# Sthiber/COSC_4397_Pathtracing_Raytracing_Project

Hardware: AMD Instinct MI355X
Metric: Msamples/s, cornell.txt 1920x1080 depth 8 (+PSNR vs 5000spp ref) (higher is better)
Workload: dtype f32

## Files before the change

cosc_4397_pathtracing_raytracing_project_amd/capi.py:

```python
from __future__ import annotations

import ctypes as C
import os
from typing import Optional, Sequence, Tuple

import numpy as np

_PKG = os.path.dirname(os.path.abspath(__file__))
LIB_PATH = os.environ.get("PT_AMD_LIB") or os.path.join(_PKG, "libpt_amd.so")
PT_MAX_DEPTH = 64
ARITH = {"exact": 0, "fma": 1, "fast": 2}
ARITH_NAMES = {v: k for k, v in ARITH.items()}
FEATURE_PLANES = 3
NOISE_PLANES = 2
NOISE_PIXELS_PER_PARTIAL = 1024
CONVERGENCE_WAVES = 16
CONVERGENCE_CAPACITY = 65536
FLT_MAX = float(np.finfo(np.float32).max)


class PtGeom(C.Structure):
    _fields_ = [("type", C.c_int32), ("materialid", C.c_int32), ("transform", C.c_float * 16),
                ("inverseTransform", C.c_float * 16), ("invTranspose", C.c_float * 16)]


class PtMaterial(C.Structure):
    _fields_ = [("color", C.c_float * 3), ("specular_exponent", C.c_float), ("specular_color", C.c_float * 3),
                ("hasReflective", C.c_float), ("hasRefractive", C.c_float), ("indexOfRefraction", C.c_float),
                ("emittance", C.c_float)]


class PtCamera(C.Structure):
    _fields_ = [("resolution", C.c_int32 * 2), ("position", C.c_float * 3), ("lookAt", C.c_float * 3),
                ("view", C.c_float * 3), ("up", C.c_float * 3), ("right", C.c_float * 3), ("fov", C.c_float * 2),
                ("pixelLength", C.c_float * 2)]


class PtBVHNode(C.Structure):
    _fields_ = [("bmin", C.c_float * 3), ("bmax", C.c_float * 3), ("left", C.c_int32), ("right", C.c_int32),
                ("geomIndex", C.c_int32)]


class PtGridInfo(C.Structure):
    _fields_ = [("res", C.c_int32 * 3), ("origin", C.c_float * 3), ("cell_size", C.c_float * 3), ("pad", C.c_float),
                ("num_cells", C.c_int32), ("num_records", C.c_int32), ("num_leaves", C.c_int32)]


class PtGridRecord(C.Structure):
    _fields_ = [("bmin", C.c_float * 3), ("bmax", C.c_float * 3), ("leaf", C.c_int32), ("neighbours", C.c_int32)]


class PtSceneDesc(C.Structure):
    _fields_ = [("geoms", C.POINTER(PtGeom)), ("num_geoms", C.c_int32), ("materials", C.POINTER(PtMaterial)),
                ("num_materials", C.c_int32), ("camera", PtCamera), ("trace_depth", C.c_int32)]


class PtOptions(C.Structure):
    _fields_ = [("device", C.c_int32), ("pixel_begin", C.c_int32), ("pixel_count", C.c_int32),
                ("iters_per_batch", C.c_int32), ("num_queues", C.c_int32), ("blocks_per_cu", C.c_int32),
                ("time_kernels", C.c_int32), ("legacy_traversal", C.c_int32), ("debug_flags", C.c_int32), ("unfused_primary", C.c_int32), ("unfused_bounces", C.c_int32), ("stripe_pixels", C.c_int32), ("stripe_stride", C.c_int32),
                ("arith", C.c_int32), ("aa_jitter", C.c_int32), ("convergence", C.c_int32),
                ("lds_table_kb", C.c_int32), ("primary_pieces", C.c_int32), ("paths_pieces", C.c_int32), ("paths_min_piece", C.c_int32)]


class PtStats(C.Structure):
    _fields_ = [("samples", C.c_int64), ("live_rays", C.c_int64 * PT_MAX_DEPTH), ("intersect_launches", C.c_int64),
                ("intersect_ms", C.c_double), ("render_ms", C.c_double), ("num_cus", C.c_int32),
                ("grid_blocks", C.c_int32), ("num_queues", C.c_int32), ("iters_per_batch", C.c_int32),
                ("device_bytes", C.c_int64), ("primary_fused", C.c_int32), ("bounces_fused", C.c_int32),
                ("arith", C.c_int32), ("grid_cells", C.c_int32), ("tight_leaves", C.c_int32), ("paths_waves", C.c_int32)]


class PtDenoiseOptions(C.Structure):
    _fields_ = [("levels", C.c_int32), ("sigma_color", C.c_float), ("sigma_normal", C.c_float), ("sigma_position", C.c_float),
                ("keep_albedo", C.c_int32)]


class PtError(RuntimeError):
    pass


_lib: Optional[C.CDLL] = None
_fp = C.POINTER(C.c_float)
_ip = C.POINTER(C.c_int32)


def lib() -> C.CDLL:
    global _lib
    if _lib is not None:
        return _lib
    if not os.path.exists(LIB_PATH):
        raise PtError(f"{LIB_PATH} not found: run `python -c 'import __graft_entry__ as g; g.build()'` "
                      "(hipcc --offload-arch=gfx950).  There is no CPU fallback.")
    L = C.CDLL(LIB_PATH)
    L.pt_last_error.restype = C.c_char_p
    L.pt_scene_load.argtypes = [C.c_char_p, C.c_int, C.c_int, C.POINTER(C.c_void_p)]
    L.pt_scene_free.argtypes = [C.c_void_p]
    L.pt_scene_free.restype = None
    L.pt_scene_desc.argtypes = [C.c_void_p, C.POINTER(PtSceneDesc)]
    L.pt_scene_iterations.argtypes = [C.c_void_p]
    L.pt_scene_image_name.argtypes = [C.c_void_p]
    L.pt_scene_image_name.restype = C.c_char_p
    L.pt_build_bvh.argtypes = [C.POINTER(PtGeom), C.c_int, C.POINTER(PtBVHNode), C.c_int]
    L.pt_build_grid.argtypes = [C.POINTER(PtGeom), C.c_int, C.c_int, C.POINTER(PtGridInfo), C.POINTER(C.c_uint32), C.POINTER(PtGridRecord)]
    if hasattr(L, "pt_selfcheck_ieee"):
        L.pt_selfcheck_ieee.argtypes = [C.c_int, C.c_int, C.c_uint64, C.c_uint64, C.c_uint32, C.POINTER(C.c_uint64)]
    if hasattr(L, "pt_traversal_boxes"):
        L.pt_traversal_boxes.argtypes = [C.POINTER(PtGeom), C.c_int, _fp, _fp]
    if hasattr(L, "pt_center_half_box"):
        L.pt_center_half_box.argtypes = [_fp, _fp, C.c_int, C.c_float, _fp, _fp]
        L.pt_center_half_box.restype = None
    L.pt_build_transform.argtypes = [_fp, _fp, _fp, _fp]
    L.pt_init.argtypes = [C.POINTER(PtSceneDesc), C.POINTER(PtOptions)]
    L.pt_render.argtypes = [C.c_int, C.c_int]
    L.pt_readback.argtypes = [_fp]
    L.pt_readback_device.argtypes = [C.c_void_p]
    L.pt_preview_rgba8.argtypes = [C.c_int, C.POINTER(C.c_uint8)]
    L.pt_preview_rgba8_device.argtypes = [C.c_int, C.c_void_p]
    L.pt_get_stats.argtypes = [C.POINTER(PtStats)]
    L.pt_stage_generate.argtypes = [C.c_int, C.c_int, _fp, _fp]
    L.pt_stage_intersect.argtypes = [C.c_int, _fp, _fp, _fp, _fp, _ip, _fp]
    if hasattr(L, "pt_stage_intersect_grid"):
        L.pt_stage_intersect_grid.argtypes = [C.c_int, _fp, _fp, C.c_int, _fp, _fp, _ip, _fp]
        L.pt_stage_grid_info.argtypes = [C.POINTER(PtGridInfo), C.POINTER(C.c_int32)]
    L.pt_stage_shade.argtypes = [C.c_int, C.c_int, _ip, _ip, _fp, _fp, _ip, _fp, _fp, _fp, _fp, _ip]
    _u8p = C.POINTER(C.c_uint8)
    L.pt_save_u8.argtypes = [C.c_float, _u8p]
    L.pt_stage_save_u8.argtypes = [C.c_int, C.c_int, C.c_float, _fp, _u8p]
    L.pt_ctx_create.argtypes = [C.POINTER(PtSceneDesc), C.POINTER(PtOptions), C.POINTER(C.c_void_p)]
    L.pt_ctx_destroy.argtypes = [C.c_void_p]
    L.pt_ctx_render.argtypes = [C.c_void_p, C.c_int, C.c_int]
    L.pt_ctx_sync.argtypes = [C.c_void_p]
    L.pt_ctx_readback.argtypes = [C.c_void_p, _fp]
    L.pt_ctx_readback_device.argtypes = [C.c_void_p, C.c_void_p]
    L.pt_ctx_save_u8.argtypes = [C.c_void_p, C.c_float, _u8p]
    L.pt_ctx_get_stats.argtypes = [C.c_void_p, C.POINTER(PtStats)]
    L.pt_ctx_reset_stats.argtypes = [C.c_void_p]
    L.pt_ctx_clear.argtypes = [C.c_void_p]
    L.pt_ctx_pixel_count.argtypes = [C.c_void_p]
    L.pt_group_create.argtypes = [C.POINTER(PtSceneDesc), C.POINTER(PtOptions), _ip, C.c_int, C.POINTER(C.c_void_p)]
    if hasattr(L, "pt_group_create_ex"):
        L.pt_group_create_ex.argtypes = [C.POINTER(PtSceneDesc), C.POINTER(PtOptions), _ip, C.c_int, C.c_int, C.POINTER(C.c_void_p)]
        L.pt_group_transport.argtypes = [C.c_void_p]
    L.pt_group_destroy.argtypes = [C.c_void_p]
    L.pt_group_size.argtypes = [C.c_void_p]
    L.pt_group_context.argtypes = [C.c_void_p, C.c_int]
    L.pt_group_context.restype = C.c_void_p
    L.pt_group_render.argtypes = [C.c_void_p, C.c_int, C.c_int]
    L.pt_group_sync.argtypes = [C.c_void_p]
    L.pt_group_gather.argtypes = [C.c_void_p, _fp]
    L.pt_group_gather_u8.argtypes = [C.c_void_p, C.c_float, _u8p]
    L.pt_group_preview_rgba8.argtypes = [C.c_void_p, C.c_int, _u8p]
    L.pt_write_png_rgb8.argtypes = [C.c_char_p, _u8p, C.c_int, C.c_int]
    L.pt_output_basename.argtypes = [C.c_char_p, C.c_int, C.c_char_p, C.c_int]
    L.pt_save_png.argtypes = [C.c_char_p, _fp, C.c_int, C.c_int, C.c_float]
    L.pt_save_hdr.argtypes = [C.c_char_p, _fp, C.c_int, C.c_int, C.c_float]
    L.pt_save_pfm.argtypes = [C.c_char_p, _fp, C.c_int, C.c_int, C.c_float]
    L.pt_load_pfm.argtypes = [C.c_char_p, _fp, C.c_int, _ip, _ip, C.c_float]
    _dp = C.POINTER(C.c_double)
    L.pt_psnr_from_sse.argtypes = [C.c_double, C.c_int64]
    L.pt_psnr_from_sse.restype = C.c_float
    L.pt_set_reference.argtypes = [_fp]
    L.pt_get_convergence.argtypes = [C.c_int, C.c_int, _dp]
    L.pt_iterations_to_clean.argtypes = [C.c_float, _ip]
    L.pt_ctx_set_reference.argtypes = [C.c_void_p, _fp]
    L.pt_ctx_get_convergence.argtypes = [C.c_void_p, C.c_int, C.c_int, _dp]
    L.pt_ctx_iterations_to_clean.argtypes = [C.c_void_p, C.c_float, _ip]
    L.pt_group_set_reference.argtypes = [C.c_void_p, _fp]
    L.pt_group_get_convergence.argtypes = [C.c_void_p, C.c_int, C.c_int, _dp]
    L.pt_group_iterations_to_clean.argtypes = [C.c_void_p, C.c_float, _ip]
    if hasattr(L, "pt_render_features"):
        L.pt_render_features.argtypes = [C.c_int, C.c_int]
        L.pt_readback_features.argtypes = [_fp]
        L.pt_ctx_render_features.argtypes = [C.c_void_p, C.c_int, C.c_int]
        L.pt_ctx_readback_features.argtypes = [C.c_void_p, _fp]
        L.pt_ctx_device_features.argtypes = [C.c_void_p]
        L.pt_ctx_device_features.restype = C.c_void_p
        L.pt_group_render_features.argtypes = [C.c_void_p, C.c_int, C.c_int]
        L.pt_group_gather_features.argtypes = [C.c_void_p, _fp]
    if hasattr(L, "pt_denoise"):
        _dno = C.POINTER(PtDenoiseOptions)
        L.pt_denoise.argtypes = [C.c_float, _dno, _fp]
        L.pt_ctx_denoise.argtypes = [C.c_void_p, C.c_float, _dno, _fp]
        L.pt_ctx_denoise_device.argtypes = [C.c_void_p, C.c_float, _dno, C.POINTER(C.c_void_p)]
        L.pt_group_denoise.argtypes = [C.c_void_p, C.c_float, _dno, _fp]
        L.pt_stage_denoise.argtypes = [C.c_int, C.c_int, _fp, _fp, C.c_float, _dno, _fp]
        L.pt_denoise_host.argtypes = [C.c_int, C.c_int, _fp, _fp, C.c_float, _dno, _fp]
    if hasattr(L, "pt_denoise_guided"):
        _dno = C.POINTER(PtDenoiseOptions)
        _guided = [C.c_int, C.c_int, _fp, _fp, _fp, C.c_int, C.c_int64, _dno]
        L.pt_denoise_guided.argtypes = [_dno, _fp]
        L.pt_ctx_denoise_guided.argtypes = [C.c_void_p, _dno, _fp]
        L.pt_ctx_denoise_guided_device.argtypes = [C.c_void_p, _dno, C.POINTER(C.c_void_p)]
        L.pt_group_denoise_guided.argtypes = [C.c_void_p, _dno, _fp]
        L.pt_stage_denoise_guided.argtypes = _guided + [_fp]
        L.pt_denoise_guided_host.argtypes = _guided + [_fp]
        L.pt_denoise_guided_variance_host.argtypes = _guided + [_fp, _fp]
    if hasattr(L, "pt_noise_fold"):
        _until = [C.c_int, C.c_int, C.c_int, C.c_float, _ip, _fp]
        L.pt_noise_fold.argtypes = []
        L.pt_get_noise.argtypes = [_dp, _ip, _ip]
        L.pt_readback_noise.argtypes = [_fp]
        L.pt_render_until.argtypes = _until
        L.pt_ctx_noise_fold.argtypes = [C.c_void_p]
        L.pt_ctx_get_noise.argtypes = [C.c_void_p, _dp, _ip, _ip]
        L.pt_ctx_readback_noise.argtypes = [C.c_void_p, _fp]
        L.pt_ctx_render_until.argtypes = [C.c_void_p] + _until
        L.pt_ctx_device_noise.argtypes = [C.c_void_p]
        L.pt_ctx_device_noise.restype = C.c_void_p
        L.pt_group_noise_fold.argtypes = [C.c_void_p]
        L.pt_group_get_noise.argtypes = [C.c_void_p, _dp, _ip, _ip]
        L.pt_group_render_until.argtypes = [C.c_void_p] + _until
        L.pt_noise_fold_host.argtypes = [C.c_int, _fp, _fp, C.c_int, C.c_int, C.c_int64, _dp]
    if hasattr(L, "pt_adaptive_round"):
        _i64p = C.POINTER(C.c_int64)
        _adaptive = [C.c_int, C.c_int, C.c_int, C.c_float, C.c_float, _ip, _i64p, _fp]
        L.pt_adaptive_round.argtypes = [C.c_int, C.c_int, C.c_float]
        L.pt_render_adaptive.argtypes = _adaptive
        L.pt_readback_adaptive.argtypes = [_ip]
        L.pt_resolve.argtypes = [_fp]
        L.pt_ctx_adaptive_round.argtypes = [C.c_void_p, C.c_int, C.c_int, C.c_float]
        L.pt_ctx_render_adaptive.argtypes = [C.c_void_p] + _adaptive
        L.pt_ctx_readback_adaptive.argtypes = [C.c_void_p, _ip]
        L.pt_ctx_resolve.argtypes = [C.c_void_p, _fp]
        L.pt_ctx_resolve_device.argtypes = [C.c_void_p, C.POINTER(C.c_void_p)]
        L.pt_adaptive_select_host.argtypes = [C.c_int, C.c_int, _fp, _ip, C.c_int, _ip]
        L.pt_stage_adaptive_select.argtypes = [C.c_int, C.c_int, _fp, _ip, C.c_int, _ip]
        L.pt_adaptive_merge_host.argtypes = [C.c_int, _fp, _fp, _ip, _ip, C.c_int, _fp, C.c_int, _dp]
        L.pt_stage_render_list.argtypes = [_ip, C.c_int, C.c_int, C.c_int, _fp]
    if hasattr(L, "pt_denoise_adaptive"):
        _dno = C.POINTER(PtDenoiseOptions)
        _dn_adaptive = [C.c_int, C.c_int, _fp, _fp, _fp, _ip, _dno]
        L.pt_denoise_adaptive.argtypes = [_dno, _fp]
        L.pt_ctx_denoise_adaptive.argtypes = [C.c_void_p, _dno, _fp]
        L.pt_ctx_denoise_adaptive_device.argtypes = [C.c_void_p, _dno, C.POINTER(C.c_void_p)]
        L.pt_stage_denoise_adaptive.argtypes = _dn_adaptive + [_fp]
        L.pt_denoise_adaptive_host.argtypes = _dn_adaptive + [_fp]
        L.pt_denoise_adaptive_variance_host.argtypes = _dn_adaptive + [_fp, _fp]
    _lib = L
    return L


def _check(rc: int) -> None:
    if rc != 0:
        raise PtError(lib().pt_last_error().decode(errors="replace"))


def _f(a: np.ndarray):
    assert a.dtype == np.float32 and a.flags.c_contiguous
    return a.ctypes.data_as(_fp)


def _i(a: np.ndarray):
    assert a.dtype == np.int32 and a.flags.c_contiguous
    return a.ctypes.data_as(_ip)


class Scene:

    def __init__(self, path: str, res: Optional[Tuple[int, int]] = None):
        self._h = C.c_void_p()
        w, h = res if res else (0, 0)
        _check(lib().pt_scene_load(os.fsencode(path), int(w), int(h), C.byref(self._h)))
        self.desc = PtSceneDesc()
        _check(lib().pt_scene_desc(self._h, C.byref(self.desc)))

    def __del__(self):
        h = getattr(self, "_h", None)
        if h is not None and h.value and _lib is not None:
            _lib.pt_scene_free(h)
            self._h = C.c_void_p()

    @property
    def resolution(self) -> Tuple[int, int]:
        return self.desc.camera.resolution[0], self.desc.camera.resolution[1]

    @property
    def trace_depth(self) -> int:
        return self.desc.trace_depth

    @trace_depth.setter
    def trace_depth(self, d: int) -> None:
        self.desc.trace_depth = int(d)

    @property
    def iterations(self) -> int:
        return lib().pt_scene_iterations(self._h)

    @property
    def image_name(self) -> str:
        return lib().pt_scene_image_name(self._h).decode()

    def geoms(self):
        return [self.desc.geoms[i] for i in range(self.desc.num_geoms)]

    def materials(self):
        return [self.desc.materials[i] for i in range(self.desc.num_materials)]

    def grid(self, forced: bool = False):
        info = PtGridInfo()
        rc = lib().pt_build_grid(self.desc.geoms, self.desc.num_geoms, int(forced), C.byref(info), None, None)
        if rc < 0:
            raise PtError(lib().pt_last_error().decode(errors="replace"))
        if rc == 0:
            return None
        start = (C.c_uint32 * (info.num_cells + 1))()
        recs = (PtGridRecord * info.num_records)()
        lib().pt_build_grid(self.desc.geoms, self.desc.num_geoms, int(forced), C.byref(info), start, recs)
        return info, np.frombuffer(start, np.uint32).copy(), recs

    def traversal_boxes(self):
        boxes = np.zeros((self.desc.num_geoms, 6), np.float32)
        cam = np.asarray(list(self.desc.camera.position), np.float32)
        rc = lib().pt_traversal_boxes(self.desc.geoms, self.desc.num_geoms, _f(cam), _f(boxes))
        if rc < 0:
            raise PtError(lib().pt_last_error().decode(errors="replace"))
        return boxes, rc

    def bvh(self):
        n = lib().pt_build_bvh(self.desc.geoms, self.desc.num_geoms, None, 0)
        arr = (PtBVHNode * n)()
        lib().pt_build_bvh(self.desc.geoms, self.desc.num_geoms, arr, n)
        return arr


def selfcheck_ieee(kind: int, first: int, count: int, seed: int = 0, arith: str = "exact") -> int:
    n = C.c_uint64(0)
    _check(lib().pt_selfcheck_ieee(ARITH[arith], kind, first, count, seed, C.byref(n)))
    return int(n.value)


def build_transform(trs: Sequence[float]):
    t = np.asarray(trs, np.float32).copy()
    m, i, it = (np.zeros(16, np.float32) for _ in range(3))
    lib().pt_build_transform(_f(t), _f(m), _f(i), _f(it))
    return m, i, it


def make_options(device: int = 0, pixel_begin: int = 0, pixel_count: int = 0, iters_per_batch: int = 0,
                 num_queues: int = 0, blocks_per_cu: int = 0, time_kernels: bool = False, legacy_traversal: bool = False,
                 debug_flags: int = 0, unfused_primary: bool = False, unfused_bounces: bool = False,
                 stripe_pixels: int = 0, stripe_stride: int = 0, arith="exact", aa_jitter: bool = False,
                 lds_table_kb: int = 0, primary_pieces: int = 0, paths_pieces: int = 0, paths_min_piece: int = 0, primary_share: int = 0,
                 convergence: int = 0) -> PtOptions:
    opt = PtOptions()
    opt.device = device
    opt.pixel_begin = pixel_begin
    opt.pixel_count = pixel_count
    opt.iters_per_batch = iters_per_batch
    opt.num_queues = num_queues
    opt.blocks_per_cu = blocks_per_cu
    opt.time_kernels = 1 if time_kernels else 0
    opt.legacy_traversal = 1 if legacy_traversal else 0
    opt.debug_flags = int(debug_flags)
    opt.unfused_primary = 1 if unfused_primary else 0
    opt.unfused_bounces = 1 if unfused_bounces else 0
    opt.stripe_pixels = int(stripe_pixels)
    opt.stripe_stride = int(stripe_stride)
    opt.arith = ARITH[arith] if isinstance(arith, str) else int(arith)
    opt.aa_jitter = 1 if aa_jitter else 0
    opt.convergence = int(convergence)
    opt.lds_table_kb = int(lds_table_kb)
    pp = int(primary_pieces)
    opt.primary_pieces = pp if pp < 0 else min(pp, 0x7fff) | max(0, min(int(primary_share), 64)) << 16
    opt.paths_pieces = int(paths_pieces)
    opt.paths_min_piece = int(paths_min_piece)
    return opt


def split_features(planes: np.ndarray) -> dict:
    p = planes.reshape(FEATURE_PLANES, -1, 4)
    return dict(normal=np.ascontiguousarray(p[0, :, :3]), depth=np.ascontiguousarray(p[0, :, 3]),
                albedo=np.ascontiguousarray(p[1, :, :3]), hits=np.ascontiguousarray(p[1, :, 3]),
# ... 504 lines not shown
```

cosc_4397_pathtracing_raytracing_project_amd/csrc/pt_api.cpp:

```cpp
#include <cmath>
#include <cstdarg>
#include <cstdio>
#include <cstring>
#include <string>

#include "pt_adaptive.h"
#include "pt_context.h"
#include "pt_scene.h"
#include "pt_sched.h"

namespace {

std::string g_err;
constexpr int kDebugFlags = 16 | 32 | 64 | 128 | 256 | 512 | ptk::kRetireEveryIteration | 2048 | ptk::kWholeRecords;
static_assert(sizeof(PtOptions) == 80, "capi.PtOptions mirrors this layout");
static_assert(PT_CONVERGENCE_WAVES == ptk::kConvWaves, "pt_amd.h documents the size of the convergence metric's partial sums");
}
int pt_fail(const char* fmt, ...) {
  char buf[1024];
  va_list ap;
  va_start(ap, fmt);
  vsnprintf(buf, sizeof(buf), fmt, ap);
  va_end(ap);
  g_err = buf;
  return -1;
}

namespace ptc {
static PtContext* g_default = nullptr;
PtContext* default_context() { return g_default; }

int get_events(Ctx& g, EventPair* ev) {
  if (!g.free_events.empty()) {
    *ev = g.free_events.back();
    g.free_events.pop_back();
    return 0;
  }
  HIP_OK(hipEventCreate(&ev->a));
  HIP_OK(hipEventCreate(&ev->b));
  return 0;
}
static int resolve_events(Ctx& g) {
  auto drain = [&](std::vector<EventPair>& pending, double& total_ms) -> int {
    for (auto& e : pending) {
      float ms = 0;
      HIP_OK(hipEventElapsedTime(&ms, e.a, e.b));
      total_ms += ms;
      g.free_events.push_back(e);
    }
    pending.clear();
    return 0;
  };
  g.isect_launches += (int64_t)g.pending_isect.size();
  return drain(g.pending_isect, g.isect_ms) || drain(g.pending_render, g.render_ms) ? -1 : 0;
}

ptk::SceneTables tables(const Ctx& g) {
  ptk::SceneTables t = g.scene;
  if (g.debug_flags & 16) t.cull_margin = INFINITY;
  if (g.debug_flags & 32) t.top_xor = 0;
  t.lds_table_bytes = g.lds_table_bytes;
  t.max_batch_iters = g.K;
  t.trace_depth = g.depth;
  t.scan_nodes_lds = -1;
  t.use_grid = !g.grids.empty() && g.grid_enabled && !(g.debug_flags & 512) ? 1 : 0;
  if (t.use_grid) {
    const Ctx::DeviceGrid& gr = g.grids[g.grid_pick];
    t.lds_table_bytes = -1;
    t.grid_start = gr.d_start + gr.guard;
    t.grid_items = gr.d_items;
    t.grid_items_b = gr.d_items_b;
    for (int a = 0; a < 3; ++a)
      t.grid_res[a] = gr.shape.res[a], t.grid_min[a] = gr.shape.gmin[a], t.grid_cs[a] = gr.shape.cs[a], t.grid_inv_cs[a] = gr.shape.inv_cs[a];
    t.grid_pad = gr.shape.pad;
  }
  return t;
}

static size_t pathbuf_words(int64_t stride) { return (size_t)(2 * stride + (stride * ptd::kPathPlane2Bytes + 15) / 16); }
static int alloc_pathbuf(Ctx& g, ptd::PathBuf* b, int64_t stride) {
  b->stride = stride;
  return dalloc(g, &b->r, pathbuf_words(stride));
}
static int alloc_hitbuf(Ctx& g, ptd::HitBuf* h, int64_t stride) {
  h->stride = stride;
  return dalloc(g, &h->t, stride) || dalloc(g, &h->n, 3 * stride) || dalloc(g, &h->mat, stride) || dalloc(g, &h->p, 3 * stride) ? -1 : 0;
}

static ptd::Queues queues_for(const Ctx& g, int grid) {
  ptd::Queues q = g.qs;
  q.W = grid * ptk::kWavesPerBlock;
  return q;
}

static int primary_share_of(const Ctx& g) { return (g.debug_flags & 128) ? 1 : g.primary_share ? g.primary_share : ptk::kShareMax; }
static bool shares_first_hit(const Ctx& g) { return ptk::primary_shares(primary_share_of(g), g.aa_jitter, !g.fuse_bounces); }

ptk::BatchInfo tile_batch(const Ctx& g, int iter_first, int K) {
  ptk::BatchInfo b{};
  b.iter_first = iter_first;
  b.K = K;
  b.N = g.N;
  b.pixel_begin = g.pixel_begin;
  b.trace_depth = g.depth;
  b.aa_jitter = g.aa_jitter ? 1 : 0;
  b.stripe = g.stripe;
  b.gap = g.stripe ? g.stripe_stride - g.stripe : 0;
  b.inv_stripe = g.stripe ? 1.0f / (float)g.stripe : 0.0f;
  return b;
}

int run_batch(Ctx& g, int iter_first, int kb) {
  ptk::BatchInfo b = tile_batch(g, iter_first, kb);
  b.slot_shift = g.slot_shift;
  b.flat = g.fuse_bounces ? 0 : 1;
  b.primary_share = primary_share_of(g);
  b.primary_pieces = g.primary_pieces ? g.primary_pieces
                     : ptk::primary_shares(b) ? ptk::auto_shared_pieces(kb, g.qs.nq, g.ret.wq0) : ptk::auto_primary_pieces(kb, g.qs.nq, g.ret.wq0);
  b.paths_pieces = g.paths_pieces;
  b.retire_once = ptk::retires_once(b, g.debug_flags) ? 1 : 0;
  b.split_records = ptk::splits_records(b, g.debug_flags) ? 1 : 0;
  b.list = g.list;
  if (b.list) b.stripe = 1, b.gap = 0, b.inv_stripe = 1.0f;
  const ptk::SceneTables sc = tables(g);
  const ptk::KernelApi& k = *g.k;
  auto cnt_row = [&](int d) { return g.d_cnt + ptk::cnt_index(g.qs, d, 0); };
  int d0 = 0;
  if (g.fuse_primary) {
    k.primary(g.stream, g.grid_primary, sc, g.dcam, b, queues_for(g, g.grid_primary), cnt_row(0), cnt_row(1), g.buf[1],
              g.ret);
    d0 = 1;
  } else {
    k.generate(g.stream, g.grid_gen, g.dcam, b, queues_for(g, g.grid_gen), g.buf[0], cnt_row(0));
  }
  int src = d0 & 1;
  const bool all_depths = g.grid_paths > 0;
  EventPair ev{};
  auto timed_from = [&]() -> int {
    if (!g.time_kernels) return 0;
    if (get_events(g, &ev)) return -1;
    HIP_OK(hipEventRecord(ev.a, g.stream));
    return 0;
  };
  auto timed_to = [&]() -> int {
    if (!g.time_kernels) return 0;
    HIP_OK(hipEventRecord(ev.b, g.stream));
    g.pending_isect.push_back(ev);
    return 0;
  };
  if (all_depths) {
    if (timed_from()) return -1;
    k.paths(g.stream, g.grid_paths, sc, b, queues_for(g, g.grid_paths), g.d_cnt, g.buf[1], g.ret);
    if (timed_to()) return -1;
  }
  for (int d = d0; d < g.depth && !all_depths; ++d) {
    const int32_t* cin = cnt_row(d);
    int32_t* cout = cnt_row(d + 1);
    if (timed_from()) return -1;
    k.intersect(g.stream, g.grid_isect, sc, queues_for(g, g.grid_isect), cin, g.buf[src], g.hits, g.legacy, d == 0);
    if (timed_to()) return -1;
    k.shade(g.stream, g.grid_shade, sc, b, d, queues_for(g, g.grid_shade), cin, cout, g.buf[src], g.hits, g.buf[src ^ 1], g.ret);
    src ^= 1;
  }
  k.count_stats(g.stream, g.qs, g.d_cnt, g.depth, g.d_stats);
  ptk::ConvInfo cv{g.d_ref, g.d_partial, -1, kb};
  if (g.conv_live) {
    if (g.conv_have_ref) cv.first_k = 0;
    else if (g.conv >= iter_first && g.conv < iter_first + kb) cv.capture_k = g.conv - iter_first, cv.first_k = cv.capture_k + 1, g.conv_have_ref = true;
    g.conv_last = std::max(g.conv_last, iter_first + kb - 1);
  }
  if (cv.capture_k >= 0 || cv.first_k < kb) k.collect_conv(g.stream, b, g.qs, g.ret, g.d_image, cv, g.d_sse);
  else k.collect(g.stream, b, g.qs, g.ret, g.d_image);
  HIP_OK(hipGetLastError());
  g.samples += (int64_t)kb * g.N;
  if (g.pending_isect.size() > 16384) {
    HIP_OK(hipStreamSynchronize(g.stream));
    if (resolve_events(g)) return -1;
  }
  return 0;
}

void plan_launch(Ctx& g) {
  if (!g.borrowed) g.lds_table_bytes = g.k->lds_table_limit(tables(g), g.lds_table_forced);
  const ptk::SceneTables t = tables(g);
  g.grid_gen = g.num_cus * std::min(g.cap_bpc, g.k->resident_blocks_per_cu(ptk::kGenerate, t));
  g.grid_isect = g.num_cus * std::min(g.cap_bpc, g.k->resident_blocks_per_cu(g.legacy ? ptk::kIntersectLegacy : ptk::kIntersect, t));
  g.grid_shade = g.num_cus * std::min(g.cap_bpc, g.k->resident_blocks_per_cu(ptk::kShade, t));
  g.grid_primary = g.num_cus * std::min(g.cap_bpc, g.k->resident_blocks_per_cu(shares_first_hit(g) ? ptk::kPrimaryShared : ptk::kPrimary, t));
  g.ret.wq0 = ptk::wave_slot(0, g.qs.Q, g.grid_primary * ptk::kWavesPerBlock).wq;
  g.grid_paths = (g.fuse_bounces && g.depth > 1) ? g.num_cus * std::min(g.cap_bpc, g.k->resident_blocks_per_cu(ptk::kPaths, t)) : 0;
  g.qs.paths_W = g.grid_paths * ptk::kWavesPerBlock;
}

static int choose_traversal(Ctx& g) {
  auto drop_unused_grids = [&](size_t keep) {
    for (size_t i = 0; i < g.grids.size(); ++i) {
      const Ctx::DeviceGrid& d = g.grids[i];
      if (i == keep) continue;
      for (void* p : {(void*)d.d_start, (void*)d.d_items, d.d_items_b != d.d_items ? (void*)d.d_items_b : nullptr}) {
        if (!p) continue;
        (void)hipFree(p);
        g.allocs.erase(std::remove(g.allocs.begin(), g.allocs.end(), p), g.allocs.end());
      }
      g.device_bytes -= (int64_t)d.bytes;
    }
    g.grids = {g.grids[keep]};
    g.grid_pick = 0;
  };
  if (g.grids.empty()) return 0;
  if (!g.fuse_bounces || (g.debug_flags & (256 | 512))) {
    drop_unused_grids(0);
    return 0;
  }
  auto time_one = [&](float* ms) -> int {
    plan_launch(g);
    for (int rep = 0; rep < 2; ++rep) {
      EventPair ev{};
      if (get_events(g, &ev)) return -1;
      HIP_OK(hipEventRecord(ev.a, g.stream));
      if (run_batch(g, 1, std::min(g.K, 8))) return -1;
      HIP_OK(hipEventRecord(ev.b, g.stream));
      HIP_OK(hipStreamSynchronize(g.stream));
      HIP_OK(hipEventElapsedTime(ms, ev.a, ev.b));
      g.free_events.push_back(ev);
    }
    return 0;
  };
  g.grid_enabled = false;
  if (time_one(&g.probe_ms[0])) return -1;
  g.grid_enabled = true;
  size_t best = 0;
  for (size_t i = 0; i < g.grids.size(); ++i) {
    float ms = 0.f;
    g.grid_pick = i;
    if (time_one(&ms)) return -1;
    if (i == 0 || ms < 0.97f * g.probe_ms[1]) g.probe_ms[1] = ms, best = i;
  }
  drop_unused_grids(best);
  g.grid_enabled = g.probe_ms[1] < 0.95f * g.probe_ms[0];
  plan_launch(g);
  HIP_OK(hipMemsetAsync(g.d_image, 0, 3 * (size_t)g.N * sizeof(float), g.stream));
  HIP_OK(hipMemsetAsync(g.d_stats, 0, PT_MAX_DEPTH * sizeof(unsigned long long), g.stream));
  HIP_OK(hipStreamSynchronize(g.stream));
  g.samples = 0;
  return 0;
}

ptd::Queues single_queue(const Ctx& g, int n) {
  ptd::Queues qs{};
  qs.Q = 1;
  const ptk::QueuePlan p = ptk::queue_plan(n, 1, 1);
  qs.cap = p.cap;
  qs.W = g.grid * ptk::kWavesPerBlock;
  qs.cnt_stride = 16;
  qs.nq = p.nq;
  qs.inv_nq = 1.0f / (float)qs.nq;
  return qs;
}

void destroy(Ctx* c) {
  if (!c) return;
  destroy(c->worker);
  (void)hipSetDevice(c->device);
  if (c->stream) (void)hipStreamSynchronize(c->stream);
  for (void* p : c->allocs) (void)hipFree(p);
  auto kill = [](std::vector<EventPair>& v) {
    for (auto& e : v) {
      (void)hipEventDestroy(e.a);
      (void)hipEventDestroy(e.b);
    }
    v.clear();
  };
  kill(c->free_events);
  kill(c->pending_isect);
  kill(c->pending_render);
  if (c->stream && !c->borrowed) (void)hipStreamDestroy(c->stream);
  delete c;
}

static int open_device(Ctx& g, const PtOptions& opt) {
  g.arith = opt.arith;
  g.k = ptk::api_for(opt.arith);
  if (!g.k) return pt_fail("pt_init: arith %d is not one of PT_ARITH_EXACT / PT_ARITH_FMA / PT_ARITH_FAST", opt.arith);
  if (opt.convergence < -1) return pt_fail("pt_init: convergence %d is not 0 (off), N > 0 (frame captured at iteration N) or -1 (frame supplied)", opt.convergence);
  if (opt.convergence > PT_CONVERGENCE_CAPACITY) return pt_fail("pt_init: convergence %d exceeds PT_CONVERGENCE_CAPACITY (%d iterations)", opt.convergence, PT_CONVERGENCE_CAPACITY);
  if (opt.primary_pieces > 0 && (opt.primary_pieces >> 16) > ptk::kShareMax) return pt_fail("pt_init: primary_pieces 0x%x: primary_share %d exceeds %d (PT_PRIMARY_PIECES)", opt.primary_pieces, opt.primary_pieces >> 16, ptk::kShareMax);
  if (opt.debug_flags & ~kDebugFlags) return pt_fail("pt_init: debug_flags 0x%x: bits 0x%x are not defined", opt.debug_flags, opt.debug_flags & ~kDebugFlags);
  int ndev = 0;
  HIP_OK(hipGetDeviceCount(&ndev));
  if (ndev <= 0) return pt_fail("pt_init: no HIP device (this library has no CPU fallback)");
  if (opt.device < 0 || opt.device >= ndev) return pt_fail("pt_init: device %d of %d", opt.device, ndev);
  g.device = opt.device;
  HIP_OK(hipSetDevice(g.device));
  hipDeviceProp_t prop;
  HIP_OK(hipGetDeviceProperties(&prop, g.device));
  g.num_cus = prop.multiProcessorCount;
  HIP_OK(hipStreamCreateWithFlags(&g.stream, hipStreamNonBlocking));
  return 0;
}

static void take_scene_and_options(Ctx& g, const PtSceneDesc* sc, const PtOptions& opt) {
  g.cam = sc->camera;
  g.depth = sc->trace_depth;
  g.dcam.res_x = g.cam.resolution[0], g.dcam.res_y = g.cam.resolution[1];
  std::memcpy(g.dcam.pos, g.cam.position, 12);
  std::memcpy(g.dcam.view, g.cam.view, 12);
  std::memcpy(g.dcam.up, g.cam.up, 12);
  std::memcpy(g.dcam.right, g.cam.right, 12);
  g.dcam.pl_x = g.cam.pixelLength[0], g.dcam.pl_y = g.cam.pixelLength[1];
  g.legacy = opt.legacy_traversal != 0;
  g.aa_jitter = opt.aa_jitter != 0;
  g.debug_flags = opt.debug_flags;
  g.conv = opt.convergence;
  auto pieces = [](int v, int automatic) { return v ? std::clamp(v, 1, 0x7fff) : automatic; };
  g.lds_table_forced = opt.lds_table_kb ? std::clamp(opt.lds_table_kb, 0, ptk::kLdsTableBytes / 1024) * 1024 : -1;
  g.primary_pieces = pieces(opt.primary_pieces < 0 ? opt.primary_pieces : opt.primary_pieces & 0xffff, 0);
  g.primary_share = opt.primary_pieces < 0 ? 0 : std::min(opt.primary_pieces >> 16 & 0x7f, ptk::kShareMax);
  g.paths_pieces = ptk::pack_paths_pieces(pieces(opt.paths_pieces, 2), pieces(opt.paths_min_piece, 64));
  g.fuse_primary = !g.legacy && !opt.unfused_primary;
  g.fuse_bounces = g.fuse_primary && !opt.unfused_bounces;
  g.cap_bpc = opt.blocks_per_cu > 0 ? std::min(opt.blocks_per_cu, 8) : 8;
}

int batch_iters_for(int iters_per_batch, int N, int* slot_shift) {
  int K = iters_per_batch;
  if (K <= 0) {
    const int64_t target = 48ll << 20;
    K = (int)std::max<int64_t>(1, std::min<int64_t>(256, (target + N - 1) / N));
  }
  int shift = 1;
  while ((1ll << shift) < N) ++shift;
  if (shift > 30) return pt_fail("pt_init: tiles of more than 2^30 pixels are not supported");
  while (K > 1 && K > (1 << (31 - shift))) --K;
  if (slot_shift) *slot_shift = shift;
  return K;
}

int plan_batches(Ctx& g, const PtOptions& opt) {
  const int W = g.cam.resolution[0], H = g.cam.resolution[1];
  g.opt_iters_per_batch = opt.iters_per_batch, g.opt_num_queues = opt.num_queues;
  g.pixel_begin = opt.pixel_begin;
  g.N = opt.pixel_count > 0 ? opt.pixel_count : W * H - opt.pixel_begin;
  g.stripe = opt.stripe_pixels;
  g.stripe_stride = opt.stripe_stride;
  if (g.stripe < 0 || (g.stripe > 0 && g.stripe_stride < g.stripe)) return pt_fail("pt_init: bad stripe %d / stride %d", g.stripe, g.stripe_stride);
  {
    int64_t last = (int64_t)g.pixel_begin + g.N - 1;
    if (g.stripe > 0) last = (int64_t)g.pixel_begin + (g.N - 1) + (int64_t)((g.N - 1) / g.stripe) * (g.stripe_stride - g.stripe);
    if (g.pixel_begin < 0 || g.N <= 0 || last >= (int64_t)W * H)
      return pt_fail("pt_init: tile [%d, +%d, stripe %d/%d) outside %dx%d", opt.pixel_begin, opt.pixel_count, g.stripe, g.stripe_stride, W, H);
    if (g.stripe > 0 && g.N / g.stripe >= 32768) return pt_fail("pt_init: more than 32767 stripes");
    if (H >= 32768) return pt_fail("pt_init: image height %d not supported (>= 32768)", H);
  }
  const int K = batch_iters_for(opt.iters_per_batch, g.N, &g.slot_shift);
  if (K < 0) return -1;

  int Q = opt.num_queues > 0 ? opt.num_queues : 256;
  const int cu_waves = g.num_cus * ptk::kWavesPerBlock;
  if (Q > cu_waves) Q = cu_waves;
  while (cu_waves % Q) --Q;
  if (opt.num_queues <= 0)
    while (ptk::chunks_per_queue(g.N, Q) > 128 && 2 * Q <= cu_waves && cu_waves % (2 * Q) == 0) Q *= 2;
  const ptk::QueuePlan plan = ptk::queue_plan(g.N, Q, K);
  const int grid = g.num_cus * 8;
  g.K = K;
  g.grid = grid;
  g.qs.Q = Q;
  g.qs.W = grid * ptk::kWavesPerBlock;
  g.qs.cnt_stride = 16;
  g.qs.nq = plan.nq;
  g.qs.inv_nq = 1.0f / (float)plan.nq;
  g.qs.cap = plan.cap;
  g.stride = (int64_t)Q * g.qs.cap;
  g.ret.seg_cap = plan.seg_cap;
  g.ret.kmax = K;
  return 0;
}

template <typename T>
static const T* upload(Ctx& g, const std::vector<T>& v) {
  T* p = nullptr;
  if (dalloc(g, &p, v.size())) return nullptr;
  const hipError_t e = hipMemcpy(p, v.data(), v.size() * sizeof(T), hipMemcpyHostToDevice);
  return e == hipSuccess ? p : (pt_fail("hipMemcpy(%zu bytes) failed: %s", v.size() * sizeof(T), hipGetErrorString(e)), nullptr);
}
static int upload_tables(Ctx& g, const pt::HostTables& t) {
  ptk::SceneTables& s = g.scene;
  s.num_nodes = (int)t.nodes.size(), s.num_geoms = (int)t.geoms.size(), s.num_mats = (int)t.mats.size(), s.num_top = (int)t.top.size();
  std::memcpy(s.root_min, t.root_min, 12);
  std::memcpy(s.root_max, t.root_max, 12);
  s.cull_margin = t.cull_margin;
  s.top_xor = t.top_xor;
  s.has_triangles = t.has_triangles ? 1 : 0;
  g.tight_leaves = t.tight_leaves;
  if (!(s.nodes = upload(g, t.nodes)) || !(s.geoms = upload(g, t.geoms)) || !(s.mats = upload(g, t.mats)) || !(s.top = upload(g, t.top))) return -1;
  s.nodes_b = s.nodes, s.top_b = s.top;
  if (!t.nodes_b.empty() && (!(s.nodes_b = upload(g, t.nodes_b)) || !(s.top_b = upload(g, t.top_b)))) return -1;
  for (const pt::Grid& gr : t.grids) {
    Ctx::DeviceGrid d{gr.shape, gr.guard, nullptr, nullptr, nullptr, 0, gr.start};
    const int64_t before = g.device_bytes;
    if (!(d.d_start = upload(g, gr.start)) || !(d.d_items = upload(g, gr.items))) return -1;
    if (!(d.d_items_b = gr.items_b.empty() ? d.d_items : upload(g, gr.items_b))) return -1;
    d.bytes = (size_t)(g.device_bytes - before);
    g.grids.push_back(d);
  }
  return 0;
}

static __global__ void k_poison_records(ptd::Word4* rec, unsigned long long per_queue, unsigned long long total, int Q) {
  const float nan = __builtin_nanf("");
  for (unsigned long long i = (unsigned long long)blockIdx.x * blockDim.x + threadIdx.x; i < total; i += (unsigned long long)gridDim.x * blockDim.x)
    rec[i] = ptd::Word4{nan, nan, nan, __int_as_float(ptk::chunk_pixel((int)(i / per_queue), 0, Q))};
}

int alloc_batch_buffers(Ctx& g) {
  const int Q = g.qs.Q;
  if (alloc_pathbuf(g, &g.buf[0], g.stride) || alloc_pathbuf(g, &g.buf[1], g.stride)) return -1;
  for (const ptd::PathBuf& pb : g.buf) HIP_OK(hipMemset(pb.r, 0xff, pathbuf_words(pb.stride) * sizeof(ptd::Word4)));
  if (!g.fuse_bounces && alloc_hitbuf(g, &g.hits, g.stride)) return -1;
  {
    const size_t regions = (size_t)Q * g.ret.kmax;
    const size_t wq_max = ptk::sub_stride(g.num_cus * 8 * ptk::kWavesPerBlock, Q);
    if (dalloc(g, &g.ret.rec, regions * g.ret.seg_cap)) return -1;
    if (ensure(g, g.ret.cnt, regions * sizeof(*g.ret.cnt), Zero::blocking) || ensure(g, g.ret.sub, regions * wq_max * sizeof(*g.ret.sub), Zero::blocking)) return -1;
    {
      const size_t per_queue = (size_t)g.ret.kmax * g.ret.seg_cap;
      hipLaunchKernelGGL(k_poison_records, dim3((unsigned)std::min<size_t>((regions * g.ret.seg_cap + 255) / 256, 65536)), dim3(256), 0, g.stream, g.ret.rec,
                         (unsigned long long)per_queue, (unsigned long long)(regions * g.ret.seg_cap), Q);
      HIP_OK(hipGetLastError());
    }
  }
  const size_t image_bytes = 3 * (size_t)g.N * sizeof(float);
  const size_t cnt_words = ptk::cnt_index(g.qs, g.depth + 1, 0);
  if (ensure(g, g.d_image, image_bytes, Zero::blocking) || ensure(g, g.d_cnt, cnt_words * sizeof(int32_t), Zero::blocking) ||
      ensure(g, g.d_stats, PT_MAX_DEPTH * sizeof(*g.d_stats), Zero::blocking))
    return -1;
  if (!(g.debug_flags & 64) && ensure(g, g.qs.deal, (size_t)ptk::deal_map(g.qs).words() * sizeof(int32_t), Zero::blocking)) return -1;
  if (g.conv) {
    const size_t partials = (size_t)g.K * Q * ptk::kConvWaves;
    if (ensure(g, g.d_ref, image_bytes, Zero::blocking) || ensure(g, g.d_partial, partials * sizeof(double), Zero::blocking)) return -1;
    if (dalloc(g, &g.d_sse, (size_t)PT_CONVERGENCE_CAPACITY)) return -1;
    HIP_OK(hipMemset(g.d_sse, 0xff, (size_t)PT_CONVERGENCE_CAPACITY * sizeof(double)));
  }
  HIP_OK(hipDeviceSynchronize());
  return 0;
}

static int setup(Ctx& g, const PtSceneDesc* sc, const PtOptions& opt) {
  if (open_device(g, opt)) return -1;
  take_scene_and_options(g, sc, opt);
  if (plan_batches(g, opt)) return -1;
  if ((size_t)sc->num_materials * sizeof(ptd::Mat) > 60 * 1024) return pt_fail("pt_init: %zu materials exceed the LDS table", (size_t)sc->num_materials);
  const pt::HostTables host = pt::build_scene_tables(*sc, g.debug_flags, g.k->boxes_center_half != 0);
  if (upload_tables(g, host)) return -1;
  plan_launch(g);
  if (alloc_batch_buffers(g) || choose_traversal(g)) return -1;
  g.time_kernels = opt.time_kernels != 0;
  g.conv_live = g.conv != 0;
  return 0;
}

int need(const PtContext* c, const char* who) { return c ? 0 : pt_fail("%s: pt_init has not been called", who); }

int admit(const PtContext& g, const char* who, unsigned req) {
  if ((req & kNotFailed) && g.failed) return pt_fail("%s: an earlier batch of this context failed (%s); free it and create a new one", who, g_err.c_str());
  if ((req & kUniform) && g.adaptive)
    return pt_fail("%s: the renderer is in the adaptive state (pt_adaptive_round): one sample count no longer describes the image; read it with pt_resolve, or "
                   "return to the uniform state with pt_clear", who);
  const int W = g.cam.resolution[0];
  if ((req & kWholeRows) && (g.stripe || g.pixel_begin % W || g.N % W))
    return pt_fail("%s: the tile must consist of whole contiguous image rows (begin %d, count %d, stripe %d, width %d)", who, g.pixel_begin, g.N, g.stripe, W);
  if ((req & kFoldedAll) && g.rendered != g.noise_iters)
    return pt_fail("%s: %lld iteration(s) rendered since the last fold; fold first (pt_noise_fold)", who, (long long)(g.rendered - g.noise_iters));
  if (req & kOnDevice) HIP_OK(hipSetDevice(g.device));
  return 0;
}

}
using namespace ptc;

extern "C" {

const char* pt_last_error(void) { return g_err.c_str(); }

int pt_selfcheck_ieee(int arith, int kind, uint64_t first, uint64_t count, uint32_t seed, uint64_t* mismatches) {
  const ptk::KernelApi* k = ptk::api_for(arith);
  if (!k || kind < 0 || kind > 4 || !mismatches) return pt_fail("pt_selfcheck_ieee: bad argument");
  unsigned long long* d = nullptr;
  HIP_OK(hipMalloc(&d, sizeof(*d)));
  hipError_t e = hipMemset(d, 0, sizeof(*d));
  if (e == hipSuccess) {
    k->ieee_check(nullptr, kind, first, count, seed, d);
    e = hipGetLastError();
  }
  unsigned long long h = 0;
  if (e == hipSuccess) e = hipMemcpy(&h, d, sizeof(h), hipMemcpyDeviceToHost);
  (void)hipFree(d);
  if (e != hipSuccess) return pt_fail("pt_selfcheck_ieee: %s", hipGetErrorString(e));
  *mismatches = h;
  return 0;
}

struct PtScene {
  pt::Scene scene;
  explicit PtScene(const std::string& f) : scene(f) {}
};

int pt_scene_load(const char* path, int res_w, int res_h, PtScene** out) {
  if (!path || !out) return pt_fail("pt_scene_load: null argument");
  try {
    PtScene* s = new PtScene(path);
    if (res_w > 0 && res_h > 0) s->scene.overrideResolution(res_w, res_h);
    s->scene.applyInitialCameraState();
    *out = s;
    return 0;
  } catch (const std::exception& e) {
    return pt_fail("pt_scene_load: %s", e.what());
  }
}
void pt_scene_free(PtScene* s) { delete s; }
int pt_scene_desc(const PtScene* s, PtSceneDesc* out) {
  if (!s || !out) return pt_fail("pt_scene_desc: null argument");
  *out = s->scene.desc();
  return 0;
}
int pt_scene_iterations(const PtScene* s) { return s ? (int)s->scene.state.iterations : 0; }
const char* pt_scene_image_name(const PtScene* s) { return s ? s->scene.state.imageName.c_str() : ""; }

int pt_build_bvh(const PtGeom* geoms, int num_geoms, PtBVHNode* out, int cap) {
  std::vector<PtBVHNode> nodes;
  pt::buildBVH(geoms, num_geoms, nodes);
  if (out) std::memcpy(out, nodes.data(), sizeof(PtBVHNode) * std::min<size_t>(nodes.size(), (size_t)std::max(cap, 0)));
  return (int)nodes.size();
}

int pt_traversal_boxes(const PtGeom* geoms, int num_geoms, const float camera_position[3], float* boxes) {
  if (!geoms || num_geoms <= 0 || !camera_position || !boxes) return pt_fail("pt_traversal_boxes: null argument");
  pt::ThreadedBvh bvh = pt::threaded_bvh(geoms, num_geoms);
  double olo[3], ohi[3];
  pt::origin_region(bvh.ref[0].bmin, bvh.ref[0].bmax, camera_position, olo, ohi);
  const int tightened = pt::tighten_sphere_leaves(bvh.nodes, geoms, olo, ohi);
  for (const ptd::Node& n : bvh.nodes)
    if (n.geom >= 0) std::memcpy(boxes + 6 * (size_t)n.geom, n.bmin, 12), std::memcpy(boxes + 6 * (size_t)n.geom + 3, n.bmax, 12);
  return tightened;
}

int pt_build_grid(const PtGeom* geoms, int num_geoms, int forced, PtGridInfo* info, uint32_t* cell_start, PtGridRecord* records) {
  if (!geoms || num_geoms <= 0 || !info) return pt_fail("pt_build_grid: null argument");
  const pt::ThreadedBvh bvh = pt::threaded_bvh(geoms, num_geoms);
  std::memset(info, 0, sizeof(*info));
  info->num_leaves = num_geoms;
  if (!forced && (int)bvh.nodes.size() < pt::kGridNodes) return 0;
  pt::Grid gr;
  if (!pt::build_grid(bvh.nodes, geoms, num_geoms, bvh.ref[0].bmin, bvh.ref[0].bmax, 0.0, 0.0, forced != 0, gr)) return 0;
  for (int a = 0; a < 3; ++a) info->res[a] = gr.shape.res[a], info->origin[a] = gr.shape.gmin[a], info->cell_size[a] = gr.shape.cs[a];
  info->pad = gr.shape.pad;
  info->num_cells = (int32_t)(gr.start.size() - 1);
  info->num_records = (int32_t)gr.items.size();
  if (cell_start) std::memcpy(cell_start, gr.start.data(), gr.start.size() * sizeof(uint32_t));
  static_assert(sizeof(PtGridRecord) == sizeof(ptd::Node), "PtGridRecord mirrors the device record");
  if (records) std::memcpy(records, gr.items.data(), gr.items.size() * sizeof(ptd::Node));
  return 1;
}

void pt_center_half_box(const float lo[3], const float hi[3], int inner, float magnitude, float center[3], float half_extent[3]) {
  float a[3] = {lo[0], lo[1], lo[2]}, b[3] = {hi[0], hi[1], hi[2]};
  pt::center_half_box(a, b, inner != 0, (double)magnitude);
  std::memcpy(center, a, 12);
  std::memcpy(half_extent, b, 12);
}

int pt_build_transform(const float* trs, float* transform, float* inverse, float* invTranspose) {
  if (!trs || !transform || !inverse || !invTranspose) return pt_fail("pt_build_transform: null argument");
  pt::buildTransform(trs, transform, inverse, invTranspose);
  return 0;
}

int pt_ctx_create(const PtSceneDesc* sc, const PtOptions* opt_in, PtContext** out) {
  if (!out) return pt_fail("pt_ctx_create: null output");
  *out = nullptr;
  if (!sc) return pt_fail("pt_init: null scene");
  if (sc->num_geoms <= 0 || !sc->geoms) return pt_fail("pt_init: scene has no geometry");
  if (sc->num_materials <= 0 || !sc->materials) return pt_fail("pt_init: scene has no materials");
  if (sc->trace_depth <= 0 || sc->trace_depth > PT_MAX_DEPTH) return pt_fail("pt_init: trace_depth %d out of range", sc->trace_depth);
  const int W = sc->camera.resolution[0], H = sc->camera.resolution[1];
  if (W <= 0 || H <= 0 || (int64_t)W * H > (1ll << 30)) return pt_fail("pt_init: bad resolution %dx%d", W, H);
  for (int i = 0; i < sc->num_geoms; ++i) {
    if (sc->geoms[i].materialid < 0 || sc->geoms[i].materialid >= sc->num_materials)
      return pt_fail("pt_init: geom %d references material %d of %d", i, sc->geoms[i].materialid, sc->num_materials);
    if (sc->geoms[i].type < PT_GEOM_SPHERE || sc->geoms[i].type > PT_GEOM_TRIANGLE)
      return pt_fail("pt_init: geom %d has unknown type %d", i, sc->geoms[i].type);
  }
  PtOptions opt{};
  if (opt_in) opt = *opt_in;
  PtContext* c = new PtContext();
  if (setup(*c, sc, opt)) {
    destroy(c);
    return -1;
  }
  *out = c;
  return 0;
}

int pt_ctx_destroy(PtContext* c) {
  if (c == g_default) g_default = nullptr;
  destroy(c);
  return 0;
}

int pt_ctx_render(PtContext* c, int iter_first, int iter_count) {
  if (need(c, "pt_render")) return -1;
  if (iter_count <= 0) return 0;
  Ctx& g = *c;
  if (admit(g, "pt_render", kNotFailed | kUniform)) return -1;
  if (g.conv_live) {
    if (iter_first < 1 || (int64_t)iter_first + iter_count - 1 > PT_CONVERGENCE_CAPACITY)
      return pt_fail("pt_render: iterations %d .. %lld outside 1 .. %d (PT_CONVERGENCE_CAPACITY) with the convergence metric on", iter_first,
                  (long long)iter_first + iter_count - 1, PT_CONVERGENCE_CAPACITY);
    if (g.conv < 0 && !g.conv_have_ref) return pt_fail("pt_render: PtOptions.convergence is -1 but no reference frame has been supplied (pt_set_reference)");
  }
  HIP_OK(hipSetDevice(g.device));
  EventPair ev{};
  if (get_events(g, &ev)) return -1;
  HIP_OK(hipEventRecord(ev.a, g.stream));
  const int end = iter_first + iter_count;
  for (int it = iter_first; it < end; it += g.K)
    if (run_batch(g, it, std::min(g.K, end - it))) {
      g.failed = true;
      g.free_events.push_back(ev);
      return -1;
    }
  HIP_OK(hipEventRecord(ev.b, g.stream));
  g.pending_render.push_back(ev);
  g.rendered += iter_count;
  return 0;
}

int pt_ctx_sync(PtContext* c) {
  if (need(c, "pt_sync")) return -1;
  HIP_OK(hipSetDevice(c->device));
  HIP_OK(hipStreamSynchronize(c->stream));
  return resolve_events(*c);
}

int pt_ctx_readback(PtContext* c, float* out) {
  if (need(c, "pt_readback")) return -1;
  return copy_out(c, "pt_readback", out, 3, [&](const float** d) { return *d = c->d_image, 0; });
}

int pt_ctx_readback_device(PtContext* c, void* out) {
  if (need(c, "pt_readback_device")) return -1;
  return copy_out(c, "pt_readback_device", static_cast<float*>(out), 3, [&](const float** d) { return *d = c->d_image, 0; }, hipMemcpyDeviceToDevice);
}

const float* pt_ctx_device_image(PtContext* c) { return c ? c->d_image : nullptr; }
void* pt_ctx_stream(PtContext* c) { return c ? (void*)c->stream : nullptr; }
int pt_ctx_pixel_count(const PtContext* c) { return c ? c->N : 0; }
int pt_ctx_device(const PtContext* c) { return c ? c->device : -1; }

int pt_ctx_save_u8_device(PtContext* c, float samples, const uint8_t** rgb8_dev) {
  if (need(c, "pt_save_u8")) return -1;
  Ctx& g = *c;
  const int W = g.cam.resolution[0];
  if (!(samples > 0.0f)) return pt_fail("pt_save_u8: samples must be positive");
  if (admit(g, "pt_save_u8", kUniform)) return -1;
  if (g.pixel_begin % W || g.N % W || (g.stripe && g.stripe != W))
    return pt_fail("pt_save_u8: the tile must consist of whole image rows (begin %d, count %d, stripe %d, width %d)", g.pixel_begin, g.N, g.stripe, W);
  HIP_OK(hipSetDevice(g.device));
  if (ensure(g, g.d_rgb8, 3 * (size_t)g.N)) return -1;
  g.k->save_u8(g.stream, g.N, W, samples, g.d_image, g.d_rgb8);
  HIP_OK(hipGetLastError());
  if (rgb8_dev) *rgb8_dev = g.d_rgb8;
  return 0;
}
int pt_ctx_save_u8(PtContext* c, float samples, uint8_t* rgb8_host) {
  return copy_out(c, "pt_save_u8", rgb8_host, 3, [&](const uint8_t** d) { return pt_ctx_save_u8_device(c, samples, d); });
}

int pt_ctx_preview_rgba8_device(PtContext* c, int iterations, void* rgba_dev) {
  if (need(c, "pt_preview_rgba8_device")) return -1;
  if (!rgba_dev || iterations <= 0) return pt_fail("pt_preview_rgba8_device: bad argument");
  if (admit(*c, "pt_preview_rgba8_device", kUniform | kOnDevice)) return -1;
  c->k->preview(c->stream, c->N, iterations, c->d_image, reinterpret_cast<uchar4*>(rgba_dev));
  HIP_OK(hipStreamSynchronize(c->stream));
  return 0;
}

int pt_ctx_preview_rgba8(PtContext* c, int iterations, uint8_t* rgba_host) {
  if (need(c, "pt_preview_rgba8")) return -1;
  if (!rgba_host || iterations <= 0) return pt_fail("pt_preview_rgba8: bad argument");
  if (admit(*c, "pt_preview_rgba8", kUniform | kOnDevice)) return -1;
  uchar4* d = nullptr;
  HIP_OK(hipMalloc((void**)&d, (size_t)c->N * 4));
  c->k->preview(c->stream, c->N, iterations, c->d_image, d);
  hipError_t e = hipMemcpyAsync(rgba_host, d, (size_t)c->N * 4, hipMemcpyDeviceToHost, c->stream);
  if (e == hipSuccess) e = hipStreamSynchronize(c->stream);
  (void)hipFree(d);
  if (e != hipSuccess) return pt_fail("pt_preview_rgba8: %s", hipGetErrorString(e));
  return 0;
}

int pt_ctx_get_stats(PtContext* c, PtStats* out) {
  if (need(c, "pt_get_stats")) return -1;
  if (!out) return pt_fail("pt_get_stats: null");
  if (pt_ctx_sync(c)) return -1;
  Ctx& g = *c;
  std::memset(out, 0, sizeof(*out));
  unsigned long long st[PT_MAX_DEPTH];
  HIP_OK(hipMemcpy(st, g.d_stats, sizeof(st), hipMemcpyDeviceToHost));
  for (int d = 0; d < PT_MAX_DEPTH; ++d) out->live_rays[d] = (int64_t)st[d];
  out->samples = g.samples;
  out->intersect_launches = g.isect_launches;
  out->intersect_ms = g.isect_ms;
  out->render_ms = g.render_ms;
  out->num_cus = g.num_cus;
  out->grid_blocks = g.grid_paths > 0 ? g.grid_paths : g.grid_isect;
  out->num_queues = g.qs.Q;
  out->iters_per_batch = g.K;
  out->device_bytes = g.device_bytes;
  out->primary_fused = g.fuse_primary ? 1 : 0;
  out->bounces_fused = g.fuse_bounces ? 1 : 0;
  out->arith = g.arith;
  if (tables(g).use_grid && g.fuse_bounces) {
    const int* res = g.grids[g.grid_pick].shape.res;
    out->grid_cells = res[0] * res[1] * res[2];
  }
  out->tight_leaves = g.tight_leaves;
  out->paths_waves = 0;
  if (g.qs.deal && g.grid_paths > 0) {
    const ptk::DealMap dm = ptk::deal_map(g.qs);
    std::vector<int32_t> first((size_t)dm.made_for() + 1);
    HIP_OK(hipMemcpy(first.data(), g.qs.deal + dm.first(0), first.size() * sizeof(int32_t), hipMemcpyDeviceToHost));
    if (first[dm.made_for()] == g.qs.paths_W) {
      int lo = first[1] - first[0], hi = lo;
      for (int q = 1; q < g.qs.Q; ++q) lo = std::min(lo, first[q + 1] - first[q]), hi = std::max(hi, first[q + 1] - first[q]);
      out->paths_waves = std::min(lo, 0xffff) << 16 | std::min(hi, 0xffff);
    }
  }
  return 0;
}

int pt_ctx_reset_stats(PtContext* c) {
  if (need(c, "pt_reset_stats")) return -1;
  if (pt_ctx_sync(c)) return -1;
  Ctx& g = *c;
  HIP_OK(hipMemsetAsync(g.d_stats, 0, PT_MAX_DEPTH * sizeof(unsigned long long), g.stream));
  HIP_OK(hipStreamSynchronize(g.stream));
  g.samples = 0;
  g.isect_ms = g.render_ms = 0;
  g.isect_launches = 0;
  return 0;
}

int pt_ctx_clear(PtContext* c) {
  if (need(c, "pt_clear")) return -1;
  if (pt_ctx_sync(c)) return -1;
  HIP_OK(hipMemsetAsync(c->d_image, 0, 3 * (size_t)c->N * sizeof(float), c->stream));
  if (c->d_feat) HIP_OK(hipMemsetAsync(c->d_feat, 0, (size_t)PT_FEATURE_PLANES * c->N * sizeof(float4), c->stream));
  if (c->d_noise) HIP_OK(hipMemsetAsync(c->d_noise, 0, pt_noise_state_bytes((size_t)c->N), c->stream));
  c->noise_groups = 0;
  c->noise_iters = c->rendered = 0;
  if (c->d_acnt) HIP_OK(hipMemsetAsync(c->d_acnt, 0, (size_t)c->N * sizeof(ptad::Cnt), c->stream));
  c->adaptive = false;
  c->adaptive_rounds = 0;
  c->adaptive_last = 0;
  if (c->conv) {
    HIP_OK(hipMemsetAsync(c->d_sse, 0xff, (size_t)PT_CONVERGENCE_CAPACITY * sizeof(double), c->stream));
    c->conv_last = 0;
    if (c->conv > 0) c->conv_have_ref = false;
  }
  return pt_ctx_reset_stats(c);
}

int pt_ctx_set_reference(PtContext* c, const float* rgb_avg_host) {
  if (need(c, "pt_set_reference")) return -1;
  if (!rgb_avg_host) return pt_fail("pt_set_reference: null image");
  if (c->conv != -1) return pt_fail("pt_set_reference: the renderer was created with PtOptions.convergence = %d, not -1", c->conv);
  if (pt_ctx_sync(c)) return -1;
  HIP_OK(hipMemcpyAsync(c->d_ref, rgb_avg_host, 3 * (size_t)c->N * sizeof(float), hipMemcpyHostToDevice, c->stream));
  HIP_OK(hipStreamSynchronize(c->stream));
  c->conv_have_ref = true;
  return 0;
}

int pt_ctx_get_convergence(PtContext* c, int iter_first, int iter_count, double* sse) {
  if (need(c, "pt_get_convergence")) return -1;
  if (!c->conv) return pt_fail("pt_get_convergence: the renderer was created with PtOptions.convergence = 0 (metric off)");
  if (iter_count < 0 || (iter_count > 0 && !sse)) return pt_fail("pt_get_convergence: bad argument");
  if (pt_ctx_sync(c)) return -1;
  for (int j = 0; j < iter_count; ++j) sse[j] = -1.0;
  const int64_t lo = std::max<int64_t>(iter_first, 1), hi = std::min<int64_t>((int64_t)iter_first + iter_count, (int64_t)PT_CONVERGENCE_CAPACITY + 1);
  if (lo >= hi) return 0;
  double* dst = sse + (lo - iter_first);
  HIP_OK(hipMemcpy(dst, c->d_sse + (lo - 1), (size_t)(hi - lo) * sizeof(double), hipMemcpyDeviceToHost));
  for (int64_t j = 0; j < hi - lo; ++j)
    if (!(dst[j] >= 0.0)) dst[j] = -1.0;
  return 0;
}

int pt_ctx_iterations_to_clean(PtContext* c, float threshold_db, int* iteration) {
  if (need(c, "pt_iterations_to_clean")) return -1;
  if (!iteration) return pt_fail("pt_iterations_to_clean: null output");
  std::vector<double> sse((size_t)std::max(c->conv_last, 0));
  if (pt_ctx_get_convergence(c, 1, (int)sse.size(), sse.data())) return -1;
  *iteration = -1;
  for (size_t i = 0; i < sse.size(); ++i)
    if (sse[i] >= 0.0 && pt_psnr_from_sse(sse[i], c->N) > threshold_db) {
      *iteration = (int)i + 1;
      break;
    }
  return 0;
}

int pt_free(void) {
  PtContext* c = g_default;
  g_default = nullptr;
  destroy(c);
  return 0;
}
int pt_init(const PtSceneDesc* sc, const PtOptions* opt) {
  pt_free();
  return pt_ctx_create(sc, opt, &g_default);
}
int pt_render(int iter_first, int iter_count) { return pt_ctx_render(g_default, iter_first, iter_count); }
int pt_sync(void) { return pt_ctx_sync(g_default); }
int pt_readback(float* out) { return pt_ctx_readback(g_default, out); }
int pt_readback_device(void* out) { return pt_ctx_readback_device(g_default, out); }
int pt_save_u8(float samples, uint8_t* rgb8_host) { return pt_ctx_save_u8(g_default, samples, rgb8_host); }
int pt_preview_rgba8(int iterations, uint8_t* rgba_host) { return pt_ctx_preview_rgba8(g_default, iterations, rgba_host); }
int pt_preview_rgba8_device(int iterations, void* rgba_dev) { return pt_ctx_preview_rgba8_device(g_default, iterations, rgba_dev); }
int pt_get_stats(PtStats* out) { return pt_ctx_get_stats(g_default, out); }
int pt_reset_stats(void) { return pt_ctx_reset_stats(g_default); }
int pt_clear(void) { return pt_ctx_clear(g_default); }
int pt_render_features(int iter_first, int iter_count) { return pt_ctx_render_features(g_default, iter_first, iter_count); }
int pt_readback_features(float* planes_host) { return pt_ctx_readback_features(g_default, planes_host); }
int pt_denoise(float samples, const PtDenoiseOptions* opt, float* rgb_avg_host) { return pt_ctx_denoise(g_default, samples, opt, rgb_avg_host); }
int pt_denoise_guided(const PtDenoiseOptions* opt, float* rgb_avg_host) { return pt_ctx_denoise_guided(g_default, opt, rgb_avg_host); }
int pt_denoise_adaptive(const PtDenoiseOptions* opt, float* rgb_avg_host) { return pt_ctx_denoise_adaptive(g_default, opt, rgb_avg_host); }
int pt_noise_fold(void) { return pt_ctx_noise_fold(g_default); }
int pt_get_noise(double* sse, int* groups, int* iterations) { return pt_ctx_get_noise(g_default, sse, groups, iterations); }
int pt_readback_noise(float* planes_host) { return pt_ctx_readback_noise(g_default, planes_host); }
int pt_render_until(int iter_first, int max_iters, int group_iters, float target_db, int* iters_done, float* psnr_db) {
  return pt_ctx_render_until(g_default, iter_first, max_iters, group_iters, target_db, iters_done, psnr_db);
}
int pt_adaptive_round(int iter_first, int group_iters, float fraction) { return pt_ctx_adaptive_round(g_default, iter_first, group_iters, fraction); }
int pt_render_adaptive(int iter_first, int max_iters, int group_iters, float fraction, float target_db, int* iters_done, int64_t* samples_done,
                       float* psnr_db) {
  return pt_ctx_render_adaptive(g_default, iter_first, max_iters, group_iters, fraction, target_db, iters_done, samples_done, psnr_db);
}
int pt_readback_adaptive(int32_t* counts) { return pt_ctx_readback_adaptive(g_default, counts); }
int pt_resolve(float* rgb_avg_host) { return pt_ctx_resolve(g_default, rgb_avg_host); }
int pt_set_reference(const float* rgb_avg_host) { return pt_ctx_set_reference(g_default, rgb_avg_host); }
int pt_get_convergence(int iter_first, int iter_count, double* sse) { return pt_ctx_get_convergence(g_default, iter_first, iter_count, sse); }
int pt_iterations_to_clean(float threshold_db, int* iteration) { return pt_ctx_iterations_to_clean(g_default, threshold_db, iteration); }

}
```

cosc_4397_pathtracing_raytracing_project_amd/csrc/pt_context.h:

```cpp
#pragma once
#include <hip/hip_runtime.h>

#include <algorithm>
#include <cstdint>
#include <vector>

#include "../../include/pt_amd.h"
#include "pt_device.h"
#include "pt_internal.h"
#include "pt_kernels.h"
#include "pt_tables.h"

#define HIP_OK(expr)                                                                                      \
  do {                                                                                                    \
    hipError_t e_ = (expr);                                                                               \
    if (e_ != hipSuccess) return pt_fail("%s failed: %s (%s:%d)", #expr, hipGetErrorString(e_), __FILE__, __LINE__); \
  } while (0)

struct EventPair {
  hipEvent_t a, b;
};

struct PtShared {
  int device = 0;
  hipStream_t stream = nullptr;
  const ptk::KernelApi* k = nullptr;
  int arith = 0;
  int num_cus = 0;
  PtCamera cam{};
  ptd::Camera dcam{};
  int depth = 0;
  ptk::SceneTables scene{};
  int lds_table_bytes = -1;
  int lds_table_forced = -1;
  int primary_pieces = 0;
  int primary_share = 0;
  int paths_pieces = 0;
  struct DeviceGrid {
    pt::GridShape shape;
    size_t guard;
    const uint32_t* d_start;
    const ptd::Node* d_items;
    const ptd::Node* d_items_b;
    size_t bytes;
    std::vector<uint32_t> start;
  };
  std::vector<DeviceGrid> grids;
  size_t grid_pick = 0;
  int tight_leaves = 0;
  bool grid_enabled = true;
  int cap_bpc = 8;
  bool legacy = false;
  int debug_flags = 0;
  bool fuse_primary = true, fuse_bounces = true;
  bool aa_jitter = false;
};

struct PtContext : PtShared {
  int N = 0, pixel_begin = 0, K = 1;
  int slot_shift = 0;
  int stripe = 0, stripe_stride = 0;
  int grid = 0;
  int grid_gen = 0, grid_isect = 0, grid_shade = 0;
  ptd::Queues qs{};
  int64_t stride = 0;
  std::vector<void*> allocs;
  int64_t device_bytes = 0;
  float probe_ms[2] = {0.f, 0.f};
  int grid_primary = 0, grid_paths = 0;
  ptd::PathBuf buf[2]{};
  ptd::HitBuf hits{};
  ptd::RetireBuf ret{};
  float* d_image = nullptr;
  float4* d_feat = nullptr;
  int grid_features = 0;
  void* d_denoise = nullptr;
  void* d_noise = nullptr;
  int noise_groups = 0;
  int64_t noise_iters = 0;
  int64_t rendered = 0;
  int conv = 0;
  bool conv_live = false;
  bool conv_have_ref = false;
  int conv_last = 0;
  float* d_ref = nullptr;
  double* d_partial = nullptr;
  double* d_sse = nullptr;
  uint8_t* d_rgb8 = nullptr;
  int32_t* d_cnt = nullptr;
  unsigned long long* d_stats = nullptr;
  bool time_kernels = false;
  std::vector<EventPair> free_events, pending_isect, pending_render;
  double isect_ms = 0, render_ms = 0;
  int64_t isect_launches = 0;
  int64_t samples = 0;
  bool failed = false;
  int opt_iters_per_batch = 0, opt_num_queues = 0;
  bool borrowed = false;
  const int32_t* list = nullptr;
  PtContext* worker = nullptr;
  int32_t* d_list = nullptr;
  void* d_acnt = nullptr;
  void* d_select = nullptr;
  float* d_resolved = nullptr;
  bool adaptive = false;
  int adaptive_rounds = 0;
  int64_t adaptive_last = 0;
};

namespace ptc {
using Ctx = PtContext;

PtContext* default_context();

template <typename T>
int dalloc(Ctx& g, T** out, size_t count) {
  void* p = nullptr;
  size_t bytes = std::max<size_t>(count * sizeof(T), 16);
  hipError_t e = hipMalloc(&p, bytes);
  if (e != hipSuccess) return pt_fail("hipMalloc(%zu bytes) failed: %s", bytes, hipGetErrorString(e));
  g.allocs.push_back(p);
  g.device_bytes += (int64_t)bytes;
  *out = reinterpret_cast<T*>(p);
  return 0;
}
enum class Zero { none, blocking, on_stream };
template <typename T>
int ensure(Ctx& g, T*& p, size_t bytes, Zero zero = Zero::none) {
  if (p) return 0;
  char* q = nullptr;
  if (dalloc(g, &q, bytes)) return -1;
  p = reinterpret_cast<T*>(q);
  if (zero == Zero::blocking) HIP_OK(hipMemset(q, 0, bytes));
  if (zero == Zero::on_stream) HIP_OK(hipMemsetAsync(q, 0, bytes, g.stream));
  return 0;
}
struct Scratch {
  std::vector<void*> p;
  ~Scratch() { for (void* q : p) (void)hipFree(q); }
  template <typename T>
  T* get(size_t n) {
    void* q = nullptr;
    if (hipMalloc(&q, std::max<size_t>(n * sizeof(T), 16)) != hipSuccess) return nullptr;
    p.push_back(q);
    return reinterpret_cast<T*>(q);
  }
};

int need(const PtContext* c, const char* who);
enum Require : unsigned {
  kNotFailed = 1,
  kUniform = 2,
  kWholeRows = 4,
  kFoldedAll = 8,
  kOnDevice = 16,
};
int admit(const PtContext& g, const char* who, unsigned req);

template <typename T, typename Source>
int copy_out(PtContext* c, const char* who, T* host, size_t per_pixel, Source source, hipMemcpyKind kind = hipMemcpyDeviceToHost) {
  if (!host) return pt_fail("%s: null buffer", who);
  const T* d = nullptr;
  if (source(&d)) return -1;
  HIP_OK(hipSetDevice(c->device));
  HIP_OK(hipMemcpyAsync(host, d, per_pixel * (size_t)c->N * sizeof(T), kind, c->stream));
  return pt_ctx_sync(c);
}

ptk::SceneTables tables(const Ctx& g);
ptk::BatchInfo tile_batch(const Ctx& g, int iter_first, int K);
int run_batch(Ctx& g, int iter_first, int kb);
int batch_iters_for(int iters_per_batch, int N, int* slot_shift);
int plan_batches(Ctx& g, const PtOptions& opt);
void plan_launch(Ctx& g);
int alloc_batch_buffers(Ctx& g);
int get_events(Ctx& g, EventPair* ev);
ptd::Queues single_queue(const Ctx& g, int n);
void destroy(Ctx* c);
int ensure_worker(Ctx& g, int m);
int render_list(Ctx& g, int iter_first, int iter_count);
}
```

cosc_4397_pathtracing_raytracing_project_amd/csrc/pt_kernels.hip:

```cpp
#include "pt_kernels.h"

#include <float.h>

#include <type_traits>

#include "pt_lds.h"
#include "pt_sched.h"
#include "pt_portable_math.h"

#ifndef PT_ARITH
#define PT_ARITH 0
#endif
#if PT_ARITH == 0
#define PT_NS arith_exact
#define PT_API_FN api_exact
#elif PT_ARITH == 1
#define PT_NS arith_fma
#define PT_API_FN api_fma
#elif PT_ARITH == 2
#define PT_NS arith_fast
#define PT_API_FN api_fast
#else
#error "PT_ARITH must be 0, 1 or 2"
#endif
// ... 573 lines not shown
        scan_step<EX>(reinterpret_cast<const v4f*>(nodes), wk.o, wk.ri, act, wk.cur, bt, cand, at_n, aux);
      },
      [&](bool cand, int at_n, int own, int aux) {
        const bool cbox = cand && geoms[aux].type == 1;
        const bool csph = cand && !cbox;
        const unsigned long long mb = ballot(cbox), msp = ballot(csph);
        if (mb | msp) {
          if (nb + ns + 128 > kCandCap) {
            flush_candidates<false, EX>(w, nb, ns, lane, o, d, nodes, geoms, tri);
            nb = ns = 0;
          }
          const uint32_t entry = ((uint32_t)at_n << 6) | (uint32_t)own;
          const int rb = rank_in(mb);
          const int rs = rank_in(msp);
          const int cb = __popcll(mb), cs = __popcll(msp);
          if (cbox) w.list[nb + rb] = entry;
          if (csph) w.list[kCandCap - ns - cs + rs] = entry;
          nb += cb;
          ns += cs;
        }
      });
  if (nb + ns) flush_candidates<false, EX>(w, nb, ns, lane, o, d, nodes, geoms, tri);
}

typedef __attribute__((address_space(4))) const v4f cnode4;
template <bool EX>
PT_DEV void trace_group_packet(const WaveLds& w, const ptd::Node* __restrict__ nodes, int num_nodes, const ptd::Geom* __restrict__ geoms,
                               f3 o, f3 d, bool valid, int lane, bool tri) {
  const RayInv ri = Ar<EX>::ray_inv(d, o);
  w.best[lane] = kNoHit;
  int nb = 0, ns = 0;
  cnode4* cn = (cnode4*)(uintptr_t)nodes;
  int i = 0;
  while (i < num_nodes) {
    const v4f NA = cn[2 * i], NB = cn[2 * i + 1];
    const bool pass = valid && Ar<EX>::slab(o, ri, NA.x, NA.y, NA.z, NA.w, NB.x, NB.y);
    const unsigned long long m = ballot(pass);
    const int gi = __float_as_int(NB.w);
    if (!m) {
      i = __float_as_int(NB.z);
      continue;
    }
    if (gi >= 0) {
      if (nb + ns + 64 > kCandCap) {
        flush_candidates<true, EX>(w, nb, ns, lane, o, d, nodes, geoms, tri);
        nb = ns = 0;
      }
      const int rank = rank_in(m), cnt = __popcll(m);
      const uint32_t entry = ((uint32_t)i << 6) | (uint32_t)lane;
      if (__builtin_amdgcn_readfirstlane(geoms[gi].type) == 1) {
        if (pass) w.list[nb + rank] = entry;
        nb += cnt;
      } else {
        if (pass) w.list[kCandCap - ns - cnt + rank] = entry;
        ns += cnt;
      }
    }
    ++i;
  }
  if (nb + ns) flush_candidates<true, EX>(w, nb, ns, lane, o, d, nodes, geoms, tri);
}

template <bool TABLES_IN_LDS, bool EX>
__global__ __launch_bounds__(kBlock) void k_intersect(SceneTables sc, ptd::Queues qs, const int32_t* __restrict__ cnt_in,
                                                      ptd::PathBuf paths, ptd::HitBuf hits) {
  extern __shared__ float4 lds_raw[];
  char* lds = reinterpret_cast<char*>(lds_raw);
  const IntersectLds L = intersect_lds<TABLES_IN_LDS>(sc);
  stage16(lds + L.top, EX ? sc.top : sc.top_b, top_bytes(sc));
  const float4* top = reinterpret_cast<const float4*>(lds + L.top);
  const ptd::Node* nodes = EX ? sc.nodes : sc.nodes_b;
  const ptd::Geom* geoms = sc.geoms;
  if (TABLES_IN_LDS) {
    stage16(lds + L.nodes, nodes, node_bytes(sc));
    stage16(lds + L.geoms, sc.geoms, geom_bytes(sc));
    nodes = reinterpret_cast<const ptd::Node*>(lds + L.nodes);
    geoms = reinterpret_cast<const ptd::Geom*>(lds + L.geoms);
  }
  __syncthreads();
  const int wib = threadIdx.x >> 6;
  WaveLds w = wave_lds_init(lds + L.waves + wib * L.wave_bytes);
  const int ntop = sc.num_top;

  const int wave = blockIdx.x * kWavesPerBlock + wib;
  const int lane = lane_id();
  const auto [q, r, wq] = wave_slot(wave, qs.Q, qs.W);
  const int n_q = cnt_in[cnt_index(qs, 0, q)];
  const int64_t HS = hits.stride;
  const int64_t qbase = (int64_t)q * qs.cap;
  const int last = qs.cap - 64 + lane;
  f3 no, nd;
  path_load_ray(paths, qbase + min(r * 64 + lane, last), no, nd);
  for (int j = r; j * 64 < n_q; j += wq) {
    const int i = j * 64 + lane;
    const bool valid = i < n_q;
    const int64_t at = qbase + i;
    const f3 o = no, d = nd;
    path_load_ray(paths, qbase + min((j + wq) * 64 + lane, last), no, nd);
    trace_group<EX>(w, top, ntop, nodes, geoms, o, d, valid, lane, sc.cull_margin, sc.top_xor, sc.has_triangles != 0);

    const unsigned long long best = w.best[lane];
    const bool hit = (uint32_t)(best >> 32) != 0x7f7fffffu;
    const int leaf = hit ? (int)(uint32_t)best : 0;
    hits.t[at] = hit ? __uint_as_float((uint32_t)(best >> 32)) : -1.0f;
    hits.n[at] = hit ? w.rec[0 * 64 + lane] : 0.f;
    hits.n[HS + at] = hit ? w.rec[1 * 64 + lane] : 0.f;
    hits.n[2 * HS + at] = hit ? w.rec[2 * 64 + lane] : 0.f;
    hits.mat[at] = hit ? geoms[nodes[leaf].geom].material : 0;
    hits.p[at] = hit ? w.rec[3 * 64 + lane] : 0.f;
    hits.p[HS + at] = hit ? w.rec[4 * 64 + lane] : 0.f;
    hits.p[2 * HS + at] = hit ? w.rec[5 * 64 + lane] : 0.f;
  }
}

#include "pt_shade.inc"
template <bool SMALL, int NPAR>
struct Carry {
  using Ent = typename std::conditional<SMALL, uint16_t, uint32_t>::type;
  unsigned long long* best;
  float* rec;
  Ent* ent;
  float* ray;
  f3 cam_o;
  static constexpr int kRayPlanes = SMALL ? 3 : 6;
  int* slot;
  uint32_t* gix;
  const float* qo_tab;
  int head, count;
  int appended, processed;
  const __attribute__((address_space(3))) v4f* lnodes;
  bool lds_nodes;
};
template <bool SMALL, int NPAR>
PT_DEV Carry<SMALL, NPAR> carry_init(char* base) {
  using M = CarryMap<SMALL, NPAR>;
  Carry<SMALL, NPAR> c;
  c.best = reinterpret_cast<unsigned long long*>(base + M::best);
  c.rec = reinterpret_cast<float*>(base + M::rec);
  c.ray = reinterpret_cast<float*>(base + M::ray);
  c.ent = reinterpret_cast<typename Carry<SMALL, NPAR>::Ent*>(base + M::ent);
  c.slot = reinterpret_cast<int*>(base + M::slot);
  c.cam_o = mk(0.f, 0.f, 0.f);
  c.head = c.count = c.appended = c.processed = 0;
  c.gix = nullptr;
  c.qo_tab = nullptr;
  c.lnodes = nullptr;
  c.lds_nodes = false;
  return c;
}
template <bool SMALL, int NPAR, bool EX = false, bool LEAN = false, bool QO = false>
PT_DEV void carry_chunk(Carry<SMALL, NPAR>& c, int n, int lane, const ptd::Node* __restrict__ nodes,
                        const ptd::Geom* __restrict__ geoms) {
  const bool valid = lane < n;
  PT_STAT(6, 1);
  PT_STAT(7, n);
  const int idx = (c.head + lane) & (kRing - 1);
  const uint32_t entry = (uint32_t)c.ent[idx];
  const int src = (int)(entry & 63u);
  const int par = (int)((entry >> 6) & 1u);
  const uint32_t leaf = entry >> 7;
  constexpr int RP = Carry<SMALL, NPAR>::kRayPlanes;
  const float* ray = c.ray + par * RP * 64 + src;
  const f3 ro = SMALL ? c.cam_o : mk(ray[0 * 64], ray[1 * 64], ray[2 * 64]);
  const f3 rd = mk(ray[(RP - 3) * 64], ray[(RP - 2) * 64], ray[(RP - 1) * 64]);
  const uint32_t gw = LEAN ? c.gix[idx] : 0u;
  const int gi = valid ? (LEAN ? (int)(gw & 0x3fffffffu) : nodes[leaf].geom) : 0;
  const ptd::Geom* G = geoms + gi;
  f3 pt = mk(0.f, 0.f, 0.f), nrm = mk(0.f, 0.f, 0.f);
  float t = -1.0f;
  if (LEAN) t = Ar<EX>::template geom_test<-1, false, true>(G, ro, rd, pt, nrm, mk(0.f, 0.f, 0.f), valid ? (int)(gw >> 30) : 0);
  else if (QO) t = Ar<EX>::template geom_test<-1, true>(G, ro, rd, pt, nrm, mk(c.qo_tab[3 * gi], c.qo_tab[3 * gi + 1], c.qo_tab[3 * gi + 2]));
  else t = Ar<EX>::template geom_test<-1, false>(G, ro, rd, pt, nrm, mk(0.f, 0.f, 0.f));
  keep_closest(&c.best[par * 64 + src], c.rec + par * 6 * 64 + src, 0, t, leaf, nrm, pt, valid);
  c.head = (c.head + n) & (kRing - 1);
  c.count -= n;
  c.processed += n;
}
template <bool SMALL, int NPAR, bool EX = false, bool LEAN = false>
PT_DEV void carry_append(Carry<SMALL, NPAR>& c, bool pass, uint32_t leaf, int par, int owner, int lane,
                         const ptd::Node* __restrict__ nodes, const ptd::Geom* __restrict__ geoms, uint32_t gword = 0u) {
  const unsigned long long m = ballot(pass);
  if (!m) return;
  const int rank = rank_in(m);
  if (pass) {
    const int idx = (c.head + c.count + rank) & (kRing - 1);
    c.ent[idx] = (typename Carry<SMALL, NPAR>::Ent)((leaf << 7) | ((uint32_t)par << 6) | (uint32_t)owner);
    if (LEAN) c.gix[idx] = gword;
  }
  const int cnt = __popcll(m);
  c.count += cnt;
  c.appended += cnt;
  if (c.count >= 64) carry_chunk<SMALL, NPAR, EX, LEAN>(c, 64, lane, nodes, geoms);
}
template <bool SUB, int NPAR, bool CAM = false, bool EX = false>
PT_DEV void carry_search(Carry<!SUB, NPAR>& c, const float4* top, int ntop, const ptd::Node* __restrict__ nodes,
                         const ptd::Geom* __restrict__ geoms, f3 o, f3 d, bool valid, int lane, int par, float cull,
                         unsigned long long top_xor) {
  static_assert(CAM == !SUB, "the top-list-only form is the primary kernel's camera ring (Carry<true>: origins not stored); subtree scans take any origin");
  const RayInv ri = Ar<EX>::ray_inv(d, o);
  {
    constexpr int RP = Carry<!SUB, NPAR>::kRayPlanes;
    float* ray = c.ray + par * RP * 64 + lane;
    if (RP == 6) ray[0 * 64] = o.x, ray[1 * 64] = o.y, ray[2 * 64] = o.z;
    ray[(RP - 3) * 64] = d.x, ray[(RP - 2) * 64] = d.y, ray[(RP - 1) * 64] = d.z;
  }
  if (!SUB) {
    uint32_t mask = 0;
    for (int e0 = 0; e0 < ntop; e0 += 8) {
#pragma unroll
      for (int u = 0; u < 8; ++u) {
        const int e = e0 + u;
        if (e < ntop) {
          const float4 A = top[2 * e], B = top[2 * e + 1];
          mask = push_bit(mask, CAM ? Ar<EX>::slab_rel(ri, A.x, A.y, A.z, A.w, B.x, B.y) : Ar<EX>::slab(o, ri, A.x, A.y, A.z, A.w, B.x, B.y));
        }
      }
    }
    mask = valid ? mask : 0u;
    const uint32_t tag = ((uint32_t)par << 6) | (uint32_t)lane;
    while (true) {
      const unsigned long long m = ballot(mask != 0u);
      if (!m) break;
      const int rank = rank_in(m);
      if (mask != 0u) {
        const int te = ntop - 1 - __builtin_ctz(mask);
        mask &= mask - 1u;
        const uint32_t leaf = __float_as_uint(reinterpret_cast<const float*>(top)[8 * te + 6]);
        c.ent[(c.head + c.count + rank) & (kRing - 1)] = (typename Carry<!SUB, NPAR>::Ent)((leaf << 7) | tag);
      }
      const int cnt = __popcll(m);
      c.count += cnt;
      c.appended += cnt;
      if (c.count >= 64) carry_chunk<!SUB, NPAR, EX, false, CAM>(c, 64, lane, nodes, geoms);
    }
    return;
  }
  uint32_t pend = 0;
  PT_STAT(0, 1);
  PT_STAT(13, __popcll(ballot(valid)));
  float4 A = top[0], B = top[1];
  for (int e = 0; e < ntop; ++e) {
    const float4 TA = A, TB = B;
    if (e + 1 < ntop) A = top[2 * e + 2], B = top[2 * e + 3];
    const int t_idx = __builtin_amdgcn_readfirstlane(__float_as_int(TB.z));
    const int t_link = __builtin_amdgcn_readfirstlane(__float_as_int(TB.w));
    const bool pass = valid && slab(o, ri, TA.x, TA.y, TA.z, TA.w, TB.x, TB.y);
    PT_STAT(8, __popcll(ballot(pass)));
    if (t_link < 0) carry_append(c, pass, (uint32_t)t_idx, par, lane, lane, nodes, geoms);
    else if (pass) pend |= 1u << e;
  }
  if constexpr (SUB)
    scan_subtrees(
        pend, top, o, ri, lane, top_xor, cull, c.best + par * 64, c.slot,
        [&](Walker& wk, bool act, float bt, bool& cand, int& at_n, int& aux) {
          if (c.lds_nodes) scan_step(c.lnodes, wk.o, wk.ri, act, wk.cur, bt, cand, at_n, aux);
          else scan_step(reinterpret_cast<const v4f*>(nodes), wk.o, wk.ri, act, wk.cur, bt, cand, at_n, aux);
        },
        [&](bool cand, int at_n, int own, int) { carry_append(c, cand, (uint32_t)at_n, par, own, lane, nodes, geoms); });
}
template <bool SMALL, int NPAR, bool EX = false, bool QO = false>
PT_DEV void carry_drain_to(Carry<SMALL, NPAR>& c, int mark, int lane, const ptd::Node* __restrict__ nodes,
                           const ptd::Geom* __restrict__ geoms) {
  while (c.processed - mark < 0) carry_chunk<SMALL, NPAR, EX, false, QO>(c, min(64, c.count), lane, nodes, geoms);
}

#include "pt_grid.inc"
template <bool EX>
__global__ __launch_bounds__(kBlock) void k_intersect_grid(SceneTables sc, ptd::Queues qs, const int32_t* __restrict__ cnt_in,
                                                           ptd::PathBuf paths, ptd::HitBuf hits) {
  extern __shared__ float4 lds_raw[];
  char* lds = reinterpret_cast<char*>(lds_raw);
  const IntersectGridLds L = intersect_grid_lds<kFast, EX>(sc);
  const ptd::Node* nodes = EX ? sc.nodes : sc.nodes_b;
  const ptd::Geom* geoms = sc.geoms;
  const int wib = threadIdx.x >> 6;
  GridRings ws = grid_rings_init<EX>(lds + L.waves + wib * L.wave_bytes);
  const LeafGeom<true, EX> leaf_geom{nodes, geoms};

  const int wave = blockIdx.x * kWavesPerBlock + wib;
  const int lane = lane_id();
  const auto [q, r, wq] = wave_slot(wave, qs.Q, qs.W);
  const int n_q = cnt_in[cnt_index(qs, 0, q)];
  const int64_t HS = hits.stride;
  const int64_t qbase = (int64_t)q * qs.cap;
  const int last = qs.cap - 64 + lane;
  f3 no, nd;
  path_load_ray(paths, qbase + min(r * 64 + lane, last), no, nd);
  for (int j = r; j * 64 < n_q; j += wq) {
    const int i = j * 64 + lane;
    const bool valid = i < n_q;
    const int64_t at = qbase + i;
    const f3 o = no, d = nd;
    path_load_ray(paths, qbase + min((j + wq) * 64 + lane, last), no, nd);
    ws.cy.best[lane] = kNoHit;
    grid_search<1, EX>(ws.cy, ws.cr, sc, nodes, geoms, o, d, valid, lane, 0);
    while (ws.cy.count > 0) carry_chunk<false, 1, EX, true>(ws.cy, min(64, ws.cy.count), lane, nodes, geoms);
    const Hit h = resolve_hit(ws.cy.best[lane], ws.cy.rec + lane, valid, leaf_geom);
    hits.t[at] = h.t;
    hits.n[at] = h.n.x, hits.n[HS + at] = h.n.y, hits.n[2 * HS + at] = h.n.z;
    hits.mat[at] = h.mat;
    hits.p[at] = h.p.x, hits.p[HS + at] = h.p.y, hits.p[2 * HS + at] = h.p.z;
  }
}
template <Search F, bool SPLIT>
constexpr int primary_waves() {
  return SPLIT && ((PT_ARITH == 2 && F == kTopScan) || (PT_ARITH == 0 && F == kLdsTables)) ? 7 : kPrimaryWaves;
}
template <Search F, bool SHARE = false, bool SPLIT = false>
__global__ __launch_bounds__(kBlock, (primary_waves<F, SPLIT>())) void k_primary(SceneTables sc, ptd::Camera cam, BatchInfo b, ptd::Queues qs,
                                                    int32_t* __restrict__ cnt0, int32_t* __restrict__ cnt_out,
                                                    ptd::PathBuf out, ptd::RetireBuf ret) {
  extern __shared__ float4 lds_raw[];
  char* lds = reinterpret_cast<char*>(lds_raw);
  constexpr bool GRID = F == kGrid, TABLES_IN_LDS = F == kLdsTables, RING = TABLES_IN_LDS;
  const PrimaryLds L = primary_lds<F, kFast, kD0>(sc);
  stage16(lds + L.top, sc.top, GRID ? 0 : top_bytes(sc));
  stage16(lds + L.mats, sc.mats, mat_bytes(sc));
  const ptd::Mat* mats = reinterpret_cast<const ptd::Mat*>(lds + L.mats);
  const ptd::Node* nodes = sc.nodes;
  const ptd::Geom* geoms = sc.geoms;
  if (TABLES_IN_LDS) {
    stage16(lds + L.nodes, sc.nodes, node_bytes(sc));
    stage16(lds + L.geoms, sc.geoms, geom_bytes(sc));
    nodes = reinterpret_cast<const ptd::Node*>(lds + L.nodes);
    geoms = reinterpret_cast<const ptd::Geom*>(lds + L.geoms);
  }
  uint32_t* ihash = reinterpret_cast<uint32_t*>(lds + L.ihash);
  iter_hash_fill(ihash, sc, b, 0);
  float4* cam_top = reinterpret_cast<float4*>(lds + L.cam_top);
  float* cam_qo = reinterpret_cast<float*>(lds + L.cam_qo);
  {
    const f3 cp = mk(cam.pos[0], cam.pos[1], cam.pos[2]);
    for (int e = threadIdx.x; !GRID && e < sc.num_top; e += blockDim.x) {
      const ptd::TopEntry t = sc.top[e];
      cam_top[2 * e] = make_float4(t.bmin[0] - cp.x, t.bmin[1] - cp.y, t.bmin[2] - cp.z, t.bmax[0] - cp.x);
      cam_top[2 * e + 1] = make_float4(t.bmax[1] - cp.y, t.bmax[2] - cp.z, __int_as_float(t.idx), __int_as_float(t.link));
    }
    for (int gi = threadIdx.x; TABLES_IN_LDS && gi < sc.num_geoms; gi += blockDim.x) {
      const f3 q = Ar<kD0>::xf_point(sc.geoms[gi].inv, cp);
      cam_qo[3 * gi] = q.x, cam_qo[3 * gi + 1] = q.y, cam_qo[3 * gi + 2] = q.z;
    }
  }
  __syncthreads();
  const int wib = threadIdx.x >> 6;
  char* wbase = lds + L.waves + wib * L.wave_bytes;
  auto ws = [wbase] {
    if constexpr (RING) return carry_init<true, 2>(wbase);
    else if constexpr (GRID) return grid_rings_init<kD0>(wbase);
    else return wave_lds_init(wbase);
  }();
  const int ntop = sc.num_top;
  const int wave = __builtin_amdgcn_readfirstlane(blockIdx.x * kWavesPerBlock + wib);
  const int lane = lane_id();
  const StrandPlan plan = strand_plan(b.K, b.primary_pieces, qs.deal != nullptr, b.flat != 0);
  for (int strand = wave; strand < qs.W * plan.pieces;) {
    const Strand st = strand_of(strand, plan, b.K, qs.Q, qs.W);
    const int piece = st.piece, q = st.q, r = st.r, wq = st.wq, k0 = st.k0, k1 = st.k1;
    const Retire rt = retire_of(ret, q);
    const QueueShare sh = queue_share(b, qs, q);
    if (piece == 0 && r == 0 && lane == 0) cnt0[cnt_index(qs, 0, q)] = b.K * sh.my_pixels;
    const int64_t qbase = (int64_t)q * qs.cap;
    const float inv_w = 1.0f / (float)cam.res_x;
    const f3 o = mk(cam.pos[0], cam.pos[1], cam.pos[2]);
    int32_t* counter = &cnt_out[cnt_index(qs, 0, q)];
    const int quo = sh.my_nq / wq, rem = sh.my_nq % wq;
    int ck = k0 - 1, crho = strand_rho_before(r, k0, wq), nl = 0, nd = 0;
    auto publish = [&]() {
      if (ck >= k0 && lane == 0) rt.sub[ck * rt.wq0 + crho] = ((unsigned long long)(uint32_t)nd << 32) | (uint32_t)nl;
    };
    auto next_iteration = [&]() {
      publish();
      nl = nd = 0;
      ++ck;
      crho = crho + 1 == wq ? 0 : crho + 1;
    };
    struct Group {
      f3 d;
      int k, pl, slot;
      uint32_t phash;
      int valid;
    };
    auto group_of = [&](int jj, int k) {
      Group g;
      const int pl_raw = chunk_pixel(q, jj, qs.Q) + lane;
      g.valid = pl_raw < b.N;
      g.pl = g.valid ? pl_raw : b.N - 1;
      g.k = k, g.slot = SHARE ? 0 : make_slot(b, k, g.pl);
      const int p = global_pixel(b, g.pl);
      g.phash = utilhash((uint32_t)p);
      float jx = 0.f, jy = 0.f;
      const bool aa = !SHARE && b.aa_jitter != 0;
      if (aa) aa_jitter(b.iter_first + k, p, jx, jy);
      g.d = Ar<kD0>::camera_dir(cam, inv_w, p, aa, jx, jy);
      return g;
    };
    struct {
      Group g;
      int par, mark;
      bool any;
    } pp;
    pp.any = false;
    auto trace = [&](int it, const Group& g, auto&& shade) {
      const bool near_scene = ballot(g.valid && Ar<kD0>::slab(o, Ar<kD0>::ray_inv(g.d, o), sc.root_min[0], sc.root_min[1], sc.root_min[2],
                                                       sc.root_max[0], sc.root_max[1], sc.root_max[2])) != 0;
      if constexpr (RING) {
        const int par = it & 1;
        ws.best[par * 64 + lane] = kNoHit;
        if (near_scene) carry_search<false, 2, true, kD0>(ws, cam_top, ntop, nodes, geoms, o, g.d, g.valid, lane, par, sc.cull_margin, sc.top_xor);
        if (pp.any) {
          carry_drain_to<true, 2, kD0, true>(ws, pp.mark, lane, nodes, geoms);
          shade(ws.best[pp.par * 64 + lane], ws.rec + pp.par * 6 * 64 + lane, pp.g);
        }
        pp.g = g, pp.par = par, pp.mark = ws.appended, pp.any = true;
      } else if constexpr (GRID) {
        ws.cy.best[lane] = kNoHit;
        if (near_scene) {
          grid_search<1, kD0>(ws.cy, ws.cr, sc, nodes, geoms, o, g.d, g.valid, lane, 0);
          while (ws.cy.count > 0) carry_chunk<false, 1, kD0, true>(ws.cy, min(64, ws.cy.count), lane, nodes, geoms);
        }
        shade(ws.cy.best[lane], ws.cy.rec + lane, g);
      } else {
        if (near_scene) trace_group_packet<kD0>(ws, nodes, sc.num_nodes, geoms, o, g.d, g.valid, lane, sc.has_triangles != 0);
        else ws.best[lane] = kNoHit;
        shade(ws.best[lane], ws.rec + lane, g);
      }
    };
    const LeafGeom<GRID, kD0> leaf_geom{nodes, geoms};
    auto shade_group = [&](unsigned long long best, const float* rec, const Group& g) {
      const bool valid = g.valid;
      const int k = g.k, pl = g.pl;
      ShadeIO s;
      s.o = o;
      s.d = g.d;
      s.c = mk(1.0f, 1.0f, 1.0f);
      s.alive = false;
      Bounce bo;
      bo.kind = 0;
      const Hit h = resolve_hit(best, rec, valid, leaf_geom);
      if (valid) bo = shade_decide(mats, b.trace_depth, 0, iter_hash_of(ihash, sc, b, 0, k) ^ g.phash, h.t, h.mat, s);
      const bool alive = valid && s.alive, dead = valid && !s.alive;
      if (alive) shade_bounce(bo, h.n, h.p, s);
      const unsigned long long live = ballot(alive);
      const PathTag tag{g.slot, g.phash, k};
      if (b.flat) {
        int base = 0;
        if (live && lane == 0) base = atomicAdd(counter, (int)__popcll(live));
        base = __builtin_amdgcn_readfirstlane(base);
        if (alive) path_store(out, qbase + base + rank_in(live), s.o, s.d, s.c, tag);
        retire_append(rt, dead, k, pl, s.c);
        return;
      }
      while (ck < k) next_iteration();
      const int sub0 = k * rt.seg_cap + sub_offset(quo, rem, crho) * 64;
      const unsigned long long deadm = ballot(dead);
      if (alive) path_store(out, qbase + sub0 + nl + rank_in(live), s.o, s.d, s.c, tag);
      if (dead) rt.rec[sub0 + nd + rank_in(deadm)] = ptd::Word4{s.c.x, s.c.y, s.c.z, __int_as_float(pl)};
      nl += (int)__popcll(live), nd += (int)__popcll(deadm);
    };
    if constexpr (RING) ws = carry_init<true, 2>(wbase), ws.qo_tab = cam_qo, ws.cam_o = o;
    if constexpr (SHARE) {
      const int cap = shared_run_cap(b.primary_share), sub_off = sub_offset(quo, rem, shared_rho(r, k0, wq)) * 64;
      const bool once = b.retire_once != 0;
      for (int run = 0, runs = shared_runs(k0, k1, cap); run < runs; ++run) {
        const Run sr = shared_run(k0, k1, cap, run);
        const int s0 = sr.k0, s1 = sr.k1;
        int vnl = 0, vnd = 0;
        auto shade_run = [&](unsigned long long best, const float* rec, const Group& g) {
          const bool valid = g.valid;
          const int pl = g.pl;
          const uint32_t phash = g.phash;
          const f3 d = g.d;
          const Hit h = resolve_hit(best, rec, valid, leaf_geom);
          const float ht = h.t;
          const int hmat = h.mat;
          const f3 hn = h.n, hp = h.p;
          if constexpr (SPLIT) {
            if (s0 == 0) {
              const bool lives = valid && !(ht < 0.0f || mats[hmat].emittance > 0.0f);
              const unsigned long long livem = ballot(lives);
              const f3 o1 = bounce_origin(hn, hp);
              if (lives) out.r[out.stride + qbase + sub_off + __builtin_amdgcn_readlane(vnl, 0) + rank_in(livem)] = ptd::Word4{o1.x, o1.y, o1.z, __int_as_float(hmat)};
            }
          }
          const bool cdead = once && valid && (ht < 0.0f || mats[hmat].emittance > 0.0f);
          const unsigned long long cdeadm = once ? ballot(cdead) : 0ull;
          if (once) {
            if (s0 == 0 && cdeadm) {
              ShadeIO s;
              s.o = o;
              s.d = d;
              s.c = mk(1.0f, 1.0f, 1.0f);
              s.alive = false;
              if (cdead) {
                shade_decide(mats, b.trace_depth, 0, iter_hash_of(ihash, sc, b, 0, 0) ^ phash, ht, hmat, s);
                rt.rec[sub_off + __builtin_amdgcn_readlane(vnd, 0) + rank_in(cdeadm)] = ptd::Word4{s.c.x, s.c.y, s.c.z, __int_as_float(pl)};
              }
            }
            if (ballot(valid && !cdead) == 0) {
              if (lane < s1 - s0) vnd += (int)__popcll(cdeadm);
              return;
            }
          }
          for (int k = s0; k < s1; ++k) {
            ShadeIO s;
            s.o = o;
            s.d = d;
            s.c = mk(1.0f, 1.0f, 1.0f);
            s.alive = false;
            Bounce bo;
            bo.kind = 0;
            if (valid) bo = shade_decide(mats, b.trace_depth, 0, iter_hash_of(ihash, sc, b, 0, k) ^ phash, ht, hmat, s);
            const bool alive = valid && s.alive, dead = valid && !s.alive;
            if (alive) shade_bounce(bo, hn, hp, s);
            const unsigned long long live = ballot(alive), deadm = once ? cdeadm : ballot(dead);
            const int nl = __builtin_amdgcn_readlane(vnl, k - s0), nd = __builtin_amdgcn_readlane(vnd, k - s0);
            const int sub0 = k * rt.seg_cap + sub_off;
            const PathTag tag{make_slot(b, k, pl), phash, k};
            if constexpr (SPLIT) {
              if (alive) out.r[qbase + sub0 + nl + rank_in(live)] = ptd::Word4{s.d.x, s.d.y, s.d.z, __uint_as_float(pack_kind(tag.slot, bo.kind == 1))};
            } else if (alive) path_store(out, qbase + sub0 + nl + rank_in(live), s.o, s.d, s.c, tag);
            if (dead && !once) rt.rec[sub0 + nd + rank_in(deadm)] = ptd::Word4{s.c.x, s.c.y, s.c.z, __int_as_float(pl)};
            if (lane == k - s0) vnl += (int)__popcll(live), vnd += (int)__popcll(deadm);
          }
        };
        if constexpr (RING) ws = carry_init<true, 2>(wbase), ws.qo_tab = cam_qo, ws.cam_o = o;
        pp.any = false;
        int it = 0;
        for (int jj = shared_rho(r, s0, wq); jj < sh.my_nq; jj += wq, ++it) trace(it, group_of(jj, 0), shade_run);
        if constexpr (RING) {
          if (pp.any) {
            carry_drain_to<true, 2, kD0, true>(ws, pp.mark, lane, nodes, geoms);
            shade_run(ws.best[pp.par * 64 + lane], ws.rec + pp.par * 6 * 64 + lane, pp.g);
          }
        }
        if (lane < s1 - s0) rt.sub[(s0 + lane) * rt.wq0 + shared_rho(r, s0 + lane, wq)] = ((unsigned long long)(uint32_t)vnd << 32) | (uint32_t)vnl;
      }
    } else {
      int it = 0;
      for (int k = k0, rho = strand_rho(r, k0, wq); k < k1; ++k, rho = rho + 1 == wq ? 0 : rho + 1) {
        for (int jj = rho; jj < sh.my_nq; jj += wq, ++it) trace(it, group_of(jj, k), shade_group);
      }
      if constexpr (RING) {
        if (pp.any) {
          carry_drain_to<true, 2, kD0, true>(ws, pp.mark, lane, nodes, geoms);
          shade_group(ws.best[pp.par * 64 + lane], ws.rec + pp.par * 6 * 64 + lane, pp.g);
        }
      }
      if (!b.flat)
        while (ck < k1) next_iteration();
    }
    if (plan.pieces == 1) break;
    int nx = 0;
    if (lane == 0) nx = atomicAdd(&qs.deal[deal_map(qs).strand_counter()], 1);
    strand = qs.W + __builtin_amdgcn_readfirstlane(nx);
  }
}

constexpr int kPathsWaves = 6;
constexpr int kPathsMinReady = 32;
PT_DEV uint32_t lds_offset(const void* p) { return (uint32_t)(uintptr_t)(__attribute__((address_space(3))) const char*)p; }
template <typename T>
PT_DEV const T* uniform_ptr(const T* p) {
  const uint64_t v = (uint64_t)(uintptr_t)p;
  const uint32_t lo = (uint32_t)__builtin_amdgcn_readfirstlane((int)(uint32_t)v), hi = (uint32_t)__builtin_amdgcn_readfirstlane((int)(uint32_t)(v >> 32));
  return reinterpret_cast<const T*>((uintptr_t)(((uint64_t)hi << 32) | lo));
}
PT_DEV void fetch_record_to_lds(const void* b0, const void* b1, const void* b2, int i, uint32_t lds_base) {
  uint32_t keep;
  const uint32_t off16 = (uint32_t)i << 4, off8 = (uint32_t)i << 3;
  asm volatile(
      "s_mov_b32 %[keep], m0\n\t"
      "s_mov_b32 m0, %[base]\n\t"
      "s_nop 0\n\t"
      "global_load_lds_dwordx4 %[o16], %[b0]\n\t"
      "s_add_u32 m0, m0, 0x400\n\t"
      "s_nop 0\n\t"
      "global_load_lds_dwordx4 %[o16], %[b1]\n\t"
      "s_add_u32 m0, m0, 0x400\n\t"
      "s_nop 0\n\t"
      "global_load_lds_dword %[o8], %[b2]\n\t"
      "s_add_u32 m0, m0, 0xfc\n\t"
      "s_nop 0\n\t"
      "global_load_lds_dword %[o8], %[b2] offset:4\n\t"
      "s_mov_b32 m0, %[keep]"
      : [keep] "=&s"(keep)
      : [base] "s"(lds_base), [b0] "s"(b0), [b1] "s"(b1), [b2] "s"(b2), [o16] "v"(off16), [o8] "v"(off8)
      : "memory", "scc");
}
PT_DEV void fetch_split_to_lds(const void* b0, const void* b1, int i, int i0, uint32_t lds_base) {
  uint32_t keep;
  const uint32_t off = (uint32_t)i << 4, off0 = (uint32_t)i0 << 4;
  asm volatile(
      "s_mov_b32 %[keep], m0\n\t"
      "s_mov_b32 m0, %[base]\n\t"
      "s_nop 0\n\t"
      "global_load_lds_dwordx4 %[o], %[b0]\n\t"
      "s_add_u32 m0, m0, 0x400\n\t"
      "s_nop 0\n\t"
      "global_load_lds_dwordx4 %[o0], %[b1]\n\t"
      "s_mov_b32 m0, %[keep]"
      : [keep] "=&s"(keep)
      : [base] "s"(lds_base), [b0] "s"(b0), [b1] "s"(b1), [o] "v"(off), [o0] "v"(off0)
      : "memory", "scc");
}
struct Lanes {
  unsigned long long* best;
  float* rec;
  uint16_t* ent;
  int head, count;
  int appended, processed;
};
PT_DEV Lanes lanes_init(char* base) {
  Lanes c;
  c.best = reinterpret_cast<unsigned long long*>(base + LanesMap::best);
  c.rec = reinterpret_cast<float*>(base + LanesMap::rec);
  c.ent = reinterpret_cast<uint16_t*>(base + LanesMap::ent);
  c.head = c.count = c.appended = c.processed = 0;
  return c;
}
PT_DEV void paths_chunk(Lanes& c, int n, int lane, f3 o, f3 d, const uint32_t* tword, const ptd::Geom* __restrict__ geoms) {
  const bool valid = lane < n;
  const uint32_t entry = c.ent[(c.head + lane) & (kRing - 1)];
  const int src = (int)(entry & 63u);
  const uint32_t tw = tword[valid ? entry >> 6 : 0u];
  const uint32_t leaf = tw & 255u;
  const f3 ro = mk(bperm(src, o.x), bperm(src, o.y), bperm(src, o.z));
  const f3 rd = mk(bperm(src, d.x), bperm(src, d.y), bperm(src, d.z));
  const ptd::Geom* G = geoms + (valid ? (int)(tw >> 8) : 0);
  f3 pt = mk(0.f, 0.f, 0.f), nrm = mk(0.f, 0.f, 0.f);
  const float t = geom_test<-1, false>(G, ro, rd, pt, nrm, mk(0.f, 0.f, 0.f));
  const uint32_t tb = __float_as_uint(t);
  if (valid && t > 0.f && tb < 0x7f7fffffu) {
    const unsigned long long key = ((unsigned long long)tb << 32) | leaf;
    unsigned long long* slot = &c.best[src];
    atomicMin(slot, key);
    if (*slot == key) {
      float* r = c.rec + src;
      r[0 * 64] = nrm.x, r[1 * 64] = nrm.y, r[2 * 64] = nrm.z;
      r[3 * 64] = pt.x, r[4 * 64] = pt.y, r[5 * 64] = pt.z;
    }
  }
  c.head = (c.head + n) & (kRing - 1);
  c.count -= n;
  c.processed += n;
}
typedef __attribute__((address_space(4))) const v4f cfloat4;
template <typename TOP>
PT_DEV void paths_search(Lanes& c, TOP* top, const uint32_t* tword, int ntop, const ptd::Geom* __restrict__ geoms, f3 o, f3 d,
                         bool fresh, int lane, int& mark) {
  const RayInv ri = ray_inv(d, o);
  if (fresh) {
    c.best[lane] = kNoHit;
    mark = c.processed;
  }
  uint32_t mask = 0;
  for (int e0 = 0; e0 < ntop; e0 += 8) {
#pragma unroll
    for (int u = 0; u < 8; ++u) {
      const int e = e0 + u;
      if (e < ntop) {
        const auto A = top[2 * e], B = top[2 * e + 1];
        mask = push_bit(mask, slab(o, ri, A.x, A.y, A.z, A.w, B.x, B.y));
      }
    }
  }
  mask = fresh ? mask : 0u;
  while (true) {
    const unsigned long long m = ballot(mask != 0u);
    if (!m) break;
    const int rank = rank_in(m);
    if (mask != 0u) {
      const int te = ntop - 1 - __builtin_ctz(mask);
      mask &= mask - 1u;
      c.ent[(c.head + c.count + rank) & (kRing - 1)] = (uint16_t)((te << 6) | lane);
      if (mask == 0u) mark = c.appended + rank + 1;
    }
    const int cnt = __popcll(m);
    c.count += cnt;
    c.appended += cnt;
    if (c.count >= 64) paths_chunk(c, 64, lane, o, d, tword, geoms);
  }
}
constexpr int kPathsScanWaves = 5, kPathsGridWaves = 5;
constexpr int kVisitLap = 32, kVisitsPerRefill = 31;
static_assert(kVisitLap + kVisitsPerRefill + 1 <= kVisitRing, "the visit ring laps a path in flight");
static_assert((kVisitRing & (kVisitRing - 1)) == 0, "visit numbers wrap with a mask");
template <Search MODE, bool SPLIT = false>
__global__ __launch_bounds__(kBlock, MODE == 0 ? kPathsWaves : MODE == 1 ? kPathsScanWaves : kPathsGridWaves) void k_paths(SceneTables sc, BatchInfo b, ptd::Queues qs, int32_t* __restrict__ cnt ,
                                                               ptd::PathBuf in, ptd::RetireBuf ret) {
  extern __shared__ float4 lds_raw[];
  char* lds = reinterpret_cast<char*>(lds_raw);
  const PathsLds L = paths_lds<MODE, kFast>(sc);
  stage16(lds + L.top, sc.top_b, MODE == 2 ? 0 : top_bytes(sc));
  stage16(lds + L.mats, sc.mats, mat_bytes(sc));
  const float4* top = reinterpret_cast<const float4*>(lds + L.top);
  const ptd::Mat* mats = reinterpret_cast<const ptd::Mat*>(lds + L.mats);
  const ptd::Node* nodes = sc.nodes_b;
  const ptd::Geom* geoms = sc.geoms;
  if (MODE == 0) {
    stage16(lds + L.geoms, sc.geoms, geom_bytes(sc));
    geoms = reinterpret_cast<const ptd::Geom*>(lds + L.geoms);
  }
  const char* lnodes = nullptr;
  if (MODE == 1 && sc.scan_nodes_lds > 0) {
    stage16(lds + L.nodes, sc.nodes_b, node_bytes(sc));
    lnodes = lds + L.nodes;
  }
  using WM = PathsWaveMap<MODE, kFast>;
  const int he = iter_hash_entries(sc);
  uint32_t* tword = reinterpret_cast<uint32_t*>(lds + L.tword);
  int* lmat = reinterpret_cast<int*>(lds + L.lmat);
  uint32_t* ihash = reinterpret_cast<uint32_t*>(lds + L.ihash);
  for (int d = 1; d < b.trace_depth; ++d) iter_hash_fill(ihash + (d - 1) * he, sc, b, d);
  for (int e = threadIdx.x; MODE == 0 && e < sc.num_top; e += blockDim.x) {
    const int leaf = sc.top[e].idx, gi = sc.nodes[leaf].geom;
    tword[e] = (uint32_t)leaf | ((uint32_t)gi << 8);
    lmat[leaf & 63] = sc.geoms[gi].material;
  }
  __syncthreads();
  const int wib = threadIdx.x >> 6;
  char* wbase = lds + L.waves + wib * L.wave_bytes;
  Lanes cy = lanes_init(wbase);
  GridRings gr = grid_rings_init<false>(wbase);
  Carry<false, 1>& cb = gr.cy;
  CellRing& cr = gr.cr;
  cb.lnodes = (const __attribute__((address_space(3))) v4f*)(lnodes ? lnodes : lds), cb.lds_nodes = lnodes != nullptr;
  constexpr bool SLOTS = MODE == 0;
  char* slots = wbase + WM::slots;
  int* died = reinterpret_cast<int*>(wbase + WM::died);
  int* fillc = reinterpret_cast<int*>(wbase + WM::fillc);
  const int ntop = sc.num_top;
  const int wave = __builtin_amdgcn_readfirstlane(blockIdx.x * kWavesPerBlock + wib);
  const int lane = lane_id();
  died[lane] = 0;
  const uint64_t t_begin = __builtin_amdgcn_s_memrealtime();
  const DealMap dm = deal_map(qs);
  const WaveSlot even = wave_slot(wave, qs.Q, qs.W);
  int q = even.q, r = even.r, wq = even.wq;
  if (qs.deal != nullptr && qs.deal[dm.made_for()] == qs.W) {
    int at_or_before = 0;
    for (int e0 = 0; e0 < qs.Q; e0 += 64) at_or_before += (int)__popcll(ballot(e0 + lane < qs.Q && qs.deal[dm.first(e0 + lane)] <= wave));
    q = at_or_before - 1;
    const int first = qs.deal[dm.first(q)];
    r = wave - first, wq = qs.deal[dm.first(q + 1)] - first;
  }
  const Retire rt = retire_of(ret, q);
  const int64_t qbase = (int64_t)q * qs.cap;
  const int wq0 = rt.wq0, ne = b.K * wq0;
  const int my_nq = queue_share(b, qs, q).my_nq, quo = my_nq / wq0, rem = my_nq % wq0;
  auto count_of = [&](int e) { return e < ne ? (int)(uint32_t)rt.sub[e] : 0; };
  int total = 0, csum = 0;
  const bool chunk_sums = ne <= 64 * 64;
  for (int e0 = 0; e0 < ne; e0 += 256) {
    int n4[4];
#pragma unroll
    for (int j = 0; j < 4; ++j) n4[j] = count_of(e0 + 64 * j + lane);
#pragma unroll
    for (int j = 0; j < 4; ++j) {
      int sum;
      (void)wave_prefix6(n4[j], sum);
      total += sum;
      if (lane == (e0 >> 6) + j) csum = sum;
    }
  }
  if (r == 0 && lane == 0) cnt[cnt_index(qs, 1, q)] = total;
  const PiecePlan pieces = piece_plan(total, wq, b.paths_pieces, qs.deal != nullptr, chunk_sums);
  [[maybe_unused]] int clist0 = 0;
  int ce = ne, cstart = total, ccnt = 0, clist = 0;
  int cord = 0;
  int win0 = -64;
  unsigned long long wsub = 0ull;
  auto window_to = [&](int e) {
    if (e < win0 || e >= win0 + 64) {
      win0 = e;
      wsub = (e + lane < ne) ? rt.sub[e + lane] : 0ull;
    }
  };
  auto sub_word = [&](int e) -> unsigned long long {
    const uint32_t lo32 = (uint32_t)__builtin_amdgcn_readlane((int)(uint32_t)wsub, e - win0);
    const uint32_t hi32 = (uint32_t)__builtin_amdgcn_readlane((int)(uint32_t)(wsub >> 32), e - win0);
    return ((unsigned long long)hi32 << 32) | lo32;
  };
  window_to(0);
  auto cursor_bases = [&](int first_rank) {
    const int ec = min(ce, ne - 1), ck = ec / wq0, crho = ec - ck * wq0;
    clist = ck * rt.seg_cap + sub_offset(quo, rem, crho) * 64;
    if constexpr (SPLIT) clist0 = invariant_slot(clist, ck, rt.seg_cap);
    window_to(ec);
    const int crec = clist + (int)(uint32_t)(sub_word(ec) >> 32);
    if (lane == 0) fillc[cord & (kVisitRing - 1)] = crec + (first_rank - cstart);
  };
  auto seek = [&](int at_rank) {
    int cum = 0, e_begin = 0;
    if (chunk_sums) {
      int all;
      const int cbefore = wave_prefix6(csum, all);
      const unsigned long long here = ballot(csum > 0 && cbefore <= at_rank && at_rank < cbefore + csum);
      if (here) {
        const int l = __builtin_ctzll(here);
        e_begin = l * 64, cum = __builtin_amdgcn_readlane(cbefore, l);
      }
    }
    for (int e0 = e_begin; e0 < ne; e0 += 64) {
      const int n = count_of(e0 + lane);
      int sum;
      const int before = wave_prefix6(n, sum);
      const unsigned long long here = ballot(n > 0 && cum + before <= at_rank && at_rank < cum + before + n);
      if (here) {
        const int l = __builtin_ctzll(here);
        ce = e0 + l, cstart = cum + __builtin_amdgcn_readlane(before, l), ccnt = __builtin_amdgcn_readlane(n, l);
        break;
      }
      cum += sum;
    }
    ++cord;
    cursor_bases(at_rank);
  };
  auto assign = [&](bool want, int rank, int& at, [[maybe_unused]] int& at0, int& rs) -> bool {
    bool pending = want;
    const int cord0 = cord;
    while (true) {
      const bool in = pending && rank < cstart + ccnt;
      if (in) at = clist + (rank - cstart), rs = cord;
      if constexpr (SPLIT)
        if (in) at0 = clist0 + (rank - cstart);
      pending = pending && !in;
      if (!ballot(pending) || ce >= ne || cord - cord0 >= kVisitsPerRefill) break;
      cstart += ccnt;
      ccnt = 0;
      int nxt = ce + 1;
      while (nxt < ne) {
        window_to(nxt);
        const unsigned long long holds = ballot((uint32_t)wsub != 0u) & (~0ull << (nxt - win0));
        if (holds) {
          nxt = win0 + (int)__builtin_ctzll(holds);
          ccnt = (int)(uint32_t)sub_word(nxt);
          break;
        }
        nxt = win0 + 64;
      }
      ce = min(nxt, ne);
      ++cord;
      cursor_bases(cstart);
    }
    return want && !pending;
  };
  const uint32_t s_base = (uint32_t)__builtin_amdgcn_readfirstlane((int)lds_offset(slots));
  const uint32_t s16 = s_base + (uint32_t)lane * 16u, s4 = s_base + (uint32_t)kSlotTail + (uint32_t)lane * 4u;
  const ptd::Word4 *in0 = uniform_ptr(in.r + qbase), *in1 = uniform_ptr(in.r + in.stride + qbase);
  const float* in2 = uniform_ptr(reinterpret_cast<const float*>(in.r + 2 * in.stride) + 2 * qbase);
  PathRec nx;
  nx.o = nx.d = nx.c = mk(0.f, 0.f, 0.f), nx.tag = PathTag{0, 0u, 0};
  int nx_rs = 0;
  int* slot_rs = reinterpret_cast<int*>(slots + kSlotVisit) + lane;
  auto fetch = [&](int at, [[maybe_unused]] int at0, int rs) {
    if constexpr (SLOTS && SPLIT) fetch_split_to_lds(in0, in1, at, at0, s_base), *slot_rs = rs;
    else if constexpr (SLOTS) fetch_record_to_lds(in0, in1, in2, at, s_base), *slot_rs = rs;
    else if constexpr (SPLIT) {
      const ptd::Word4 w0 = in.r[qbase + at], w1 = in.r[in.stride + qbase + at0];
      nx.o = mk(w0.x, w0.y, w0.z), nx.d = mk(w0.w, w1.x, w1.y), nx.c = mk(w1.z, w1.w, 0.f), nx_rs = rs;
    } else nx = path_load(in, qbase + at), nx_rs = rs;
  };
  f3 o = mk(0.f, 0.f, 0.f), d = o, c = o;
  int slot = 0, depth = 1, mark = 0, rslot = 0;
  uint32_t phash = 0u;
  bool valid = false, fresh = false, owes = false;
  bool has_next = false;
  int streamed = 0, p_hi = 0;
  while (true) {
    if (streamed >= p_hi && p_hi >= 0) {
      int nextp = -1;
      if (cord == 0) nextp = r;
      else if (pieces.needs_counter()) {
        int v = 0;
        if (lane == 0) v = atomicAdd(&qs.deal[dm.piece_counter(q)], 1);
        nextp = wq + __builtin_amdgcn_readfirstlane(v);
      }
      const PieceRange pr = pieces.piece_range(nextp);
      if (pr.some) {
        streamed = pr.start, p_hi = pr.end;
        seek(streamed);
      } else {
        p_hi = -1;
      }
    }
    const bool take = !valid && has_next;
    if (ballot(take || owes || (!valid && !has_next && streamed < p_hi))) {
      v4f w0, w1;
      float cz;
      int nslot, nrs;
      if constexpr (SLOTS && SPLIT) {
        asm volatile(
            "s_waitcnt vmcnt(0)\n\t"
            "ds_read_b128 %0, %3\n\t"
            "ds_read_b128 %1, %3 offset:1024\n\t"
            "ds_read_b32 %2, %4 offset:512\n\t"
            "s_waitcnt lgkmcnt(0)"
            : "=&v"(w0), "=&v"(w1), "=&v"(nrs)
            : "v"(s16), "v"(s4)
            : "memory");
        cz = 0.f, nslot = 0;
      } else if constexpr (SLOTS) {
        asm volatile(
            "s_waitcnt vmcnt(0)\n\t"
            "ds_read_b128 %0, %5\n\t"
            "ds_read_b128 %1, %5 offset:1024\n\t"
            "ds_read_b32 %2, %6\n\t"
            "ds_read_b32 %3, %6 offset:256\n\t"
            "ds_read_b32 %4, %6 offset:512\n\t"
            "s_waitcnt lgkmcnt(0)"
            : "=&v"(w0), "=&v"(w1), "=&v"(cz), "=&v"(nslot), "=&v"(nrs)
            : "v"(s16), "v"(s4)
            : "memory");
      } else {
        w0 = v4f{nx.o.x, nx.o.y, nx.o.z, nx.d.x}, w1 = v4f{nx.d.y, nx.d.z, nx.c.x, nx.c.y}, cz = nx.c.z, nslot = nx.tag.slot, nrs = nx_rs;
      }
      if (owes) {
        rt.rec[rslot] = ptd::Word4{c.x, c.y, c.z, __int_as_float(slot & ((1 << b.slot_shift) - 1))};
        owes = false;
      }
      if constexpr (SPLIT) {
        if (take) {
          const uint32_t word = __float_as_uint(w0.w);
          const ptd::Mat* m = mats + __float_as_int(w1.w);
          nslot = kind_sample_id(word);
          o = mk(w1.x, w1.y, w1.z), d = mk(w0.x, w0.y, w0.z);
          c = mul(mk(1.0f, 1.0f, 1.0f), kind_specular(word) ? mk(m->spec[0], m->spec[1], m->spec[2]) : mk(m->color[0], m->color[1], m->color[2]));
        }
      } else if (take) o = mk(w0.x, w0.y, w0.z), d = mk(w0.w, w1.x, w1.y), c = mk(w1.z, w1.w, cz);
      if (take) {
        slot = nslot, rslot = nrs;
        phash = utilhash((uint32_t)global_pixel(b, nslot & ((1 << b.slot_shift) - 1)));
        depth = 1;
        valid = fresh = true;
        has_next = false;
      }
      const bool lapping = ballot(valid && cord - rslot >= kVisitLap) != 0ull;
      const bool empty = !has_next && !lapping;
      const unsigned long long em = ballot(empty);
      const int rank = rank_in(em);
      const bool more = empty && streamed + rank < p_hi;
      int at = 0, at0 = 0, rs = 0;
      const bool served = assign(more, streamed + rank, at, at0, rs);
      if (served) {
        has_next = true;
        fetch(at, at0, rs);
      }
      streamed += (int)__popcll(ballot(served));
    }
    if (!ballot(valid || has_next) && p_hi < 0) break;
    bool ready;
    if constexpr (MODE == 0) {
      if (ballot(fresh)) {
        if constexpr (kFast) paths_search(cy, (cfloat4*)(uintptr_t)sc.top_b, tword, ntop, geoms, o, d, fresh, lane, mark);
        else paths_search(cy, top, tword, ntop, geoms, o, d, fresh, lane, mark);
      }
      ready = valid && (cy.processed - mark) >= 0;
      if (cy.count > 0 && __popcll(ballot(ready)) < kPathsMinReady) {
        paths_chunk(cy, cy.count, lane, o, d, tword, geoms);
        ready = valid;
      }
    } else {
      cb.best[lane] = kNoHit;
      if constexpr (MODE == 2) grid_search<1>(cb, cr, sc, nodes, geoms, o, d, valid, lane, 0);
      else {
        PT_STAT(14, 1);
        PT_STAT(15, __popcll(ballot(valid)));
        carry_search<true, 1>(cb, top, ntop, nodes, geoms, o, d, valid, lane, 0, sc.cull_margin, sc.top_xor);
      }
      while (cb.count > 0) carry_chunk<false, 1, false, MODE == 2>(cb, min(64, cb.count), lane, nodes, geoms);
      ready = valid;
    }
    fresh = false;
    {
      ShadeIO s;
      s.o = mk(0.f, 0.f, 0.f);
      s.d = d;
      s.c = c;
      s.alive = false;
      Bounce bo;
      bo.kind = 0;
      const int k = (int)((uint32_t)slot >> b.slot_shift);
      const unsigned long long best = cy.best[lane];
      Hit h{false, -1.0f, -1, 0, mk(0.f, 0.f, 0.f), mk(0.f, 0.f, 0.f)};
      if (ready) {
        if ((uint32_t)(best >> 32) != 0x7f7fffffu) {
          h.t = __uint_as_float((uint32_t)(best >> 32));
          const float* rr = cy.rec + lane;
          h.n = mk(rr[0 * 64], rr[1 * 64], rr[2 * 64]);
          h.p = mk(rr[3 * 64], rr[4 * 64], rr[5 * 64]);
          if constexpr (MODE == 0) {
            h.mat = lmat[(uint32_t)best & 63u];
          } else {
            const ptd::Geom* G = geoms + nodes[(uint32_t)best].geom;
            h.mat = G->material;
            if (MODE == 2) h.n = finish_normal(G, h.n);
          }
        }
        const uint32_t ih = he > 0 ? ihash[(depth - 1) * he + k] : iter_hash(b.iter_first + k, depth);
        bo = shade_decide(mats, b.trace_depth, depth, ih ^ phash, h.t, h.mat, s);
      }
      const bool alive = ready && s.alive, dead = ready && !s.alive;
      if (dead) atomicAdd(&died[depth & 63], 1);
      if (dead) rslot = atomicAdd(&fillc[rslot & (kVisitRing - 1)], 1);
      if (alive) shade_bounce(bo, h.n, h.p, s);
      if (ready) {
        c = s.c;
        if (alive) o = s.o, d = s.d, depth += 1, fresh = true;
        else valid = false, owes = true;
      }
    }
  }
  if (lane == 0) {
    int reached = 0, rays = 0;
    for (int dd = min(b.trace_depth - 1, 63); dd >= 2; --dd) {
      reached += died[dd];
      rays += reached;
      if (reached) atomicAdd(&cnt[cnt_index(qs, dd, q)], reached);
    }
    rays += reached + died[1];
    const int ticks = (int)min((uint64_t)(__builtin_amdgcn_s_memrealtime() - t_begin) >> 6, (uint64_t)0x3ffff);
    if (qs.deal != nullptr && rays) atomicAdd(&qs.deal[dm.time(q)], ticks), atomicAdd(&qs.deal[dm.rays(q)], rays);
  }
}

__global__ __launch_bounds__(kBlock) void k_shade_stage(SceneTables sc, int trace_depth, int depth, int n,
                                                        const int32_t* __restrict__ iter,
                                                        const int32_t* __restrict__ pixel, ptd::HitBuf hits,
                                                        ptd::PathBuf paths, int32_t* __restrict__ alive) {
  extern __shared__ float4 lds_raw[];
  char* lds = reinterpret_cast<char*>(lds_raw);
  const ShadeLds L = shade_lds<false>(sc);
  stage16(lds + L.mats, sc.mats, mat_bytes(sc));
  __syncthreads();
  const ptd::Mat* mats = reinterpret_cast<const ptd::Mat*>(lds + L.mats);
  const int64_t HS = hits.stride;
  for (int at = blockIdx.x * blockDim.x + threadIdx.x; at < n; at += gridDim.x * blockDim.x) {
    const PathRec pr = path_load(paths, at);
    ShadeIO s;
    s.o = pr.o;
    s.d = pr.d;
    s.c = pr.c;
    s.alive = false;
    const Bounce bo = shade_decide(mats, trace_depth, depth, iter_hash(iter[at], depth) ^ utilhash((uint32_t)pixel[at]), hits.t[at], hits.mat[at], s);
    if (bo.kind) shade_bounce(bo, mk(hits.n[at], hits.n[HS + at], hits.n[2 * HS + at]),
                              mk(hits.p[at], hits.p[HS + at], hits.p[2 * HS + at]), s);
    path_store(paths, at, s.o, s.d, s.c, pr.tag);
    alive[at] = s.alive ? 1 : 0;
  }
}

#include "pt_features.inc"
#include "pt_output.inc"
#include "pt_launch.inc"
const KernelApi kApi = {
#if PT_ARITH == 0
    "exact",
#elif PT_ARITH == 1
    "fma",
#else
    "fast",
#endif
    launch_generate, launch_primary, launch_intersect, launch_shade, launch_collect, launch_count_stats,
    launch_preview, launch_save_u8, launch_shade_stage, lds_table_limit, resident_blocks_per_cu, launch_ieee_check, launch_paths,
    launch_collect_conv, launch_features, kFast ? 1 : 0, launch_intersect_grid};

}
}

const KernelApi* PT_API_FN() { return &PT_NS::kApi; }

#if defined(PT_WALK_STATS) && PT_ARITH == 2
}
extern "C" int pt_debug_walk_stats(unsigned long long* out) {
  unsigned long long zero[16] = {0};
  if (hipDeviceSynchronize() != hipSuccess) return -1;
  if (hipMemcpyFromSymbol(out, HIP_SYMBOL(ptk::arith_fast::g_walk_stats), sizeof(zero)) != hipSuccess) return -1;
  if (hipMemcpyToSymbol(HIP_SYMBOL(ptk::arith_fast::g_walk_stats), zero, sizeof(zero)) != hipSuccess) return -1;
  return 16;
}
namespace ptk {
#endif

}
```

cosc_4397_pathtracing_raytracing_project_amd/csrc/pt_launch.inc:

```
template <bool EX, typename F>
void with_intersect_of(const SceneTables& sc, bool legacy, F&& f) {
  const bool in_lds = tables_in_lds(sc);
  if (legacy) in_lds ? f(k_intersect_legacy<true, EX>, legacy_lds<true>(sc).total) : f(k_intersect_legacy<false, EX>, legacy_lds<false>(sc).total);
  else in_lds ? f(k_intersect<true, EX>, intersect_lds<true>(sc).total) : f(k_intersect<false, EX>, intersect_lds<false>(sc).total);
}
template <typename F>
void with_intersect(const SceneTables& sc, bool legacy, bool exact, F&& f) {
  exact ? with_intersect_of<kD0>(sc, legacy, f) : with_intersect_of<false>(sc, legacy, f);
}
template <typename F>
void with_intersect_grid(const SceneTables& sc, bool primary, F&& f) {
  primary ? f(k_intersect_grid<kD0>, intersect_grid_lds<kFast, kD0>(sc).total) : f(k_intersect_grid<false>, intersect_grid_lds<kFast, false>(sc).total);
}
bool leaves_fit_top(const SceneTables& sc) { return (sc.num_nodes + 1) / 2 <= kMaxTop; }
template <typename F>
void with_features(const SceneTables& sc, F&& f) {
  if (tables_in_lds(sc)) return f(k_features<true, false>, intersect_lds<true>(sc).total);
  if (leaves_fit_top(sc)) return f(k_features<false, false>, intersect_lds<false>(sc).total);
  return f(k_features<false, true>, intersect_lds<false>(sc).total);
}
template <Search S, typename F>
void with_primary_of(const SceneTables& sc, bool share, bool split, F&& f) {
  const int lds = primary_lds<S, kFast, kD0>(sc).total;
  return !share ? f(k_primary<S>, lds) : split ? f(k_primary<S, true, true>, lds) : f(k_primary<S, true>, lds);
}
template <typename F>
void with_primary(const SceneTables& sc, bool share, bool split, F&& f) {
  switch (search_form(sc)) {
    case kLdsTables: return with_primary_of<kLdsTables>(sc, share, split, f);
    case kTopScan: return with_primary_of<kTopScan>(sc, share, split, f);
    case kGrid: return with_primary_of<kGrid>(sc, share, split, f);
  }
}

template <typename F>
void with_paths(const SceneTables& sc, Search form, bool split, F&& f) {
  switch (form) {
    case kLdsTables: return split ? f(k_paths<kLdsTables, true>, paths_lds<kLdsTables, kFast>(sc).total) : f(k_paths<kLdsTables>, paths_lds<kLdsTables, kFast>(sc).total);
    case kTopScan: return split ? f(k_paths<kTopScan, true>, paths_lds<kTopScan, kFast>(sc).total) : f(k_paths<kTopScan>, paths_lds<kTopScan, kFast>(sc).total);
    case kGrid: return split ? f(k_paths<kGrid, true>, paths_lds<kGrid, kFast>(sc).total) : f(k_paths<kGrid>, paths_lds<kGrid, kFast>(sc).total);
  }
}
int paths_lds_bytes(const SceneTables& sc, Search form) {
  int bytes = 0;
  with_paths(sc, form, false, [&](auto, int lds) { bytes = lds; });
  return bytes;
}
int lds_share_limit(int bytes);
SceneTables resolve_scan_nodes(const SceneTables& sc_in) {
  SceneTables sc = sc_in;
  if (iter_hash_entries(sc) > 0) {
    SceneTables without = sc;
    without.max_batch_iters = kIterHashMax + 1;
    const Search form = search_form(sc);
    const int reg_waves = form == kLdsTables ? kPathsWaves : form == kTopScan ? kPathsScanWaves : kPathsGridWaves;
    SceneTables a = sc, b = without;
    if (a.scan_nodes_lds < 0) a.scan_nodes_lds = b.scan_nodes_lds = 0;
    const bool costs = min(lds_share_limit(paths_lds_bytes(b, form)), reg_waves) > min(lds_share_limit(paths_lds_bytes(a, form)), reg_waves);
    if (costs) sc = without;
  }
  SceneTables t = sc;
  if (t.scan_nodes_lds >= 0) return t;
  SceneTables with = sc, without = sc;
  with.scan_nodes_lds = 1, without.scan_nodes_lds = 0;
  const int bw = paths_lds_bytes(with, kTopScan), bo = paths_lds_bytes(without, kTopScan);
  t.scan_nodes_lds = (bw <= 64 * 1024 && lds_share_limit(bw) >= min(lds_share_limit(bo), kPathsScanWaves)) ? 1 : 0;
  return t;
}
auto occupancy_into(int& n, int fallback) {
  return [&n, fallback](auto kernel, int lds) {
    if (hipOccupancyMaxActiveBlocksPerMultiprocessor(&n, kernel, kBlock, lds) != hipSuccess) n = fallback;
  };
}
int lds_table_limit(const SceneTables& sc, int forced_bytes) {
  if (forced_bytes >= 0) return leaves_fit_top(sc) ? forced_bytes : -1;
  const int tbl = table_bytes(sc);
  int with = 0, without = 0;
  if (tbl <= kLdsTableBytes && leaves_fit_top(sc)) {
    SceneTables in = sc;
    in.lds_table_bytes = tbl;
    with_paths(in, kLdsTables, false, occupancy_into(with, 0));
  }
  with_paths(sc, kTopScan, false, occupancy_into(without, 1));
  (void)hipGetLastError();
  return (with >= without && with > 0) ? tbl : -1;
}

constexpr int kLdsGranule = 1280;
int lds_share_limit(int bytes) { return bytes > 0 ? (160 * 1024) / (((bytes + kLdsGranule - 1) / kLdsGranule) * kLdsGranule) : 8; }
int resident_blocks_per_cu(KernelId id, const SceneTables& sc) {
  int n = 0, m = 0, lds = 0;
  const auto query = occupancy_into(n, 1);
  const auto query_share = [&](auto kernel, int bytes) { query(kernel, bytes), lds = bytes; };
  switch (id) {
    case kGenerate: query(k_generate, 0); break;
    case kIntersect: with_intersect(sc, false, false, query); break;
    case kIntersectLegacy: with_intersect(sc, true, false, query); break;
    case kPrimary: with_primary(sc, false, false, query_share); break;
    case kPrimaryShared: with_primary(sc, true, false, query_share), m = n, with_primary(sc, true, true, query_share), n = min(n, m); break;
    case kPaths: with_paths(resolve_scan_nodes(sc), search_form(sc), false, query_share), m = n, with_paths(resolve_scan_nodes(sc), search_form(sc), true, query_share), n = min(n, m); break;
    case kShade: query(k_shade, shade_lds<true>(sc).total); break;
    case kFeatures: with_features(sc, query); break;
  }
  if (n < 1) n = 1;
  n = min(n, max(1, lds_share_limit(lds)));
  return n > 8 ? 8 : n;
}

void launch_generate(hipStream_t s, int grid, const ptd::Camera& cam, const BatchInfo& b, const ptd::Queues& qs,
                     ptd::PathBuf out, int32_t* cnt0) {
  hipLaunchKernelGGL(k_generate, dim3(grid), dim3(kBlock), 0, s, cam, b, qs, out, cnt0);
}

void launch_intersect(hipStream_t s, int grid, const SceneTables& sc, const ptd::Queues& qs, const int32_t* cnt_in,
                      ptd::PathBuf paths, ptd::HitBuf hits, bool legacy, bool exact_arith) {
  with_intersect(sc, legacy, exact_arith, [&](auto kernel, int lds) { hipLaunchKernelGGL(kernel, dim3(grid), dim3(kBlock), lds, s, sc, qs, cnt_in, paths, hits); });
}

void launch_intersect_grid(hipStream_t s, int grid, const SceneTables& sc, const ptd::Queues& qs, const int32_t* cnt_in,
                           ptd::PathBuf paths, ptd::HitBuf hits, bool primary) {
  with_intersect_grid(sc, primary, [&](auto kernel, int lds) { hipLaunchKernelGGL(kernel, dim3(grid), dim3(kBlock), lds, s, sc, qs, cnt_in, paths, hits); });
}

void launch_primary(hipStream_t s, int grid, const SceneTables& sc, const ptd::Camera& cam, const BatchInfo& b,
                    const ptd::Queues& qs, int32_t* cnt0, int32_t* cnt_out, ptd::PathBuf out, ptd::RetireBuf ret) {
  with_primary(sc, primary_shares(b), primary_shares(b) && b.split_records != 0, [&](auto kernel, int lds) { hipLaunchKernelGGL(kernel, dim3(grid), dim3(kBlock), lds, s, sc, cam, b, qs, cnt0, cnt_out, out, ret); });
}

void launch_features(hipStream_t s, int grid, const SceneTables& sc, const ptd::Camera& cam, const BatchInfo& b, float4* feat) {
  with_features(sc, [&](auto kernel, int lds) {
    if (lds > 64 * 1024) (void)hipFuncSetAttribute(reinterpret_cast<const void*>(kernel), hipFuncAttributeMaxDynamicSharedMemorySize, lds);
    hipLaunchKernelGGL(kernel, dim3(grid), dim3(kBlock), lds, s, sc, cam, b, feat);
  });
}

void launch_paths(hipStream_t s, int grid, const SceneTables& sc_in, const BatchInfo& b, const ptd::Queues& qs, int32_t* cnt, ptd::PathBuf in, ptd::RetireBuf ret) {
  const SceneTables sc = resolve_scan_nodes(sc_in);
  with_paths(sc, search_form(sc), b.split_records != 0, [&](auto kernel, int lds) { hipLaunchKernelGGL(kernel, dim3(grid), dim3(kBlock), lds, s, sc, b, qs, cnt, in, ret); });
}
void launch_shade(hipStream_t s, int grid, const SceneTables& sc, const BatchInfo& b, int depth, const ptd::Queues& qs,
                  const int32_t* cnt_in, int32_t* cnt_out, ptd::PathBuf in, ptd::HitBuf hits, ptd::PathBuf out,
                  ptd::RetireBuf ret) {
  hipLaunchKernelGGL(k_shade, dim3(grid), dim3(kBlock), shade_lds<true>(sc).total, s, sc, b, depth, qs, cnt_in, cnt_out, in, hits, out,
                     ret);
}

int flat_grid(int n, int cap) {
  int grid = (n + kBlock - 1) / kBlock;
  return grid > cap ? cap : (grid < 1 ? 1 : grid);
}
void launch_collect(hipStream_t s, const BatchInfo& b, const ptd::Queues& qs, ptd::RetireBuf ret, float* image_rgb) {
  (void)hipFuncSetAttribute(reinterpret_cast<const void*>(k_collect), hipFuncAttributeMaxDynamicSharedMemorySize, collect_lds_bytes(ret.wq0));
  hipLaunchKernelGGL(k_collect, dim3(qs.Q), dim3(kCollectThreads), collect_lds_bytes(ret.wq0), s, b, qs, ret, image_rgb);
}
void launch_collect_conv(hipStream_t s, const BatchInfo& b, const ptd::Queues& qs, ptd::RetireBuf ret, float* image_rgb, const ConvInfo& cv, double* sse) {
  (void)hipFuncSetAttribute(reinterpret_cast<const void*>(k_collect_conv), hipFuncAttributeMaxDynamicSharedMemorySize, collect_lds_bytes(ret.wq0));
  hipLaunchKernelGGL(k_collect_conv, dim3(qs.Q), dim3(kCollectThreads), collect_lds_bytes(ret.wq0), s, b, qs, ret, image_rgb, cv);
  if (cv.first_k < b.K) hipLaunchKernelGGL(k_conv_reduce, dim3(b.K - cv.first_k), dim3(kBlock), 0, s, b.iter_first, cv.first_k, qs.Q * kCollectWaves, cv.partial, sse);
}

#include "pt_ieee_check.inc"

void launch_count_stats(hipStream_t s, const ptd::Queues& qs, int32_t* cnt, int depth_count,
                        unsigned long long* stats) {
  hipLaunchKernelGGL(k_count_stats, dim3(depth_count + 2), dim3(kBlock), 0, s, qs, cnt, depth_count, stats);
}

void launch_preview(hipStream_t s, int n, int iterations, const float* image_rgb, uchar4* rgba) {
  hipLaunchKernelGGL(k_preview, dim3(flat_grid(n, 4096)), dim3(kBlock), 0, s, n, iterations, image_rgb, rgba);
}

void launch_save_u8(hipStream_t s, int n, int width, float samples, const float* image_rgb, uint8_t* rgb8) {
  hipLaunchKernelGGL(k_save_u8, dim3(flat_grid(n, 4096)), dim3(kBlock), 0, s, n, width, samples, image_rgb, rgb8);
}

void launch_shade_stage(hipStream_t s, const SceneTables& sc, int trace_depth, int depth, int n, const int32_t* iter,
                        const int32_t* pixel, ptd::HitBuf hits, ptd::PathBuf paths, int32_t* alive) {
  hipLaunchKernelGGL(k_shade_stage, dim3(flat_grid(n, 2048)), dim3(kBlock), shade_lds<false>(sc).total, s, sc, trace_depth, depth, n, iter, pixel, hits,
                     paths, alive);
}
```

cosc_4397_pathtracing_raytracing_project_amd/csrc/pt_sched.h:

```cpp
#pragma once
#include "pt_kernels.h"

#define PT_SCHED __host__ __device__ inline __attribute__((always_inline))

namespace ptk {

PT_SCHED int sched_min(int a, int b) { return a < b ? a : b; }
PT_SCHED int sched_max(int a, int b) { return a > b ? a : b; }

struct DealMap {
  int Q;
  PT_SCHED int first(int q) const { return q; }
  PT_SCHED int made_for() const { return Q; }
  PT_SCHED int time(int q) const { return Q + 1 + q; }
  PT_SCHED int strand_counter() const { return 2 * Q + 1; }
  PT_SCHED int piece_counter(int q) const { return 2 * Q + 2 + q; }
  PT_SCHED int rays(int q) const { return 3 * Q + 2 + q; }
  PT_SCHED int words() const { return 4 * Q + 2; }
};
PT_SCHED DealMap deal_map(const ptd::Queues& qs) { return DealMap{qs.Q}; }

PT_SCHED int dealt_first(int q, int W, int Q, unsigned long long work_before, unsigned long long work_total) {
  return q + (int)((unsigned long long)(W - Q) * work_before / work_total);
}
PT_SCHED bool queues_close_together(int heaviest_rays, unsigned long long total_rays, int W, int Q) {
  return (unsigned long long)heaviest_rays * W * Q <= total_rays * ((unsigned long long)W + Q);
}

struct WaveSlot {
  int q, r, wq;
};
PT_SCHED WaveSlot wave_slot(int wave, int Q, int W) { return WaveSlot{wave % Q, wave / Q, W / Q}; }

struct QueueShare {
  int my_nq;
  int my_pixels;
  float inv_my_nq;
};
PT_SCHED QueueShare queue_share(const BatchInfo& b, const ptd::Queues& qs, int q) {
  const int chunks = (b.N + 63) >> 6;
  QueueShare sh;
  sh.my_nq = q < chunks ? (chunks - q + qs.Q - 1) / qs.Q : 0;
  const int last_q = (chunks - 1) % qs.Q;
  sh.my_pixels = sh.my_nq * 64 - ((q == last_q && (b.N & 63)) ? 64 - (b.N & 63) : 0);
  sh.inv_my_nq = sh.my_nq > 0 ? 1.0f / (float)sh.my_nq : 0.0f;
  return sh;
}
PT_SCHED int chunk_pixel(int q, int jj, int Q) { return (q + jj * Q) * 64; }
PT_SCHED int slot_pixel(int q, int li, int Q) { return chunk_pixel(q, li >> 6, Q) + (li & 63); }

PT_SCHED int sub_chunks(int quo, int rem, int rho) { return quo + (rho < rem ? 1 : 0); }
PT_SCHED int sub_offset(int quo, int rem, int rho) { return rho * quo + sched_min(rho, rem); }
struct Gap {
  int g0, g1;
};
PT_SCHED Gap region_gap(const QueueShare& sh, int wq0) {
  Gap g{0, 0};
  const int missing = sh.my_nq * 64 - sh.my_pixels;
  if (missing > 0) {
    const int quo = sh.my_nq / wq0, rem = sh.my_nq % wq0, rho = (sh.my_nq - 1) % wq0;
    g.g1 = (sub_offset(quo, rem, rho) + sub_chunks(quo, rem, rho)) * 64;
    g.g0 = g.g1 - missing;
  }
  return g;
}

PT_SCHED size_t cnt_index(const ptd::Queues& qs, int d, int q) { return (size_t)qs.Q * qs.cnt_stride * d + (size_t)q * qs.cnt_stride; }

struct QueuePlan {
  int nq, seg_cap, cap;
};
PT_SCHED int chunks_per_queue(int64_t N, int Q) { return (int)(((N + 63) / 64 + Q - 1) / Q); }
PT_SCHED QueuePlan queue_plan(int64_t N, int Q, int K) {
  QueuePlan p;
  p.nq = chunks_per_queue(N, Q);
  p.seg_cap = p.nq * 64;
  p.cap = K * p.seg_cap;
  return p;
}
PT_SCHED size_t sub_stride(int widest_grid_waves, int Q) { return (size_t)widest_grid_waves / Q; }

struct StrandPlan {
  int kp, pieces;
};
PT_SCHED StrandPlan strand_plan(int K, int primary_pieces, bool deal_present, bool flat) {
  StrandPlan p;
  p.kp = primary_pieces > 1 && deal_present && !flat ? (K + primary_pieces - 1) / primary_pieces : K;
  p.pieces = (K + p.kp - 1) / p.kp;
  return p;
}
struct Strand {
  int piece, q, r, wq, k0, k1;
};
PT_SCHED Strand strand_of(int strand, const StrandPlan& p, int K, int Q, int W) {
  Strand s;
  s.piece = strand / W;
  const WaveSlot w = wave_slot(strand - s.piece * W, Q, W);
  s.q = w.q, s.r = w.r, s.wq = w.wq;
  s.k0 = s.piece * p.kp, s.k1 = sched_min(K, s.k0 + p.kp);
  return s;
}
PT_SCHED int strand_rho(int r, int k, int wq) { return (r + k) % wq; }
PT_SCHED int strand_rho_before(int r, int k, int wq) { return (r + k + wq - 1) % wq; }
PT_SCHED int auto_primary_pieces(int K, int nq, int wq0) {
  const int64_t want = (int64_t)K * nq / sched_max(1, wq0) / 48;
  return want < 1 ? 1 : want > 4 ? 4 : (int)want;
}

constexpr int kShareMax = 64;
PT_SCHED bool primary_shares(int primary_share, bool aa_jitter, bool flat) { return primary_share > 1 && !aa_jitter && !flat; }
PT_SCHED bool primary_shares(const BatchInfo& b) { return primary_shares(b.primary_share, b.aa_jitter != 0, b.flat != 0); }
PT_SCHED int shared_rho(int r, int , int ) { return r; }
PT_SCHED int shared_run_cap(int primary_share) { return primary_share < 1 ? 1 : sched_min(primary_share, kShareMax); }
struct Run {
  int k0, k1;
};
PT_SCHED int shared_runs(int k0, int k1, int cap) { return (k1 - k0 + cap - 1) / cap; }
PT_SCHED Run shared_run(int k0, int k1, int cap, int i) { return Run{k0 + i * cap, sched_min(k1, k0 + (i + 1) * cap)}; }
PT_SCHED int auto_shared_pieces(int K, int , int ) {
  const int want = sched_max(2, (K + kShareMax - 1) / kShareMax);
  return sched_max(1, sched_min(want, K));
}

constexpr int kRetireEveryIteration = 1024;
PT_SCHED bool retires_once(int primary_share, bool aa_jitter, bool flat, int trace_depth, int debug_flags) {
  return primary_shares(primary_share, aa_jitter, flat) && trace_depth >= 2 && !(debug_flags & kRetireEveryIteration);
}
PT_SCHED bool retires_once(const BatchInfo& b, int debug_flags) {
  return retires_once(b.primary_share, b.aa_jitter != 0, b.flat != 0, b.trace_depth, debug_flags);
}
struct SubSlot {
  int rho, pos;
};
PT_SCHED SubSlot sub_slot(int quo, int rem, int i) {
  const int c = i >> 6, big = rem * (quo + 1);
  const int rho = c < big ? c / (quo + 1) : rem + (c - big) / sched_max(quo, 1);
  return SubSlot{rho, i - sub_offset(quo, rem, rho) * 64};
}
PT_SCHED bool retiree_slot(const SubSlot& s, int retirees) { return s.pos < retirees; }

constexpr int kWholeRecords = 4096;
PT_SCHED bool splits_records(int primary_share, bool aa_jitter, bool flat, int trace_depth, int debug_flags) {
  return primary_shares(primary_share, aa_jitter, flat) && trace_depth >= 2 && !(debug_flags & kWholeRecords);
}
PT_SCHED bool splits_records(const BatchInfo& b, int debug_flags) {
  return splits_records(b.primary_share, b.aa_jitter != 0, b.flat != 0, b.trace_depth, debug_flags);
}
PT_SCHED int invariant_slot(int at, int k, int seg_cap) { return at - k * seg_cap; }
PT_SCHED uint32_t pack_kind(int sample_id, bool specular) { return (uint32_t)sample_id | (specular ? 0x80000000u : 0u); }
PT_SCHED int kind_sample_id(uint32_t word) { return (int)(word & 0x7fffffffu); }
PT_SCHED bool kind_specular(uint32_t word) { return (word >> 31) != 0u; }

PT_SCHED int pack_paths_pieces(int count, int min_piece) { return count | min_piece << 16; }
PT_SCHED int paths_pieces_count(int word) { return word & 0xffff; }
PT_SCHED int paths_pieces_min(int word) { return word >> 16; }
struct PieceRange {
  int start, end;
  bool some;
};
struct PiecePlan {
  int total, wq, pieces_per_wave, ps_min, ps0;
  PT_SCHED bool needs_counter() const { return ps0 * wq < total; }
  PT_SCHED PieceRange piece_range(int nextp) const {
    int start = total, sz = ps0;
    if (nextp >= 0) {
      start = 0;
      int level = nextp / wq;
      const int idx = nextp - level * wq;
      for (; level > 0 && start < total; --level) start += wq * sz, sz = sched_max(sz - sz / pieces_per_wave, ps_min);
      start += idx * sz;
    }
    return start < total ? PieceRange{start, sched_min(start + sz, total), true} : PieceRange{total, total, false};
  }
};
PT_SCHED PiecePlan piece_plan(int total, int wq, int paths_pieces, bool deal_present, bool chunk_sums) {
  PiecePlan p;
  p.total = total, p.wq = wq;
  p.pieces_per_wave = deal_present && chunk_sums && paths_pieces_count(paths_pieces) > 1 ? paths_pieces_count(paths_pieces) : 1;
  p.ps_min = paths_pieces_min(paths_pieces);
  p.ps0 = sched_max((total + wq * p.pieces_per_wave - 1) / (wq * p.pieces_per_wave), p.ps_min);
  return p;
}

}
```

cosc_4397_pathtracing_raytracing_project_amd/csrc/pt_shade.inc:

```
PT_DEV void local_frame(f3 n, f3& tangent, f3& bitangent) {
  const bool a = __builtin_fabsf(n.x) > __builtin_fabsf(n.y);
  tangent = normalize(a ? mk(n.z, 0.f, -n.x) : mk(0.f, -n.z, n.y));
  bitangent = cross(n, tangent);
}
PT_DEV f3 sky_factor(f3 dir) {
  const float t = 0.5f * (dir.y + 1.0f);
  const float w = (1.0f - t) * 1.0f;
  return scl(mk(w + t * 0.5f, w + t * 0.7f, w + t * 1.0f), 0.5f);
}

struct ShadeIO {
  f3 o, d, c;
  bool alive;
};
struct Bounce {
  uint32_t rng_x;
  int kind;
  float roughness;
};
PT_DEV Bounce shade_decide(const ptd::Mat* __restrict__ mats, int trace_depth, int depth, uint32_t seed, float ht, int hmat,
                           ShadeIO& s) {
  Bounce bo;
  bo.kind = 0;
  bo.rng_x = 1u;
  bo.roughness = 0.f;
  s.alive = false;
  if (ht < 0.0f) {
    const f3 sky = sky_factor(s.d);
    for (int k = depth; k < trace_depth; ++k) s.c = mul(s.c, sky);
    return bo;
  }
  MinStd rng(seed);
  const ptd::Mat* m = mats + hmat;
  const f3 mcolor = mk(m->color[0], m->color[1], m->color[2]);
  if (m->emittance > 0.0f) {
    s.c = mul(s.c, scl(mcolor, m->emittance));
    return bo;
  }
  if (depth > 3) {
    const float q = __builtin_fmaxf(mcolor.x, __builtin_fmaxf(mcolor.y, mcolor.z));
    if (rng.u01() > q) return bo;
    if (kFast) s.c = scl(s.c, __builtin_amdgcn_rcpf(q));
    else ieee::div3(s.c.x, s.c.y, s.c.z, q);
  }
  const float reflectivity = m->reflective;
  bo.roughness = 1.0f - m->refractive;
  if (reflectivity > 0.0f && rng.u01() < reflectivity) {
    bo.kind = 1;
    s.c = mul(s.c, mk(m->spec[0], m->spec[1], m->spec[2]));
  } else {
    bo.kind = 2;
    s.c = mul(s.c, mcolor);
  }
  bo.rng_x = rng.x;
  s.alive = (depth + 1) < trace_depth;
  return bo;
}
PT_DEV f3 bounce_origin(f3 hn, f3 hp) {
  if (kFast || kFloatTrig) return madd(hn, 0.001f, hp);
  return add(hp, scl(hn, 0.001f));
}
template <bool HW>
PT_DEV void shade_bounce_float(const Bounce& bo, f3 hn, f3 hp, ShadeIO& s) {
  MinStd rng(1u);
  rng.x = bo.rng_x;
  const bool spec = bo.kind == 1;
  const float r1 = rng.u01(), r2 = rng.u01(), r3 = rng.u01();
  const f3 refl = madd(hn, -2.0f * dot(s.d, hn), s.d);
  const f3 f = spec ? refl : hn;
  const float rev = bo.roughness * r1 * 0.25f;
  const float ct = HW ? __builtin_amdgcn_sqrtf(1.0f - r1) : __builtin_sqrtf(1.0f - r1);
  const float st2 = __builtin_fmaxf(fma_(-ct, ct, 1.0f), 0.0f);
  const float st = HW ? __builtin_amdgcn_sqrtf(st2) : __builtin_sqrtf(st2);
  float sA = 0.0f, cA = 1.0f, c1, s2;
  if (HW) {
    sA = __builtin_amdgcn_sinf(rev), cA = __builtin_amdgcn_cosf(rev);
    c1 = __builtin_amdgcn_cosf(r2);
    s2 = __builtin_amdgcn_sinf(spec ? r3 : r2);
  } else {
    ptmath::sincos_rev(r2, &s2, &c1);
    if (ballot(spec)) {
      float s3, c3;
      ptmath::sincos_rev(rev, &sA, &cA);
      ptmath::sincos_rev(r3, &s3, &c3);
      s2 = spec ? s3 : s2;
    }
  }
  const float sX = spec ? sA : st;
  const float cX = spec ? cA : ct;
  const float x = sX * c1, z = sX * s2, y = cX;
  f3 tangent, bitangent;
  local_frame(f, tangent, bitangent);
  const f3 pert = normalize(madd(tangent, x, madd(f, y, scl(bitangent, z))));
  const bool perturb = !spec || bo.roughness > 0.0f;
  s.o = bounce_origin(hn, hp);
  s.d = perturb ? pert : refl;
}
PT_DEV void shade_bounce(const Bounce& bo, f3 hn, f3 hp, ShadeIO& s) {
  if (kFast) return shade_bounce_float<true>(bo, hn, hp, s);
  if (kFloatTrig) return shade_bounce_float<false>(bo, hn, hp, s);
  const double kPi = 3.14159265358979323846;
  MinStd rng(1u);
  rng.x = bo.rng_x;
  const bool spec = bo.kind == 1;
  const float r1 = rng.u01(), r2 = rng.u01(), r3 = rng.u01();
  const f3 refl = sub(s.d, scl(hn, 2.0f * dot(s.d, hn)));
  const f3 f = spec ? refl : hn;
  const float angle = (float)((double)(bo.roughness * r1) * kPi * (double)0.5f);
  const float theta = ptmath::acosf32(__builtin_sqrtf(1.0f - r1));
  const float phi = (float)((double)2.0f * kPi * (double)r2);
  const float X = spec ? angle : theta;
  const double Y1 = spec ? (double)2.0f * kPi * (double)r2 : (double)phi;
  const double Y2 = spec ? (double)2.0f * kPi * (double)r3 : (double)phi;
  float sX, cX;
  ptmath::sincosf32(X, &sX, &cX);
  const float c1 = ptmath::cos_r(Y1);
  const float s2 = ptmath::sin_r(Y2);
  const float x = sX * c1;
  const float z = sX * s2;
  const float y = cX;
  f3 tangent, bitangent;
  local_frame(f, tangent, bitangent);
  const f3 pert = normalize(add(add(scl(tangent, x), scl(f, y)), scl(bitangent, z)));
  const bool perturb = !spec || bo.roughness > 0.0f;
  s.o = bounce_origin(hn, hp);
  s.d = perturb ? pert : refl;
}


__global__ __launch_bounds__(kBlock) void k_shade(SceneTables sc, BatchInfo b, int depth, ptd::Queues qs,
                                                  const int32_t* __restrict__ cnt_in, int32_t* __restrict__ cnt_out,
                                                  ptd::PathBuf in, ptd::HitBuf hits, ptd::PathBuf out,
                                                  ptd::RetireBuf ret) {
  extern __shared__ float4 lds_raw[];
  char* lds = reinterpret_cast<char*>(lds_raw);
  const ShadeLds L = shade_lds<true>(sc);
  stage16(lds + L.mats, sc.mats, mat_bytes(sc));
  uint32_t* ihash = reinterpret_cast<uint32_t*>(lds + L.ihash);
  iter_hash_fill(ihash, sc, b, depth);
  __syncthreads();
  const ptd::Mat* mats = reinterpret_cast<const ptd::Mat*>(lds + L.mats);

  const int wave = blockIdx.x * kWavesPerBlock + (threadIdx.x >> 6);
  const int lane = lane_id();
  const auto [q, r, wq] = wave_slot(wave, qs.Q, qs.W);
  const Retire rt = retire_of(ret, q);
  const int n_q = cnt_in[cnt_index(qs, 0, q)];
  const int64_t HS = hits.stride;
  const int64_t qbase = (int64_t)q * qs.cap;
  struct In {
    PathTag tag;
    int hmat;
    float ht;
    f3 hn, hp, d, c;
  };
  const int last = qs.cap - 64 + lane;
  auto load = [&](int i) {
    In v;
    const int64_t at = qbase + min(i, last);
    v.ht = hits.t[at];
    v.hn = mk(hits.n[at], hits.n[HS + at], hits.n[2 * HS + at]);
    v.hmat = hits.mat[at];
    v.hp = mk(hits.p[at], hits.p[HS + at], hits.p[2 * HS + at]);
    path_load_tail(in, at, v.d, v.c, v.tag);
    return v;
  };
  In nx = load(r * 64 + lane);
  for (int j = r; j * 64 < n_q; j += wq) {
    const int i = j * 64 + lane;
    const bool valid = i < n_q;
    const In cur = nx;
    nx = load((j + wq) * 64 + lane);
    ShadeIO s;
    s.o = mk(0.f, 0.f, 0.f);
    s.d = cur.d;
    s.c = cur.c;
    s.alive = false;
    Bounce bo;
    bo.kind = 0;
    int k, pl;
    sample_of(cur.tag, b, k, pl);
    if (valid) bo = shade_decide(mats, b.trace_depth, depth, path_seed(k, pl, ihash, sc, b, depth), cur.ht, cur.hmat, s);
    retire_append(rt, valid && !s.alive, k, pl, s.c);
    const bool alive = valid && s.alive;
    const unsigned long long live = ballot(alive);
    int base = 0;
    if (live && lane == 0) base = atomicAdd(&cnt_out[cnt_index(qs, 0, q)], (int)__popcll(live));
    if (alive) shade_bounce(bo, cur.hn, cur.hp, s);
    if (live) {
      base = __builtin_amdgcn_readfirstlane(base);
      if (alive) path_store(out, qbase + base + rank_in(live), s.o, s.d, s.c, cur.tag);
    }
  }
}
```

include/pt_amd.h:

```cpp
#ifndef PT_AMD_H
#define PT_AMD_H

#include <stdint.h>

#ifdef __cplusplus
extern "C" {
#endif

#define PT_GEOM_SPHERE 0
#define PT_GEOM_CUBE 1
#define PT_GEOM_TRIANGLE 2

typedef struct PtGeom {
  int32_t type;
  int32_t materialid;
  float transform[16];
  float inverseTransform[16];
  float invTranspose[16];
} PtGeom;

typedef struct PtMaterial {
  float color[3];
  float specular_exponent;
  float specular_color[3];
  float hasReflective;
  float hasRefractive;
  float indexOfRefraction;
  float emittance;
} PtMaterial;

typedef struct PtCamera {
  int32_t resolution[2];
  float position[3];
  float lookAt[3];
  float view[3];
  float up[3];
  float right[3];
  float fov[2];
  float pixelLength[2];
} PtCamera;

typedef struct PtBVHNode {
  float bmin[3];
  float bmax[3];
  int32_t left, right, geomIndex;
} PtBVHNode;

typedef struct PtSceneDesc {
  const PtGeom* geoms;
  int32_t num_geoms;
  const PtMaterial* materials;
  int32_t num_materials;
  PtCamera camera;
  int32_t trace_depth;
} PtSceneDesc;

typedef struct PtOptions {
  int32_t device;
  int32_t pixel_begin;
  int32_t pixel_count;
  int32_t iters_per_batch;
  int32_t num_queues;
  int32_t blocks_per_cu;
  int32_t time_kernels;
  int32_t legacy_traversal;
  int32_t debug_flags;
  int32_t unfused_primary;
  int32_t unfused_bounces;
  int32_t stripe_pixels;
  int32_t stripe_stride;
  int32_t arith;
  int32_t aa_jitter;
  int32_t convergence;
  int32_t lds_table_kb;
  int32_t primary_pieces;
  int32_t paths_pieces;
  int32_t paths_min_piece;
} PtOptions;
#define PT_PRIMARY_PIECES(pieces, share) ((int32_t)((pieces) | (share) << 16))

#define PT_ARITH_EXACT 0
#define PT_ARITH_FMA 1
#define PT_ARITH_FAST 2

#define PT_MAX_DEPTH 64
typedef struct PtStats {
  int64_t samples;
  int64_t live_rays[PT_MAX_DEPTH];
  int64_t intersect_launches;
  double intersect_ms;
  double render_ms;
  int32_t num_cus, grid_blocks, num_queues, iters_per_batch;
  int64_t device_bytes;
  int32_t primary_fused;
  int32_t bounces_fused;
  int32_t arith;
  int32_t grid_cells;
  int32_t tight_leaves;
  int32_t paths_waves;
} PtStats;

typedef struct PtScene PtScene;
int pt_scene_load(const char* path, int res_w, int res_h, PtScene** out);
void pt_scene_free(PtScene* s);
int pt_scene_desc(const PtScene* s, PtSceneDesc* out);
int pt_scene_iterations(const PtScene* s);
const char* pt_scene_image_name(const PtScene* s);

int pt_build_bvh(const PtGeom* geoms, int num_geoms, PtBVHNode* out, int cap);

typedef struct PtGridInfo {
  int32_t res[3];
  float origin[3], cell_size[3], pad;
  int32_t num_cells, num_records, num_leaves;
} PtGridInfo;
typedef struct PtGridRecord {
  float bmin[3], bmax[3];
  int32_t leaf;
  int32_t neighbours;
} PtGridRecord;
int pt_build_grid(const PtGeom* geoms, int num_geoms, int forced, PtGridInfo* info, uint32_t* cell_start, PtGridRecord* records);

int pt_traversal_boxes(const PtGeom* geoms, int num_geoms, const float camera_position[3], float* boxes);

void pt_center_half_box(const float lo[3], const float hi[3], int inner, float magnitude, float center[3], float half_extent[3]);

int pt_build_transform(const float* trs, float* transform, float* inverse, float* invTranspose);

int pt_init(const PtSceneDesc* scene, const PtOptions* opt);
int pt_free(void);
int pt_render(int iter_first, int iter_count);
int pt_sync(void);
int pt_readback(float* rgb_sum_host);
int pt_readback_device(void* rgb_sum_dev);
int pt_preview_rgba8(int iterations, uint8_t* rgba_host);
int pt_preview_rgba8_device(int iterations, void* rgba_dev);
int pt_get_stats(PtStats* out);
int pt_reset_stats(void);
int pt_clear(void);
const char* pt_last_error(void);
int pt_selfcheck_ieee(int arith, int kind, uint64_t first, uint64_t count, uint32_t seed, uint64_t* mismatches);
#define PT_CONVERGENCE_WAVES 16
#define PT_CONVERGENCE_CAPACITY 65536
int pt_set_reference(const float* rgb_avg_host);
int pt_get_convergence(int iter_first, int iter_count, double* sse);
int pt_iterations_to_clean(float threshold_db, int* iteration);
float pt_psnr_from_sse(double sse, int64_t pixels);

#define PT_FEATURE_PLANES 3
int pt_render_features(int iter_first, int iter_count);
int pt_readback_features(float* planes_host);

typedef struct PtDenoiseOptions {
  int32_t levels;
  float sigma_color;
  float sigma_normal;
  float sigma_position;
  int32_t keep_albedo;
} PtDenoiseOptions;
int pt_denoise(float samples, const PtDenoiseOptions* opt, float* rgb_avg_host);
int pt_denoise_host(int w, int rows, const float* rgb_sum, const float* planes, float samples, const PtDenoiseOptions* opt, float* rgb_avg);

#define PT_NOISE_PLANES 2
#define PT_NOISE_PIXELS_PER_PARTIAL 1024
int pt_noise_fold(void);
int pt_get_noise(double* sse, int* groups, int* iterations);
int pt_readback_noise(float* planes_host);
int pt_render_until(int iter_first, int max_iters, int group_iters, float target_db, int* iters_done, float* psnr_db);
int pt_noise_fold_host(int pixels, const float* rgb_sum, float* planes, int group_iters, int groups_after, int64_t iters_after, double* sse);

#define PT_DENOISE_VARIANCE_FLOOR 1e-8f
int pt_denoise_guided(const PtDenoiseOptions* opt, float* rgb_avg_host);
int pt_denoise_guided_host(int w, int rows, const float* rgb_sum, const float* planes, const float* noise_planes, int groups, int64_t iters,
                           const PtDenoiseOptions* opt, float* rgb_avg);
int pt_denoise_guided_variance_host(int w, int rows, const float* rgb_sum, const float* planes, const float* noise_planes, int groups, int64_t iters,
                                    const PtDenoiseOptions* opt, float* var_raw, float* var_0);

int pt_adaptive_round(int iter_first, int group_iters, float fraction);
int pt_render_adaptive(int iter_first, int max_iters, int group_iters, float fraction, float target_db, int* iters_done, int64_t* samples_done,
                       float* psnr_db);
int pt_readback_adaptive(int32_t* counts);
int pt_resolve(float* rgb_avg_host);
int pt_adaptive_select_host(int w, int rows, const float* noise_planes, const int32_t* counts, int m, int32_t* list);
int pt_adaptive_merge_host(int pixels, float* rgb_sum, float* planes, int32_t* counts, const int32_t* list, int m, const float* group_sum,
                           int group_iters, double* sse);

int pt_denoise_adaptive(const PtDenoiseOptions* opt, float* rgb_avg_host);
int pt_denoise_adaptive_host(int w, int rows, const float* rgb_sum, const float* planes, const float* noise_planes, const int32_t* counts,
                             const PtDenoiseOptions* opt, float* rgb_avg);
int pt_denoise_adaptive_variance_host(int w, int rows, const float* rgb_sum, const float* planes, const float* noise_planes, const int32_t* counts,
                                      const PtDenoiseOptions* opt, float* var_raw, float* var_0);

int pt_save_u8(float samples, uint8_t* rgb8_host);

typedef struct PtContext PtContext;
int pt_ctx_create(const PtSceneDesc* scene, const PtOptions* opt, PtContext** out);
int pt_ctx_destroy(PtContext* c);
int pt_ctx_render(PtContext* c, int iter_first, int iter_count);
int pt_ctx_sync(PtContext* c);
int pt_ctx_readback(PtContext* c, float* rgb_sum_host);
int pt_ctx_readback_device(PtContext* c, void* rgb_sum_dev);
int pt_ctx_save_u8(PtContext* c, float samples, uint8_t* rgb8_host);
int pt_ctx_save_u8_device(PtContext* c, float samples, const uint8_t** rgb8_dev);
int pt_ctx_preview_rgba8(PtContext* c, int iterations, uint8_t* rgba_host);
int pt_ctx_preview_rgba8_device(PtContext* c, int iterations, void* rgba_dev);
int pt_ctx_get_stats(PtContext* c, PtStats* out);
int pt_ctx_reset_stats(PtContext* c);
int pt_ctx_clear(PtContext* c);
int pt_ctx_set_reference(PtContext* c, const float* rgb_avg_host);
int pt_ctx_get_convergence(PtContext* c, int iter_first, int iter_count, double* sse);
int pt_ctx_iterations_to_clean(PtContext* c, float threshold_db, int* iteration);
int pt_ctx_render_features(PtContext* c, int iter_first, int iter_count);
int pt_ctx_readback_features(PtContext* c, float* planes_host);
int pt_ctx_denoise(PtContext* c, float samples, const PtDenoiseOptions* opt, float* rgb_avg_host);
int pt_ctx_denoise_device(PtContext* c, float samples, const PtDenoiseOptions* opt, const float** rgb_dev);
int pt_ctx_denoise_guided(PtContext* c, const PtDenoiseOptions* opt, float* rgb_avg_host);
int pt_ctx_denoise_guided_device(PtContext* c, const PtDenoiseOptions* opt, const float** rgb_dev);
int pt_ctx_denoise_adaptive(PtContext* c, const PtDenoiseOptions* opt, float* rgb_avg_host);
int pt_ctx_denoise_adaptive_device(PtContext* c, const PtDenoiseOptions* opt, const float** rgb_dev);
int pt_ctx_noise_fold(PtContext* c);
int pt_ctx_get_noise(PtContext* c, double* sse, int* groups, int* iterations);
int pt_ctx_readback_noise(PtContext* c, float* planes_host);
int pt_ctx_render_until(PtContext* c, int iter_first, int max_iters, int group_iters, float target_db, int* iters_done, float* psnr_db);
int pt_ctx_adaptive_round(PtContext* c, int iter_first, int group_iters, float fraction);
int pt_ctx_render_adaptive(PtContext* c, int iter_first, int max_iters, int group_iters, float fraction, float target_db, int* iters_done,
                           int64_t* samples_done, float* psnr_db);
int pt_ctx_readback_adaptive(PtContext* c, int32_t* counts);
int pt_ctx_resolve(PtContext* c, float* rgb_avg_host);
int pt_ctx_resolve_device(PtContext* c, const float** rgb_dev);
const float* pt_ctx_device_noise(PtContext* c);
const float* pt_ctx_device_features(PtContext* c);
const float* pt_ctx_device_image(PtContext* c);
void* pt_ctx_stream(PtContext* c);
int pt_ctx_pixel_count(const PtContext* c);
int pt_ctx_device(const PtContext* c);

typedef struct PtGroup PtGroup;
#define PT_GROUP_TRANSPORT_AUTO 0
#define PT_GROUP_TRANSPORT_RCCL 1
#define PT_GROUP_TRANSPORT_COPY 2
int pt_group_create_ex(const PtSceneDesc* scene, const PtOptions* base, const int* devices, int num_devices, int transport,
                       PtGroup** out);
int pt_group_transport(const PtGroup* g);
int pt_group_create(const PtSceneDesc* scene, const PtOptions* base, const int* devices, int num_devices, PtGroup** out);
int pt_group_destroy(PtGroup* g);
int pt_group_size(const PtGroup* g);
PtContext* pt_group_context(PtGroup* g, int i);
int pt_group_render(PtGroup* g, int iter_first, int iter_count);
int pt_group_sync(PtGroup* g);
int pt_group_gather(PtGroup* g, float* rgb_sum_host);
int pt_group_gather_u8(PtGroup* g, float samples, uint8_t* rgb8_host);
int pt_group_render_features(PtGroup* g, int iter_first, int iter_count);
int pt_group_gather_features(PtGroup* g, float* planes_host);
int pt_group_denoise(PtGroup* g, float samples, const PtDenoiseOptions* opt, float* rgb_avg_host);
int pt_group_denoise_guided(PtGroup* g, const PtDenoiseOptions* opt, float* rgb_avg_host);
int pt_group_noise_fold(PtGroup* g);
int pt_group_get_noise(PtGroup* g, double* sse, int* groups, int* iterations);
int pt_group_render_until(PtGroup* g, int iter_first, int max_iters, int group_iters, float target_db, int* iters_done, float* psnr_db);
int pt_group_preview_rgba8(PtGroup* g, int iterations, uint8_t* rgba_host);

int pt_group_set_reference(PtGroup* g, const float* rgb_avg_host);
int pt_group_get_convergence(PtGroup* g, int iter_first, int iter_count, double* sse);
int pt_group_iterations_to_clean(PtGroup* g, float threshold_db, int* iteration);

int pt_stage_generate(int pix_begin, int n, float* origin, float* dir);
int pt_stage_intersect(int n, const float* origin, const float* dir, float* t, float* normal, int32_t* material,
                       float* point);
int pt_stage_intersect_grid(int n, const float* origin, const float* dir, int primary_form, float* t, float* normal,
                            int32_t* material, float* point);
int pt_stage_grid_info(PtGridInfo* info, int32_t* max_cell_records);
int pt_stage_shade(int n, int depth, const int32_t* iter, const int32_t* pixel, const float* t, const float* normal,
                   const int32_t* material, const float* point, float* origin, float* dir, float* color,
                   int32_t* alive);

int pt_stage_save_u8(int w, int h, float samples, const float* rgb_sum, uint8_t* rgb8);

int pt_stage_denoise(int w, int rows, const float* rgb_sum, const float* planes, float samples, const PtDenoiseOptions* opt, float* rgb_avg);
int pt_stage_denoise_guided(int w, int rows, const float* rgb_sum, const float* planes, const float* noise_planes, int groups, int64_t iters,
                            const PtDenoiseOptions* opt, float* rgb_avg);

int pt_stage_denoise_adaptive(int w, int rows, const float* rgb_sum, const float* planes, const float* noise_planes, const int32_t* counts,
                              const PtDenoiseOptions* opt, float* rgb_avg);
int pt_stage_adaptive_select(int w, int rows, const float* noise_planes, const int32_t* counts, int m, int32_t* list);
int pt_stage_render_list(const int32_t* list, int m, int iter_first, int iter_count, float* rgb_sum_host);

int pt_save_png(const char* path, const float* rgb_sum, int w, int h, float samples);
int pt_write_png_rgb8(const char* path, const uint8_t* rgb8, int w, int h);
int pt_output_basename(const char* name, int samples, char* out, int cap);
int pt_save_pfm(const char* path, const float* rgb_sum, int w, int h, float samples);
int pt_load_pfm(const char* path, float* rgb_sum, int cap_pixels, int* w, int* h, float samples);
int pt_save_hdr(const char* path, const float* rgb_sum, int w, int h, float samples);

#ifdef __cplusplus
}
#endif
#endif
```

Before: 35870.

## Defer first-bounce shading from primary kernel into paths kernel via compact hit records

Adds a third record form (first-bounce) in which the shared primary kernel writes only hit origin, normal, camera direction and a packed pixel/material word for surviving camera rays. Shading of the first bounce, meaning the material decision, throughput and bounce direction sampling, moves into the paths kernel's LDS-table refill path. The aim is to make primary-pass records smaller and to overlap first-bounce shading with traversal in the persistent paths loop. It only applies to the LDS-table search form, single-piece primary, and K/material counts that fit the packed bits, and it adds new template instantiations plus a separate loop in k_paths.

Result: faster. 39360 (median of 6 runs) (+9.7%).

```diff
diff --git a/cosc_4397_pathtracing_raytracing_project_amd/capi.py b/cosc_4397_pathtracing_raytracing_project_amd/capi.py
--- a/cosc_4397_pathtracing_raytracing_project_amd/capi.py
+++ b/cosc_4397_pathtracing_raytracing_project_amd/capi.py
@@ -68,7 +68,7 @@
                 ("intersect_ms", C.c_double), ("render_ms", C.c_double), ("num_cus", C.c_int32),
                 ("grid_blocks", C.c_int32), ("num_queues", C.c_int32), ("iters_per_batch", C.c_int32),
                 ("device_bytes", C.c_int64), ("primary_fused", C.c_int32), ("bounces_fused", C.c_int32),
-                ("arith", C.c_int32), ("grid_cells", C.c_int32), ("tight_leaves", C.c_int32), ("paths_waves", C.c_int32)]
+                ("arith", C.c_int32), ("grid_cells", C.c_int32), ("tight_leaves", C.c_int32), ("paths_waves", C.c_int32), ("record_form", C.c_int32)]
 
 
 class PtDenoiseOptions(C.Structure):
diff --git a/cosc_4397_pathtracing_raytracing_project_amd/csrc/pt_api.cpp b/cosc_4397_pathtracing_raytracing_project_amd/csrc/pt_api.cpp
--- a/cosc_4397_pathtracing_raytracing_project_amd/csrc/pt_api.cpp
+++ b/cosc_4397_pathtracing_raytracing_project_amd/csrc/pt_api.cpp
@@ -6,13 +6,14 @@
 
 #include "pt_adaptive.h"
 #include "pt_context.h"
+#include "pt_lds.h"
 #include "pt_scene.h"
 #include "pt_sched.h"
 
 namespace {
 
 std::string g_err;
-constexpr int kDebugFlags = 16 | 32 | 64 | 128 | 256 | 512 | ptk::kRetireEveryIteration | 2048 | ptk::kWholeRecords;
+constexpr int kDebugFlags = 16 | 32 | 64 | 128 | 256 | 512 | ptk::kRetireEveryIteration | 2048 | ptk::kWholeRecords | ptk::kNoFirstBounce;
 static_assert(sizeof(PtOptions) == 80, "capi.PtOptions mirrors this layout");
 static_assert(PT_CONVERGENCE_WAVES == ptk::kConvWaves, "pt_amd.h documents the size of the convergence metric's partial sums");
 }
@@ -118,11 +119,13 @@
   b.primary_pieces = g.primary_pieces ? g.primary_pieces
                      : ptk::primary_shares(b) ? ptk::auto_shared_pieces(kb, g.qs.nq, g.ret.wq0) : ptk::auto_primary_pieces(kb, g.qs.nq, g.ret.wq0);
   b.paths_pieces = g.paths_pieces;
+  const ptk::SceneTables sc = tables(g);
   b.retire_once = ptk::retires_once(b, g.debug_flags) ? 1 : 0;
-  b.split_records = ptk::splits_records(b, g.debug_flags) ? 1 : 0;
+  b.split_records = ptk::record_form(b, g.debug_flags, ptk::search_form(sc), sc.num_mats);
+  if (b.split_records == ptk::kFirstBounce) b.primary_pieces = 1;
+  g.record_form = b.split_records;
   b.list = g.list;
   if (b.list) b.stripe = 1, b.gap = 0, b.inv_stripe = 1.0f;
-  const ptk::SceneTables sc = tables(g);
   const ptk::KernelApi& k = *g.k;
   auto cnt_row = [&](int d) { return g.d_cnt + ptk::cnt_index(g.qs, d, 0); };
   int d0 = 0;
@@ -726,6 +729,7 @@
     out->grid_cells = res[0] * res[1] * res[2];
   }
   out->tight_leaves = g.tight_leaves;
+  out->record_form = g.record_form;
   out->paths_waves = 0;
   if (g.qs.deal && g.grid_paths > 0) {
     const ptk::DealMap dm = ptk::deal_map(g.qs);
diff --git a/cosc_4397_pathtracing_raytracing_project_amd/csrc/pt_context.h b/cosc_4397_pathtracing_raytracing_project_amd/csrc/pt_context.h
--- a/cosc_4397_pathtracing_raytracing_project_amd/csrc/pt_context.h
+++ b/cosc_4397_pathtracing_raytracing_project_amd/csrc/pt_context.h
@@ -52,6 +52,7 @@
   int cap_bpc = 8;
   bool legacy = false;
   int debug_flags = 0;
+  int record_form = 0;
   bool fuse_primary = true, fuse_bounces = true;
   bool aa_jitter = false;
 };
diff --git a/cosc_4397_pathtracing_raytracing_project_amd/csrc/pt_kernels.hip b/cosc_4397_pathtracing_raytracing_project_amd/csrc/pt_kernels.hip
--- a/cosc_4397_pathtracing_raytracing_project_amd/csrc/pt_kernels.hip
+++ b/cosc_4397_pathtracing_raytracing_project_amd/csrc/pt_kernels.hip
@@ -899,11 +899,11 @@
     hits.p[at] = h.p.x, hits.p[HS + at] = h.p.y, hits.p[2 * HS + at] = h.p.z;
   }
 }
-template <Search F, bool SPLIT>
+template <Search F, int SPLIT>
 constexpr int primary_waves() {
-  return SPLIT && ((PT_ARITH == 2 && F == kTopScan) || (PT_ARITH == 0 && F == kLdsTables)) ? 7 : kPrimaryWaves;
-}
-template <Search F, bool SHARE = false, bool SPLIT = false>
+  return SPLIT == kSplitRecords && ((PT_ARITH == 2 && F == kTopScan) || (PT_ARITH == 0 && F == kLdsTables)) ? 7 : kPrimaryWaves;
+}
+template <Search F, bool SHARE = false, int SPLIT = 0>
 __global__ __launch_bounds__(kBlock, (primary_waves<F, SPLIT>())) void k_primary(SceneTables sc, ptd::Camera cam, BatchInfo b, ptd::Queues qs,
                                                     int32_t* __restrict__ cnt0, int32_t* __restrict__ cnt_out,
                                                     ptd::PathBuf out, ptd::RetireBuf ret) {
@@ -1055,7 +1055,37 @@
       nl += (int)__popcll(live), nd += (int)__popcll(deadm);
     };
     if constexpr (RING) ws = carry_init<true, 2>(wbase), ws.qo_tab = cam_qo, ws.cam_o = o;
-    if constexpr (SHARE) {
+    if constexpr (SHARE && SPLIT == kFirstBounce) {
+      const int sub_off = sub_offset(quo, rem, shared_rho(r, 0, wq)) * 64;
+      int fnl = 0, fnd = 0;
+      auto record_group = [&](unsigned long long best, const float* rec, const Group& g) {
+        const bool valid = g.valid;
+        const Hit h = resolve_hit(best, rec, valid, leaf_geom);
+        const bool cdead = valid && (h.t < 0.0f || mats[h.mat].emittance > 0.0f), lives = valid && !cdead;
+        const unsigned long long livem = ballot(lives), cdeadm = ballot(cdead);
+        if (lives) path_store(out, qbase + sub_off + fnl + rank_in(livem), bounce_origin(h.n, h.p), h.n, g.d, PathTag{pack_first(g.pl, h.mat, b.slot_shift), g.phash, 0});
+        if (cdead) {
+          ShadeIO s;
+          s.o = o;
+          s.d = g.d;
+          s.c = mk(1.0f, 1.0f, 1.0f);
+          s.alive = false;
+          shade_decide(mats, b.trace_depth, 0, iter_hash_of(ihash, sc, b, 0, 0) ^ g.phash, h.t, h.mat, s);
+          rt.rec[sub_off + fnd + rank_in(cdeadm)] = ptd::Word4{s.c.x, s.c.y, s.c.z, __int_as_float(g.pl)};
+        }
+        fnl += (int)__popcll(livem), fnd += (int)__popcll(cdeadm);
+      };
+      pp.any = false;
+      int it = 0;
+      for (int jj = shared_rho(r, 0, wq); jj < sh.my_nq; jj += wq, ++it) trace(it, group_of(jj, 0), record_group);
+      if constexpr (RING) {
+        if (pp.any) {
+          carry_drain_to<true, 2, kD0, true>(ws, pp.mark, lane, nodes, geoms);
+          record_group(ws.best[pp.par * 64 + lane], ws.rec + pp.par * 6 * 64 + lane, pp.g);
+        }
+      }
+      for (int k = lane; k < b.K; k += 64) rt.sub[k * rt.wq0 + shared_rho(r, k, wq)] = ((unsigned long long)(uint32_t)fnd << 32) | (uint32_t)fnl;
+    } else if constexpr (SHARE) {
       const int cap = shared_run_cap(b.primary_share), sub_off = sub_offset(quo, rem, shared_rho(r, k0, wq)) * 64;
       const bool once = b.retire_once != 0;
       for (int run = 0, runs = shared_runs(k0, k1, cap); run < runs; ++run) {
@@ -1071,7 +1101,7 @@
           const float ht = h.t;
           const int hmat = h.mat;
           const f3 hn = h.n, hp = h.p;
-          if constexpr (SPLIT) {
+          if constexpr (SPLIT == kSplitRecords) {
             if (s0 == 0) {
               const bool lives = valid && !(ht < 0.0f || mats[hmat].emittance > 0.0f);
               const unsigned long long livem = ballot(lives);
@@ -1113,7 +1143,7 @@
             const int nl = __builtin_amdgcn_readlane(vnl, k - s0), nd = __builtin_amdgcn_readlane(vnd, k - s0);
             const int sub0 = k * rt.seg_cap + sub_off;
             const PathTag tag{make_slot(b, k, pl), phash, k};
-            if constexpr (SPLIT) {
+            if constexpr (SPLIT == kSplitRecords) {
               if (alive) out.r[qbase + sub0 + nl + rank_in(live)] = ptd::Word4{s.d.x, s.d.y, s.d.z, __uint_as_float(pack_kind(tag.slot, bo.kind == 1))};
             } else if (alive) path_store(out, qbase + sub0 + nl + rank_in(live), s.o, s.d, s.c, tag);
             if (dead && !once) rt.rec[sub0 + nd + rank_in(deadm)] = ptd::Word4{s.c.x, s.c.y, s.c.z, __int_as_float(pl)};
@@ -1200,6 +1230,19 @@
       : [base] "s"(lds_base), [b0] "s"(b0), [b1] "s"(b1), [o] "v"(off), [o0] "v"(off0)
       : "memory", "scc");
 }
+PT_DEV void read_record_slot(uint32_t s16, uint32_t s4, v4f& w0, v4f& w1, float& cz, int& nslot, int& nrs) {
+  asm volatile(
+      "s_waitcnt vmcnt(0)\n\t"
+      "ds_read_b128 %0, %5\n\t"
+      "ds_read_b128 %1, %5 offset:1024\n\t"
+      "ds_read_b32 %2, %6\n\t"
+      "ds_read_b32 %3, %6 offset:256\n\t"
+      "ds_read_b32 %4, %6 offset:512\n\t"
+      "s_waitcnt lgkmcnt(0)"
+      : "=&v"(w0), "=&v"(w1), "=&v"(cz), "=&v"(nslot), "=&v"(nrs)
+      : "v"(s16), "v"(s4)
+      : "memory");
+}
 struct Lanes {
   unsigned long long* best;
   float* rec;
@@ -1282,7 +1325,7 @@
 constexpr int kVisitLap = 32, kVisitsPerRefill = 31;
 static_assert(kVisitLap + kVisitsPerRefill + 1 <= kVisitRing, "the visit ring laps a path in flight");
 static_assert((kVisitRing & (kVisitRing - 1)) == 0, "visit numbers wrap with a mask");
-template <Search MODE, bool SPLIT = false>
+template <Search MODE, int SPLIT = 0>
 __global__ __launch_bounds__(kBlock, MODE == 0 ? kPathsWaves : MODE == 1 ? kPathsScanWaves : kPathsGridWaves) void k_paths(SceneTables sc, BatchInfo b, ptd::Queues qs, int32_t* __restrict__ cnt ,
                                                                ptd::PathBuf in, ptd::RetireBuf ret) {
   extern __shared__ float4 lds_raw[];
@@ -1365,6 +1408,8 @@
   [[maybe_unused]] int clist0 = 0;
   int ce = ne, cstart = total, ccnt = 0, clist = 0;
   int cord = 0;
+  [[maybe_unused]] int cur_k = 0;
+  [[maybe_unused]] uint32_t cur_h = 0u, next_h = 0u;
   int win0 = -64;
   unsigned long long wsub = 0ull;
   auto window_to = [&](int e) {
@@ -1382,7 +1427,8 @@
   auto cursor_bases = [&](int first_rank) {
     const int ec = min(ce, ne - 1), ck = ec / wq0, crho = ec - ck * wq0;
     clist = ck * rt.seg_cap + sub_offset(quo, rem, crho) * 64;
-    if constexpr (SPLIT) clist0 = invariant_slot(clist, ck, rt.seg_cap);
+    if constexpr (SPLIT != 0) clist0 = invariant_slot(clist, ck, rt.seg_cap);
+    if constexpr (SPLIT == kFirstBounce) cur_k = ck, cur_h = iter_hash(b.iter_first + ck, 0);
     window_to(ec);
     const int crec = clist + (int)(uint32_t)(sub_word(ec) >> 32);
     if (lane == 0) fillc[cord & (kVisitRing - 1)] = crec + (first_rank - cstart);
@@ -1419,8 +1465,10 @@
     while (true) {
       const bool in = pending && rank < cstart + ccnt;
       if (in) at = clist + (rank - cstart), rs = cord;
-      if constexpr (SPLIT)
+      if constexpr (SPLIT != 0)
         if (in) at0 = clist0 + (rank - cstart);
+      if constexpr (SPLIT == kFirstBounce)
+        if (in) rs = (int)pack_visit(cur_k, cord), next_h = cur_h;
       pending = pending && !in;
       if (!ballot(pending) || ce >= ne || cord - cord0 >= kVisitsPerRefill) break;
       cstart += ccnt;
@@ -1451,9 +1499,9 @@
   int nx_rs = 0;
   int* slot_rs = reinterpret_cast<int*>(slots + kSlotVisit) + lane;
   auto fetch = [&](int at, [[maybe_unused]] int at0, int rs) {
-    if constexpr (SLOTS && SPLIT) fetch_split_to_lds(in0, in1, at, at0, s_base), *slot_rs = rs;
-    else if constexpr (SLOTS) fetch_record_to_lds(in0, in1, in2, at, s_base), *slot_rs = rs;
-    else if constexpr (SPLIT) {
+    if constexpr (SLOTS && SPLIT == kSplitRecords) fetch_split_to_lds(in0, in1, at, at0, s_base), *slot_rs = rs;
+    else if constexpr (SLOTS) fetch_record_to_lds(in0, in1, in2, SPLIT == kFirstBounce ? at0 : at, s_base), *slot_rs = rs;
+    else if constexpr (SPLIT == kSplitRecords) {
       const ptd::Word4 w0 = in.r[qbase + at], w1 = in.r[in.stride + qbase + at0];
       nx.o = mk(w0.x, w0.y, w0.z), nx.d = mk(w0.w, w1.x, w1.y), nx.c = mk(w1.z, w1.w, 0.f), nx_rs = rs;
     } else nx = path_load(in, qbase + at), nx_rs = rs;
@@ -1464,7 +1512,7 @@
   bool valid = false, fresh = false, owes = false;
   bool has_next = false;
   int streamed = 0, p_hi = 0;
-  while (true) {
+  while (SPLIT != kFirstBounce) {
     if (streamed >= p_hi && p_hi >= 0) {
       int nextp = -1;
       if (cord == 0) nextp = r;
@@ -1486,7 +1534,7 @@
       v4f w0, w1;
       float cz;
       int nslot, nrs;
-      if constexpr (SLOTS && SPLIT) {
+      if constexpr (SLOTS && SPLIT == kSplitRecords) {
         asm volatile(
             "s_waitcnt vmcnt(0)\n\t"
             "ds_read_b128 %0, %3\n\t"
@@ -1498,17 +1546,7 @@
             : "memory");
         cz = 0.f, nslot = 0;
       } else if constexpr (SLOTS) {
-        asm volatile(
-            "s_waitcnt vmcnt(0)\n\t"
-            "ds_read_b128 %0, %5\n\t"
-            "ds_read_b128 %1, %5 offset:1024\n\t"
-            "ds_read_b32 %2, %6\n\t"
-            "ds_read_b32 %3, %6 offset:256\n\t"
-            "ds_read_b32 %4, %6 offset:512\n\t"
-            "s_waitcnt lgkmcnt(0)"
-            : "=&v"(w0), "=&v"(w1), "=&v"(cz), "=&v"(nslot), "=&v"(nrs)
-            : "v"(s16), "v"(s4)
-            : "memory");
+        read_record_slot(s16, s4, w0, w1, cz, nslot, nrs);
       } else {
         w0 = v4f{nx.o.x, nx.o.y, nx.o.z, nx.d.x}, w1 = v4f{nx.d.y, nx.d.z, nx.c.x, nx.c.y}, cz = nx.c.z, nslot = nx.tag.slot, nrs = nx_rs;
       }
@@ -1516,7 +1554,7 @@
         rt.rec[rslot] = ptd::Word4{c.x, c.y, c.z, __int_as_float(slot & ((1 << b.slot_shift) - 1))};
         owes = false;
       }
-      if constexpr (SPLIT) {
+      if constexpr (SPLIT == kSplitRecords) {
         if (take) {
           const uint32_t word = __float_as_uint(w0.w);
           const ptd::Mat* m = mats + __float_as_int(w1.w);
@@ -1608,6 +1646,114 @@
       }
     }
   }
+  if constexpr (SPLIT == kFirstBounce) {
+    static_assert(MODE == kLdsTables, "the first-bounce form takes its records from the refill slots of the LDS-table form");
+    while (true) {
+      if (ballot(fresh)) {
+        if constexpr (kFast) paths_search(cy, (cfloat4*)(uintptr_t)sc.top_b, tword, ntop, geoms, o, d, fresh, lane, mark);
+        else paths_search(cy, top, tword, ntop, geoms, o, d, fresh, lane, mark);
+      }
+      bool ready = valid && (cy.processed - mark) >= 0;
+      if (cy.count > 0 && __popcll(ballot(ready)) < kPathsMinReady) {
+        paths_chunk(cy, cy.count, lane, o, d, tword, geoms);
+        ready = valid;
+      }
+      fresh = false;
+      Bounce bo;
+      bo.kind = 0, bo.rng_x = 1u, bo.roughness = 0.f;
+      f3 axis = mk(0.f, 0.f, 0.f);
+      bool go = false;
+      {
+        ShadeIO s;
+        s.o = mk(0.f, 0.f, 0.f);
+        s.d = d;
+        s.c = c;
+        s.alive = false;
+        const int k = (int)((uint32_t)slot >> b.slot_shift);
+        const unsigned long long best = cy.best[lane];
+        Hit h{false, -1.0f, -1, 0, mk(0.f, 0.f, 0.f), mk(0.f, 0.f, 0.f)};
+        if (ready) {
+          if ((uint32_t)(best >> 32) != 0x7f7fffffu) {
+            h.t = __uint_as_float((uint32_t)(best >> 32));
+            const float* rr = cy.rec + lane;
+            h.n = mk(rr[0 * 64], rr[1 * 64], rr[2 * 64]);
+            h.p = mk(rr[3 * 64], rr[4 * 64], rr[5 * 64]);
+            h.mat = lmat[(uint32_t)best & 63u];
+          }
+          const uint32_t ih = he > 0 ? ihash[(depth - 1) * he + k] : iter_hash(b.iter_first + k, depth);
+          bo = shade_decide(mats, b.trace_depth, depth, ih ^ phash, h.t, h.mat, s);
+        }
+        const bool alive = ready && s.alive, dead = ready && !s.alive;
+        if (dead) atomicAdd(&died[depth & 63], 1);
+        if (dead) rslot = atomicAdd(&fillc[rslot & (kVisitRing - 1)], 1);
+        if (ready) {
+          c = s.c;
+          if (alive) {
+            const BounceAxis a = bounce_axis(bo, h.n, h.p, d);
+            o = a.o, axis = a.f, go = true;
+          } else valid = false, owes = true;
+        }
+      }
+      if (streamed >= p_hi && p_hi >= 0) {
+        int nextp = -1;
+        if (cord == 0) nextp = r;
+        else if (pieces.needs_counter()) {
+          int v = 0;
+          if (lane == 0) v = atomicAdd(&qs.deal[dm.piece_counter(q)], 1);
+          nextp = wq + __builtin_amdgcn_readfirstlane(v);
+        }
+        const PieceRange pr = pieces.piece_range(nextp);
+        if (pr.some) {
+          streamed = pr.start, p_hi = pr.end;
+          seek(streamed);
+        } else {
+          p_hi = -1;
+        }
+      }
+      const bool take = !valid && has_next;
+      if (ballot(take || owes || (!valid && !has_next && streamed < p_hi))) {
+        v4f w0, w1;
+        float cz;
+        int word, vword;
+        read_record_slot(s16, s4, w0, w1, cz, word, vword);
+        if (owes) {
+          rt.rec[rslot] = ptd::Word4{c.x, c.y, c.z, __int_as_float(slot & ((1 << b.slot_shift) - 1))};
+          owes = false;
+        }
+        if (take) {
+          const int pl = first_pixel(word, b.slot_shift), k = visit_k((uint32_t)vword);
+          const f3 hn = mk(w0.w, w1.x, w1.y), cam_d = mk(w1.z, w1.w, cz);
+          slot = make_slot(b, k, pl), rslot = visit_number((uint32_t)vword);
+          phash = utilhash((uint32_t)global_pixel(b, pl));
+          ShadeIO s;
+          s.o = mk(0.f, 0.f, 0.f);
+          s.d = cam_d;
+          s.c = mk(1.0f, 1.0f, 1.0f);
+          s.alive = false;
+          bo = shade_decide(mats, b.trace_depth, 0, next_h ^ phash, 0.0f, first_material(word, b.slot_shift), s);
+          o = mk(w0.x, w0.y, w0.z), c = s.c;
+          axis = bo.kind == 1 ? bounce_reflect(cam_d, hn) : hn;
+          depth = 0;
+          valid = go = true;
+          has_next = false;
+        }
+        const bool lapping = ballot(valid && visit_gap(cord, rslot) >= kVisitLap) != 0ull;
+        const bool empty = !has_next && !lapping;
+        const unsigned long long em = ballot(empty);
+        const int rank = rank_in(em);
+        const bool more = empty && streamed + rank < p_hi;
+        int at = 0, at0 = 0, rs = 0;
+        const bool served = assign(more, streamed + rank, at, at0, rs);
+        if (served) {
+          has_next = true;
+          fetch(at, at0, rs);
+        }
+        streamed += (int)__popcll(ballot(served));
+      }
+      if (!ballot(valid || has_next) && p_hi < 0) break;
+      if (go) d = bounce_sample(bo, axis), depth += 1, fresh = true;
+    }
+  }
   if (lane == 0) {
     int reached = 0, rays = 0;
     for (int dd = min(b.trace_depth - 1, 63); dd >= 2; --dd) {
diff --git a/cosc_4397_pathtracing_raytracing_project_amd/csrc/pt_launch.inc b/cosc_4397_pathtracing_raytracing_project_amd/csrc/pt_launch.inc
--- a/cosc_4397_pathtracing_raytracing_project_amd/csrc/pt_launch.inc
+++ b/cosc_4397_pathtracing_raytracing_project_amd/csrc/pt_launch.inc
@@ -20,12 +20,14 @@
   return f(k_features<false, true>, intersect_lds<false>(sc).total);
 }
 template <Search S, typename F>
-void with_primary_of(const SceneTables& sc, bool share, bool split, F&& f) {
+void with_primary_of(const SceneTables& sc, bool share, int split, F&& f) {
   const int lds = primary_lds<S, kFast, kD0>(sc).total;
-  return !share ? f(k_primary<S>, lds) : split ? f(k_primary<S, true, true>, lds) : f(k_primary<S, true>, lds);
+  if constexpr (S == kLdsTables)
+    if (share && split == kFirstBounce) return f(k_primary<S, true, kFirstBounce>, lds);
+  return !share ? f(k_primary<S>, lds) : split ? f(k_primary<S, true, kSplitRecords>, lds) : f(k_primary<S, true>, lds);
 }
 template <typename F>
-void with_primary(const SceneTables& sc, bool share, bool split, F&& f) {
+void with_primary(const SceneTables& sc, bool share, int split, F&& f) {
   switch (search_form(sc)) {
     case kLdsTables: return with_primary_of<kLdsTables>(sc, share, split, f);
     case kTopScan: return with_primary_of<kTopScan>(sc, share, split, f);
@@ -34,16 +36,18 @@
 }
 
 template <typename F>
-void with_paths(const SceneTables& sc, Search form, bool split, F&& f) {
+void with_paths(const SceneTables& sc, Search form, int split, F&& f) {
   switch (form) {
-    case kLdsTables: return split ? f(k_paths<kLdsTables, true>, paths_lds<kLdsTables, kFast>(sc).total) : f(k_paths<kLdsTables>, paths_lds<kLdsTables, kFast>(sc).total);
-    case kTopScan: return split ? f(k_paths<kTopScan, true>, paths_lds<kTopScan, kFast>(sc).total) : f(k_paths<kTopScan>, paths_lds<kTopScan, kFast>(sc).total);
-    case kGrid: return split ? f(k_paths<kGrid, true>, paths_lds<kGrid, kFast>(sc).total) : f(k_paths<kGrid>, paths_lds<kGrid, kFast>(sc).total);
+    case kLdsTables:
+      if (split == kFirstBounce) return f(k_paths<kLdsTables, kFirstBounce>, paths_lds<kLdsTables, kFast>(sc).total);
+      return split ? f(k_paths<kLdsTables, kSplitRecords>, paths_lds<kLdsTables, kFast>(sc).total) : f(k_paths<kLdsTables>, paths_lds<kLdsTables, kFast>(sc).total);
+    case kTopScan: return split ? f(k_paths<kTopScan, kSplitRecords>, paths_lds<kTopScan, kFast>(sc).total) : f(k_paths<kTopScan>, paths_lds<kTopScan, kFast>(sc).total);
+    case kGrid: return split ? f(k_paths<kGrid, kSplitRecords>, paths_lds<kGrid, kFast>(sc).total) : f(k_paths<kGrid>, paths_lds<kGrid, kFast>(sc).total);
   }
 }
 int paths_lds_bytes(const SceneTables& sc, Search form) {
   int bytes = 0;
-  with_paths(sc, form, false, [&](auto, int lds) { bytes = lds; });
+  with_paths(sc, form, 0, [&](auto, int lds) { bytes = lds; });
   return bytes;
 }
 int lds_share_limit(int bytes);
@@ -79,9 +83,9 @@
   if (tbl <= kLdsTableBytes && leaves_fit_top(sc)) {
     SceneTables in = sc;
     in.lds_table_bytes = tbl;
-    with_paths(in, kLdsTables, false, occupancy_into(with, 0));
+    with_paths(in, kLdsTables, 0, occupancy_into(with, 0));
   }
-  with_paths(sc, kTopScan, false, occupancy_into(without, 1));
+  with_paths(sc, kTopScan, 0, occupancy_into(without, 1));
   (void)hipGetLastError();
   return (with >= without && with > 0) ? tbl : -1;
 }
@@ -96,9 +100,15 @@
     case kGenerate: query(k_generate, 0); break;
     case kIntersect: with_intersect(sc, false, false, query); break;
     case kIntersectLegacy: with_intersect(sc, true, false, query); break;
-    case kPrimary: with_primary(sc, false, false, query_share); break;
-    case kPrimaryShared: with_primary(sc, true, false, query_share), m = n, with_primary(sc, true, true, query_share), n = min(n, m); break;
-    case kPaths: with_paths(resolve_scan_nodes(sc), search_form(sc), false, query_share), m = n, with_paths(resolve_scan_nodes(sc), search_form(sc), true, query_share), n = min(n, m); break;
+    case kPrimary: with_primary(sc, false, 0, query_share); break;
+    case kPrimaryShared:
+      for (int form : {0, kSplitRecords, kFirstBounce}) with_primary(sc, true, form, query_share), m = form ? min(m, n) : n;
+      n = m;
+      break;
+    case kPaths:
+      for (int form : {0, kSplitRecords, kFirstBounce}) with_paths(resolve_scan_nodes(sc), search_form(sc), form, query_share), m = form ? min(m, n) : n;
+      n = m;
+      break;
     case kShade: query(k_shade, shade_lds<true>(sc).total); break;
     case kFeatures: with_features(sc, query); break;
   }
@@ -124,7 +134,7 @@
 
 void launch_primary(hipStream_t s, int grid, const SceneTables& sc, const ptd::Camera& cam, const BatchInfo& b,
                     const ptd::Queues& qs, int32_t* cnt0, int32_t* cnt_out, ptd::PathBuf out, ptd::RetireBuf ret) {
-  with_primary(sc, primary_shares(b), primary_shares(b) && b.split_records != 0, [&](auto kernel, int lds) { hipLaunchKernelGGL(kernel, dim3(grid), dim3(kBlock), lds, s, sc, cam, b, qs, cnt0, cnt_out, out, ret); });
+  with_primary(sc, primary_shares(b), primary_shares(b) ? b.split_records : 0, [&](auto kernel, int lds) { hipLaunchKernelGGL(kernel, dim3(grid), dim3(kBlock), lds, s, sc, cam, b, qs, cnt0, cnt_out, out, ret); });
 }
 
 void launch_features(hipStream_t s, int grid, const SceneTables& sc, const ptd::Camera& cam, const BatchInfo& b, float4* feat) {
@@ -136,7 +146,7 @@
 
 void launch_paths(hipStream_t s, int grid, const SceneTables& sc_in, const BatchInfo& b, const ptd::Queues& qs, int32_t* cnt, ptd::PathBuf in, ptd::RetireBuf ret) {
   const SceneTables sc = resolve_scan_nodes(sc_in);
-  with_paths(sc, search_form(sc), b.split_records != 0, [&](auto kernel, int lds) { hipLaunchKernelGGL(kernel, dim3(grid), dim3(kBlock), lds, s, sc, b, qs, cnt, in, ret); });
+  with_paths(sc, search_form(sc), b.split_records, [&](auto kernel, int lds) { hipLaunchKernelGGL(kernel, dim3(grid), dim3(kBlock), lds, s, sc, b, qs, cnt, in, ret); });
 }
 void launch_shade(hipStream_t s, int grid, const SceneTables& sc, const BatchInfo& b, int depth, const ptd::Queues& qs,
                   const int32_t* cnt_in, int32_t* cnt_out, ptd::PathBuf in, ptd::HitBuf hits, ptd::PathBuf out,
diff --git a/cosc_4397_pathtracing_raytracing_project_amd/csrc/pt_sched.h b/cosc_4397_pathtracing_raytracing_project_amd/csrc/pt_sched.h
--- a/cosc_4397_pathtracing_raytracing_project_amd/csrc/pt_sched.h
+++ b/cosc_4397_pathtracing_raytracing_project_amd/csrc/pt_sched.h
@@ -150,6 +150,31 @@
 PT_SCHED uint32_t pack_kind(int sample_id, bool specular) { return (uint32_t)sample_id | (specular ? 0x80000000u : 0u); }
 PT_SCHED int kind_sample_id(uint32_t word) { return (int)(word & 0x7fffffffu); }
 PT_SCHED bool kind_specular(uint32_t word) { return (word >> 31) != 0u; }
+
+constexpr int kNoFirstBounce = 8192;
+constexpr int kSplitRecords = 1, kFirstBounce = 2;
+constexpr int kVisitBits = 8;
+PT_SCHED uint32_t pack_visit(int k, int visit) { return ((uint32_t)k << kVisitBits) | ((uint32_t)visit & ((1u << kVisitBits) - 1u)); }
+PT_SCHED int visit_k(uint32_t word) { return (int)(word >> kVisitBits); }
+PT_SCHED int visit_number(uint32_t word) { return (int)(word & ((1u << kVisitBits) - 1u)); }
+PT_SCHED int visit_gap(int visits_now, int visit) { return (visits_now - visit) & ((1 << kVisitBits) - 1); }
+PT_SCHED bool visit_k_fits(int K) { return K <= (1 << (31 - kVisitBits)); }
+PT_SCHED int pack_first(int pl, int mat, int slot_shift) { return (mat << slot_shift) | pl; }
+PT_SCHED int first_pixel(int word, int slot_shift) { return word & ((1 << slot_shift) - 1); }
+PT_SCHED int first_material(int word, int slot_shift) { return (int)((uint32_t)word >> slot_shift); }
+PT_SCHED bool first_material_fits(int num_mats, int slot_shift) { return num_mats <= (1 << (31 - slot_shift)); }
+PT_SCHED bool first_bounces(int primary_share, bool aa_jitter, bool flat, int trace_depth, int debug_flags, int search_form, int num_mats,
+                            int slot_shift, int K) {
+  return splits_records(primary_share, aa_jitter, flat, trace_depth, debug_flags) &&
+         retires_once(primary_share, aa_jitter, flat, trace_depth, debug_flags) && !(debug_flags & kNoFirstBounce) && search_form == 0 &&
+         first_material_fits(num_mats, slot_shift) && visit_k_fits(K);
+}
+PT_SCHED bool first_bounces(const BatchInfo& b, int debug_flags, int search_form, int num_mats) {
+  return first_bounces(b.primary_share, b.aa_jitter != 0, b.flat != 0, b.trace_depth, debug_flags, search_form, num_mats, b.slot_shift, b.K);
+}
+PT_SCHED int record_form(const BatchInfo& b, int debug_flags, int search_form, int num_mats) {
+  return first_bounces(b, debug_flags, search_form, num_mats) ? kFirstBounce : splits_records(b, debug_flags) ? kSplitRecords : 0;
+}
 
 PT_SCHED int pack_paths_pieces(int count, int min_piece) { return count | min_piece << 16; }
 PT_SCHED int paths_pieces_count(int word) { return word & 0xffff; }
diff --git a/cosc_4397_pathtracing_raytracing_project_amd/csrc/pt_shade.inc b/cosc_4397_pathtracing_raytracing_project_amd/csrc/pt_shade.inc
--- a/cosc_4397_pathtracing_raytracing_project_amd/csrc/pt_shade.inc
+++ b/cosc_4397_pathtracing_raytracing_project_amd/csrc/pt_shade.inc
@@ -60,14 +60,23 @@
   if (kFast || kFloatTrig) return madd(hn, 0.001f, hp);
   return add(hp, scl(hn, 0.001f));
 }
+struct BounceAxis {
+  f3 o, f;
+};
+PT_DEV f3 bounce_reflect(f3 d, f3 hn) {
+  if (kFast || kFloatTrig) return madd(hn, -2.0f * dot(d, hn), d);
+  return sub(d, scl(hn, 2.0f * dot(d, hn)));
+}
+PT_DEV BounceAxis bounce_axis(const Bounce& bo, f3 hn, f3 hp, f3 d) {
+  const f3 refl = bounce_reflect(d, hn);
+  return BounceAxis{bounce_origin(hn, hp), bo.kind == 1 ? refl : hn};
+}
 template <bool HW>
-PT_DEV void shade_bounce_float(const Bounce& bo, f3 hn, f3 hp, ShadeIO& s) {
+PT_DEV f3 bounce_sample_float(const Bounce& bo, f3 f) {
   MinStd rng(1u);
   rng.x = bo.rng_x;
   const bool spec = bo.kind == 1;
   const float r1 = rng.u01(), r2 = rng.u01(), r3 = rng.u01();
-  const f3 refl = madd(hn, -2.0f * dot(s.d, hn), s.d);
-  const f3 f = spec ? refl : hn;
   const float rev = bo.roughness * r1 * 0.25f;
   const float ct = HW ? __builtin_amdgcn_sqrtf(1.0f - r1) : __builtin_sqrtf(1.0f - r1);
   const float st2 = __builtin_fmaxf(fma_(-ct, ct, 1.0f), 0.0f);
@@ -93,19 +102,16 @@
   local_frame(f, tangent, bitangent);
   const f3 pert = normalize(madd(tangent, x, madd(f, y, scl(bitangent, z))));
   const bool perturb = !spec || bo.roughness > 0.0f;
-  s.o = bounce_origin(hn, hp);
-  s.d = perturb ? pert : refl;
-}
-PT_DEV void shade_bounce(const Bounce& bo, f3 hn, f3 hp, ShadeIO& s) {
-  if (kFast) return shade_bounce_float<true>(bo, hn, hp, s);
-  if (kFloatTrig) return shade_bounce_float<false>(bo, hn, hp, s);
+  return perturb ? pert : f;
+}
+PT_DEV f3 bounce_sample(const Bounce& bo, f3 f) {
+  if (kFast) return bounce_sample_float<true>(bo, f);
+  if (kFloatTrig) return bounce_sample_float<false>(bo, f);
   const double kPi = 3.14159265358979323846;
   MinStd rng(1u);
   rng.x = bo.rng_x;
   const bool spec = bo.kind == 1;
   const float r1 = rng.u01(), r2 = rng.u01(), r3 = rng.u01();
-  const f3 refl = sub(s.d, scl(hn, 2.0f * dot(s.d, hn)));
-  const f3 f = spec ? refl : hn;
   const float angle = (float)((double)(bo.roughness * r1) * kPi * (double)0.5f);
   const float theta = ptmath::acosf32(__builtin_sqrtf(1.0f - r1));
   const float phi = (float)((double)2.0f * kPi * (double)r2);
@@ -123,8 +129,12 @@
   local_frame(f, tangent, bitangent);
   const f3 pert = normalize(add(add(scl(tangent, x), scl(f, y)), scl(bitangent, z)));
   const bool perturb = !spec || bo.roughness > 0.0f;
-  s.o = bounce_origin(hn, hp);
-  s.d = perturb ? pert : refl;
+  return perturb ? pert : f;
+}
+PT_DEV void shade_bounce(const Bounce& bo, f3 hn, f3 hp, ShadeIO& s) {
+  const BounceAxis a = bounce_axis(bo, hn, hp, s.d);
+  s.o = a.o;
+  s.d = bounce_sample(bo, a.f);
 }
 
 
diff --git a/include/pt_amd.h b/include/pt_amd.h
--- a/include/pt_amd.h
+++ b/include/pt_amd.h
@@ -98,6 +98,7 @@
   int32_t grid_cells;
   int32_t tight_leaves;
   int32_t paths_waves;
+  int32_t record_form;
 } PtStats;
 
 typedef struct PtScene PtScene;
```
